# kkahatapitiya/Coarse-Fine-Networks

Hardware: AMD Instinct MI355X
Metric: clips/sec (fwd+bwd+SGD) x3d_fine X3D-M T=256x224x224 (higher is better)
Workload: dtype f32; 1 GPU; x3d_fine X3D-M train step (fwd+loss+bwd+SGD), 8x3x256x224x224 clips per GPU, random-init weights; clips_per_gpu=8, frames=256, parallelism=dp1, launch=eager

## Files before the change

### coarse-fine-networks_amd/cfn_hip/ops.py

```python
import torch
from torch.autograd import Function
from torch.autograd.function import once_differentiable

import ctypes
import threading

from . import call, call_try, check, query, ACT_NONE, ACT_RELU, ACT_SWISH, ACT_SIGMOID


_scratch_epoch = [0]


class _ZeroArena(object):
    CHUNK = 1 << 20

    def __init__(self):
        self.buf, self.off, self.epoch = {}, {}, _scratch_epoch[0]

    def take(self, numel, dev):
        if self.epoch != _scratch_epoch[0]:
            self.buf, self.off, self.epoch = {}, {}, _scratch_epoch[0]
        numel_al = (numel + 1) & ~1
        key = (dev.type, dev.index)
        if key not in self.buf or self.off[key] + numel_al > self.buf[key].numel():
            self.buf[key] = torch.zeros(max(self.CHUNK, numel_al), dtype=torch.float64, device=dev)
            self.off[key] = 0
        o = self.off[key]
        self.off[key] = o + numel_al
        return self.buf[key][o:o + numel]


class _GradCast(object):

    def __init__(self):
        self._reset()
        self.last_total = 0

    def _reset(self):
        self.cur, self.live, self.scheduled, self.seen, self.task = {}, [], False, set(), None

    def begin(self):
        tid = torch._C._current_graph_task_id()
        if tid != self.task:
            if self.live:
                self.flush()
            self._reset()
            self.task = tid

    def first_use(self, w):
        if id(w) in self.seen:
            return False
        self.seen.add(id(w))
        return True

    def take(self, numel, shape, dev):
        al = (numel + 3) & ~3
        key = (dev.type, dev.index)
        ch = self.cur.get(key)
        if ch is None or ch['off'] + al > ch['f64'].numel():
            size = max(int(self.last_total * 1.05) + 1024, al, 1 << 16)
            ch = {'f64': torch.zeros(size, dtype=torch.float64, device=dev),
                  'f32': torch.empty(size, dtype=torch.float32, device=dev), 'off': 0, 'done': 0}
            self.cur[key] = ch
            self.live.append(ch)
        o = ch['off']
        ch['off'] = o + al
        if not self.scheduled:
            torch.autograd.Variable._execution_engine.queue_callback(self._end_of_backward)
            self.scheduled = True
        return ch['f64'][o:o + numel], ch['f32'][o:o + numel].view(shape)

    def flush(self):
        for ch in self.live:
            if ch['off'] > ch['done']:
                ch['f32'][ch['done']:ch['off']].copy_(ch['f64'][ch['done']:ch['off']])
                ch['done'] = ch['off']

    def _end_of_backward(self):
        self.flush()
        self.last_total = max(sum(ch['off'] for ch in self.live), 1)
        self._reset()


class _PerThread(threading.local):

    def __init__(self):
        self.arena = _ZeroArena()
        self.gradcast = _GradCast()


_tls = _PerThread()
LAZY_GRAD_CAST = True


def _f64(n, c, dev):
    return _tls.arena.take(n * c, dev).view(n, c)


def _f64pair(n, c, dev):
    t = _tls.arena.take(2 * n * c, dev).view(2, n, c)
    return t, t[0], t[1]


def reset_scratch():
    _scratch_epoch[0] += 1


def flush_grad_casts():
    _tls.gradcast.flush()


def allow_lazy_grad_cast(params, ok=True):
    for p in params:
        p._cfn_lazy_grad_ok = bool(ok)


def _lazy_ok(w):
    if not LAZY_GRAD_CAST or w is None or not w.is_leaf or w.grad is not None or torch.is_grad_enabled():
        return False
    if not getattr(w, '_cfn_lazy_grad_ok', False):
        return False
    if w._backward_hooks:
        return False
    hooks = getattr(w, '_post_accumulate_grad_hooks', None)
    if hooks:
        from .dist import _BucketHook
        if not all(isinstance(h, _BucketHook) for h in hooks.values()):
            return False
    return True


def _lazy_ok_probe(w):
    with torch.no_grad():
        return _lazy_ok(w)


def _grad_owner(w):
    if w is not None and not w.is_leaf and w._is_view():
        base = w._base
        if base is not None and base.is_leaf and base.numel() == w.numel() and w.is_contiguous() and base.is_contiguous():
            return base
    return w


def _gw_buffers(w, rows, cols, dev):
    gc = _tls.gradcast
    owner = _grad_owner(w)
    if _lazy_ok(owner):
        gc.begin()
        if gc.first_use(owner):
            g64, g32 = gc.take(rows * cols, tuple(w.shape), dev)
            return g64.view(rows, cols), (lambda: g32)
        gc.flush()
    g64 = _f64(rows, cols, dev)
    return g64, (lambda: g64.float().view(tuple(w.shape)))


def _opt(t):
    return None if t is None else t.contiguous()


def _coef(t, rows=None, cols=None):
    if t is None:
        return None
    if rows is not None and t.numel() != rows * cols:
        raise RuntimeError('per-sample coefficients of %d x %d channels expected, got a tensor of shape %s' % (rows, cols, tuple(t.shape)))
    return t.to(torch.float64).contiguous()


class ShortcutToken(object):

    def __init__(self):
        self.acc, self.acc_stride, self.main_done = None, 1, False


class TailLink(object):

    def __init__(self):
        self.y_scale = self.res_scale = None
        self.done = False


def _bf(t):
    return t is not None and t.dtype in (torch.bfloat16, torch.float16)


def subsample_hw(x, s):
    N, C, T, H, W = x.shape
    out = torch.empty(N, C, T, (H - 1) // s + 1, (W - 1) // s + 1, dtype=x.dtype, device=x.device)
    call('cfn_subsample_hw' + _sfx(x), x, out, N * C * T, H, W, s)
    return out


class _PwConv(Function):

    @staticmethod
    def forward(ctx, x, A, B, w, act, stride, want_stats, token, role, tail=None, tail_role=None):
        x = check(x).contiguous()
        N, Cin, T, H, W = x.shape
        Cout = w.shape[0]
        Ho, Wo = (H - 1) // stride + 1, (W - 1) // stride + 1
        y = torch.empty(N, Cout, T, Ho, Wo, dtype=x.dtype, device=x.device)
        s = q = None
        if want_stats:
            s, q = _f64(N, Cout, x.device), _f64(N, Cout, x.device)
        w2 = w.reshape(Cout, Cin).contiguous()
        A, B = _coef(A, N, Cin), _coef(B, N, Cin)
        xs = None
        if _bf(x):
            xs = subsample_hw(x, stride) if stride > 1 else x
            call('cfn_pwconv_fwd' + _sfx(x), xs, A, B, act, w2, y, s, q, N, Cin, Cout, T * Ho * Wo)
        else:
            call('cfn_pwconv_fwd', x, A, B, act, w2, y, s, q, N, Cin, Cout, T, H, W, stride)
        ctx.save_for_backward(x, A, B, w2, y, xs if stride > 1 else None)
        ctx.meta = (act, stride, tuple(w.shape))
        ctx.wparam = w
        ctx.token, ctx.role = token, role
        ctx.tail, ctx.tail_role = tail, tail_role
        if not want_stats:
            return y, None, None
        return y, s, q

    @staticmethod
    @once_differentiable
    def backward(ctx, gy, gs, gq):
        x, A, B, w2, y, xs = ctx.saved_tensors
        act, stride, wshape = ctx.meta
        token, role = ctx.token, ctx.role
        N, Cin, T, H, W = x.shape
        Cout = w2.shape[0]
        gy = torch.zeros_like(y) if gy is None else gy.contiguous()
        gs, gq = _opt(gs), _opt(gq)
        gsc = None
        if ctx.tail is not None and ctx.tail.done:
            gsc = ctx.tail.y_scale if ctx.tail_role == 'y' else ctx.tail.res_scale
        if _bf(x):
            return _PwConv._backward_bf16(ctx, gy, gs, gq, gsc)
        gx = gA = gB = gw = None
        g64 = fin = None
        fused = False
        if ctx.needs_input_grad[0] or (A is not None and ctx.needs_input_grad[1]):
            if token is not None and role == 'short' and stride > 1 and not token.main_done:
                Ho, Wo = y.shape[3], y.shape[4]
                da = torch.empty(N, Cin, T, Ho, Wo, dtype=torch.float32, device=x.device)
                call('cfn_pwconv_bwd_data_acc', gy, y, gs, gq, w2, None, None, None, ACT_NONE, da, None, None, N, Cin, Cout, T,
                     Ho, Wo, 1, None, 1, gsc)
                token.acc, token.acc_stride = da, stride
            else:
                gx = torch.zeros_like(x) if stride != 1 else torch.empty_like(x)
                ab = a64 = b64 = None
                if A is not None:
                    ab, a64, b64 = _f64pair(N, Cin, x.device)
                acc, acc_stride = None, 1
                if token is not None and role == 'main':
                    if token.acc is not None:
                        acc, acc_stride, token.acc = token.acc, token.acc_stride, None
                    else:
                        token.main_done = True
                if stride == 1 and ctx.needs_input_grad[3]:
                    g64, fin = _gw_buffers(ctx.wparam, Cout, Cin, x.device)
                    fused = call_try('cfn_pwconv_bwd_fused', gy, y, gs, gq, w2, x, A, B, act, gx, a64, b64, g64, N, Cin, Cout,
                                     T, H, W, acc, acc_stride, gsc)
                if not fused:
                    call('cfn_pwconv_bwd_data_acc', gy, y, gs, gq, w2, x, A, B, act, gx, a64, b64, N, Cin, Cout, T, H, W, stride,
                         acc, acc_stride, gsc)
                if A is not None:
                    gA, gB = ab[0], ab[1]
        if ctx.needs_input_grad[3]:
            if g64 is None:
                g64, fin = _gw_buffers(ctx.wparam, Cout, Cin, x.device)
            if not fused:
                call('cfn_pwconv_bwd_weight', gy, y, gs, gq, x, A, B, act, g64, N, Cin, Cout, T, H, W, stride, gsc)
            gw = fin()
        return gx, gA, gB, gw, None, None, None, None, None, None, None

    @staticmethod
    def _backward_bf16(ctx, gy, gs, gq, gsc):
        x, A, B, w2, y, xs = ctx.saved_tensors
        act, stride, wshape = ctx.meta
        token, role = ctx.token, ctx.role
        N, Cin, T, H, W = x.shape
        Cout = w2.shape[0]
        Ho, Wo = y.shape[3], y.shape[4]
        xin = xs if stride > 1 else x
        gx = gA = gB = gw = None
        if ctx.needs_input_grad[0] or (A is not None and ctx.needs_input_grad[1]):
            if token is not None and role == 'short' and stride > 1 and not token.main_done:
                da = torch.empty(N, Cin, T, Ho, Wo, dtype=x.dtype, device=x.device)
                call('cfn_pwconv_bwd_data' + _sfx(gy), gy, y, gs, gq, w2, None, None, None, ACT_NONE, da, None, None, N, Cin, Cout, T,
                     Ho, Wo, None, 1, gsc)
                token.acc, token.acc_stride = da, stride
            else:
                ab = a64 = b64 = None
                if A is not None:
                    ab, a64, b64 = _f64pair(N, Cin, x.device)
                acc, acc_stride = None, 1
                if token is not None and role == 'main':
                    if token.acc is not None:
                        acc, acc_stride, token.acc = token.acc, token.acc_stride, None
                    else:
                        token.main_done = True
                gxc = torch.empty_like(xin)
                call('cfn_pwconv_bwd_data' + _sfx(gy), gy, y, gs, gq, w2, xin, A, B, act, gxc, a64, b64, N, Cin, Cout, T, Ho, Wo,
                     acc, acc_stride, gsc)
                if stride > 1:
                    gx = torch.zeros_like(x)
                    gx[:, :, :, ::stride, ::stride] = gxc
                else:
                    gx = gxc
                if A is not None:
                    gA, gB = ab[0], ab[1]
        if ctx.needs_input_grad[3]:
            g64, fin = _gw_buffers(ctx.wparam, Cout, Cin, x.device)
            call('cfn_pwconv_bwd_weight' + _sfx(gy), gy, y, gs, gq, xin, A, B, act, g64, N, Cin, Cout, T * Ho * Wo, gsc)
            gw = fin()
        return gx, gA, gB, gw, None, None, None, None, None, None, None


def pwconv(x, w, A=None, B=None, act=ACT_NONE, stride=1, stats=True, token=None, role=None, tail=None, tail_role=None):
    N, Cin, T, H, W = x.shape
    Ho, Wo = (H - 1) // stride + 1, (W - 1) // stride + 1
    es = x.element_size()
    lim = (1 << 31) if es == 4 else (1 << 30)
    span = max(Cin * H * W, w.shape[0] * H * W, w.shape[0] * Ho * Wo, Cin * Ho * Wo) * es
    needs_grad = torch.is_grad_enabled() and any(t is not None and t.requires_grad for t in (x, w, A, B))
    if span * T < lim or needs_grad or T == 1:
        return _PwConv.apply(x, A, B, w, act, stride, stats, token, role, tail, tail_role)
    step = max((lim - 1) // span, 1)
    odd_plane = es == 2 and (Ho * Wo) % 2 == 1
    if odd_plane:
        if 2 * span >= lim:
            raise RuntimeError('pwconv: two frames of %d x %d x %d bf16 elements exceed the 1 GiB buffer range the frame-range '
                               'chunking has to respect (odd plane: frames travel in pairs)' % (max(Cin, w.shape[0]), H, W))
        step = max(step & ~1, 2)
    y = torch.empty(N, w.shape[0], T, Ho, Wo, dtype=x.dtype, device=x.device)
    s = q = None
    t0 = 0
    while t0 < T:
        t1 = min(t0 + step, T)
        if odd_plane and (t1 - t0) % 2 and t1 - t0 > 1:
            t1 -= 1
        pad = odd_plane and (t1 - t0) % 2 == 1
        xc = x[:, :, t0:t1].contiguous()
        if pad:
            xc = torch.cat([xc, torch.zeros_like(xc)], 2)
        yc, sc, qc = _PwConv.apply(xc, A, B, w, act, stride, False if pad else stats, None, None)
        if pad:
            yc = yc[:, :, :1]
            if stats:
                sc, qc = yc.double().sum((2, 3, 4)), (yc.double() ** 2).sum((2, 3, 4))
        y[:, :, t0:t1] = yc
        if stats:
            s, q = (sc, qc) if s is None else (s + sc, q + qc)
        t0 = t1
    return y, s, q


def _sfx(t):
    return '_bf16' if t.dtype == torch.bfloat16 else ('_f16' if t.dtype == torch.float16 else '')


class _DwConv3d(Function):

    @staticmethod
    def forward(ctx, x, A, B, w, act, stride, want_stats):
        x = check(x).contiguous()
        N, C, T, H, W = x.shape
        Ho, Wo = (H + 2 - 3) // stride + 1, (W + 2 - 3) // stride + 1
        y = torch.empty(N, C, T, Ho, Wo, dtype=x.dtype, device=x.device)
        s = q = None
        if want_stats:
            s, q = _f64(N, C, x.device), _f64(N, C, x.device)
        w2 = w.reshape(C, 27).contiguous()
        A, B = _coef(A, N, C), _coef(B, N, C)
        call('cfn_dwconv3d_fwd' + _sfx(x), x, A, B, act, w2, y, s, q, N, C, T, H, W, stride)
        ctx.save_for_backward(x, A, B, w2, y)
        ctx.meta = (act, stride, tuple(w.shape))
        ctx.wparam = w
        if not want_stats:
            return y, None, None
        return y, s, q

    @staticmethod
    @once_differentiable
    def backward(ctx, gy, gs, gq):
        x, A, B, w2, y = ctx.saved_tensors
        act, stride, wshape = ctx.meta
        N, C, T, H, W = x.shape
        gy = torch.zeros_like(y) if gy is None else gy.contiguous()
        gs, gq = _opt(gs), _opt(gq)
        gx = gA = gB = gw = None
        want_x = ctx.needs_input_grad[0] or (A is not None and ctx.needs_input_grad[1])
        want_w = ctx.needs_input_grad[3]
        ab = a64 = b64 = g64 = fin = None
        if want_x:
            gx = torch.empty_like(x)
            if A is not None:
                ab, a64, b64 = _f64pair(N, C, x.device)
        if want_w:
            g64, fin = _gw_buffers(ctx.wparam, C, 27, x.device)
        sfx = _sfx(x)
        fused = want_x and want_w and stride == 1 and call_try('cfn_dwconv3d_bwd_fused' + sfx, gy, y, gs, gq, w2, x, A, B, act,
                                                             gx, a64, b64, g64, N, C, T, H, W)
        if not fused and want_x and want_w and stride == 2:
            fused = call_try('cfn_dwconv3d_bwd_fused_s2' + sfx, gy, y, gs, gq, w2, x, A, B, act, gx, a64, b64, g64, N, C, T, H, W)
        if not fused:
            if want_x:
                call('cfn_dwconv3d_bwd_data' + sfx, gy, y, gs, gq, w2, x, A, B, act, gx, a64, b64, N, C, T, H, W, stride)
            if want_w:
                call('cfn_dwconv3d_bwd_weight' + sfx, gy, y, gs, gq, x, A, B, act, g64, N, C, T, H, W, stride)
        if want_x and A is not None:
            gA, gB = ab[0], ab[1]
        if want_w:
            gw = fin()
        return gx, gA, gB, gw, None, None, None


def dwconv3d(x, w, A=None, B=None, act=ACT_NONE, stride=1, stats=True):
    return _DwConv3d.apply(x, A, B, w, act, stride, stats)


class _DwConvT5(Function):

    @staticmethod
    def forward(ctx, x, w, want_stats, out_dtype=None):
        x = check(x, torch.float32).contiguous()
        N, C, T, H, W = x.shape
        y = torch.empty_like(x, dtype=out_dtype or x.dtype)
        s = q = None
        if want_stats:
            s, q = _f64(N, C, x.device), _f64(N, C, x.device)
        w2 = w.reshape(C, 5).contiguous()
        call('cfn_dwconv_t5_fwd' + _sfx(y), x, w2, y, s, q, N, C, T, H * W)
        ctx.save_for_backward(x, w2, y)
        ctx.wshape = tuple(w.shape)
        ctx.wparam = w
        if not want_stats:
            return y, None, None
        return y, s, q

    @staticmethod
    @once_differentiable
    def backward(ctx, gy, gs, gq):
        x, w2, y = ctx.saved_tensors
        N, C, T, H, W = x.shape
        gy = torch.zeros_like(y) if gy is None else gy.contiguous()
        gs, gq = _opt(gs), _opt(gq)
        gx = gw = None
        want_x, want_w = ctx.needs_input_grad[0], ctx.needs_input_grad[1]
        if want_x:
            gx = torch.empty_like(x)
        if want_w:
            g64, fin = _gw_buffers(ctx.wparam, C, 5, x.device)
        fused = want_x and want_w and call_try('cfn_dwconv_t5_bwd_fused' + _sfx(y), gy, y, gs, gq, w2, x, gx, g64, N, C, T, H * W)
        if not fused:
            if want_x:
                call('cfn_dwconv_t5_bwd_data' + _sfx(y), gy, y, gs, gq, w2, gx, N, C, T, H * W)
            if want_w:
                call('cfn_dwconv_t5_bwd_weight' + _sfx(y), gy, y, gs, gq, x, g64, N, C, T, H * W)
        if want_w:
            gw = fin()
        return gx, gw, None, None


def dwconv_t5(x, w, stats=True, out_dtype=None):
    return _DwConvT5.apply(x, w, stats, out_dtype)


class _StemConv(Function):

    @staticmethod
    def forward(ctx, x, w):
        x = check(x).contiguous()
        N, Ci, T, H, W = x.shape
        Co = w.shape[0]
        Ho, Wo = (H + 2 - 3) // 2 + 1, (W + 2 - 3) // 2 + 1
        y = torch.empty(N, Co, T, Ho, Wo, dtype=torch.float32, device=x.device)
        w2 = w.reshape(Co, Ci * 9).contiguous()
        call('cfn_stem_conv_fwd', x, w2, y, N, Ci, Co, T, H, W)
        ctx.save_for_backward(x)
        ctx.wshape = tuple(w.shape)
        ctx.wparam = w
        return y

    @staticmethod
    @once_differentiable
    def backward(ctx, gy):
        (x,) = ctx.saved_tensors
        N, Ci, T, H, W = x.shape
        Co = ctx.wshape[0]
        gw = None
        if ctx.needs_input_grad[1]:
            g64, fin = _gw_buffers(ctx.wparam, Co, Ci * 9, x.device)
            call('cfn_stem_conv_bwd_weight', gy.contiguous(), x, g64, N, Ci, Co, T, H, W)
            gw = fin()
        return None, gw


def stem_conv(x, w):
    return _StemConv.apply(x, w)


class _BnFold(Function):

    @staticmethod
    def forward(ctx, s, q, gamma, beta, w1, b1, w2, b2, bufs, cfg):
        training, N, C, S, count, eps, momentum, pool_count = cfg
        run_mean, run_var, nbt = bufs
        dev = run_mean.device
        Wd = w1.shape[0] if w1 is not None else 0
        Se = S if training else 1
        A = torch.empty(N, C, dtype=torch.float64, device=dev)
        B = torch.empty_like(A)
        mean = torch.empty(Se, C, dtype=torch.float64, device=dev)
        rstd = torch.empty_like(mean)
        A0 = B0 = gate = hbuf = pooled = None
        w1c = w2c = None
        if Wd:
            A0, B0, gate, pooled = (torch.empty(N, C, dtype=torch.float32, device=dev) for _ in range(4))
            hbuf = torch.empty(N, Wd, dtype=torch.float32, device=dev)
            w1c, w2c = w1.reshape(Wd, C).contiguous(), w2.reshape(C, Wd).contiguous()
        s, q = _opt(s), _opt(q)
        call('cfn_bn_fold_fwd', s, q, gamma, beta, run_mean, run_var, nbt if training else None, int(training), N, C, S,
             float(count), float(eps), float(momentum), w1c, b1, w2c, b2, Wd, float(pool_count), A, B, mean, rstd,
             A0, B0, gate, hbuf, pooled)
        ctx.save_for_backward(s, gamma, mean, rstd, A0, B0, gate, hbuf, pooled, w1c, w2c)
        ctx.cfg = (training, N, C, S, Wd, count, pool_count, None if w1 is None else tuple(w1.shape),
                   None if w2 is None else tuple(w2.shape))
        return A, B

    @staticmethod
    @once_differentiable
    def backward(ctx, gA, gB):
        s, gamma, mean, rstd, A0, B0, gate, hbuf, pooled, w1c, w2c = ctx.saved_tensors
        training, N, C, S, Wd, count, pool_count, w1s, w2s = ctx.cfg
        dev = mean.device
        gA = torch.zeros(N, C, dtype=torch.float64, device=dev) if gA is None else gA.contiguous()
        gB = torch.zeros(N, C, dtype=torch.float64, device=dev) if gB is None else gB.contiguous()
        gs = gq = None
        if training:
            gs = torch.empty(N, C, dtype=torch.float64, device=dev)
            gq = torch.empty_like(gs)
        elif Wd:
            gs = torch.empty(N, C, dtype=torch.float64, device=dev)
        gg = gbt = None
        if gamma is not None:
            gg, gbt = torch.empty(C, device=dev), torch.empty(C, device=dev)
        gw1 = gb1 = gw2 = gb2 = tA = tB = None
        if Wd:
            gw1, gb1 = torch.empty(Wd, C, device=dev), torch.empty(Wd, device=dev)
            gw2, gb2 = torch.empty(C, Wd, device=dev), torch.empty(C, device=dev)
            tA, tB = (torch.empty(N, C, dtype=torch.float64, device=dev) for _ in range(2))
        call('cfn_bn_fold_bwd', gA, gB, s, gamma, mean, rstd, A0, B0, gate, hbuf, pooled, w1c, w2c, int(training), N, C, S,
             Wd, float(count), float(pool_count), gs, gq, gg, gbt, gw1, gb1, gw2, gb2, tA, tB)
        if Wd:
            gw1, gw2 = gw1.view(w1s), gw2.view(w2s)
        return gs, gq, gg, gbt, gw1, gb1, gw2, gb2, None, None


def bn_fold(s, q, gamma, beta, bufs, training, N, C, S, count, eps, momentum, se=None, pool_count=1.0):
    w1, b1, w2, b2 = se if se is not None else (None, None, None, None)
    return _BnFold.apply(s, q, gamma, beta, w1, b1, w2, b2, bufs, (training, N, C, S, count, eps, momentum, pool_count))


class _BnAddRelu(Function):

    @staticmethod
    def forward(ctx, y, A, B, res, Ar, Br, split, link):
        y, res = check(y).contiguous(), check(res).contiguous()
        N, C = y.shape[:2]
        vol = y[0, 0].numel()
        if tuple(res.shape) != tuple(y.shape):
            raise RuntimeError('bn_add_relu: residual %s does not match y %s' % (tuple(res.shape), tuple(y.shape)))
        out = torch.empty_like(y)
        A, B, Ar, Br = _coef(A, N, C), _coef(B, N, C), _coef(Ar, N, C), _coef(Br, N, C)
        mask = None
        sfx = _sfx(y)
        if link is not None:
            words = query('cfn_bn_add_relu_mask_words' + sfx, N * C, vol)
            if words > 0:
                mask = torch.empty(words, dtype=torch.int32, device=y.device)
        call('cfn_bn_add_relu_fwd' + sfx, y, A, B, res, Ar, Br, out, mask, N * C, vol)
        ctx.link, ctx.has_mask = link, mask is not None
        ctx.save_for_backward(y, A, res, Ar, mask if mask is not None else out)
        if not split:
            return out
        alias = torch.empty(0, dtype=out.dtype, device=out.device).set_(out.untyped_storage(), out.storage_offset(),
                                                                         out.shape, out.stride())
        return out, alias

    @staticmethod
    @once_differentiable
    def backward(ctx, gout, gout2=None):
        y, A, res, Ar, out = ctx.saved_tensors
        N, C = y.shape[:2]
        vol = y[0, 0].numel()
        if gout is None:
            gout, gout2 = gout2, None
        if gout is None:
            gout = torch.zeros_like(y)
        gout2 = None if gout2 is None else gout2.contiguous()
        t3 = _tls.arena.take(3 * N * C, y.device).view(3, N, C)
        gA, gB = t3[0], t3[1]
        gAr = t3[2] if Ar is not None else None
        gBr = gB if Ar is not None else None
        link = ctx.link
        if link is not None:
            g = torch.empty_like(y)
            mask = out if ctx.has_mask else None
            call('cfn_bn_add_relu_bwd_g' + _sfx(y), gout.contiguous(), gout2, None if ctx.has_mask else out, mask, y,
                 res if Ar is not None else None, g, gA, gB, gAr, N * C, vol)
            link.y_scale, link.res_scale, link.done = A.detach(), (None if Ar is None else Ar.detach()), True
            g2 = torch.empty(0, dtype=g.dtype, device=g.device).set_(g.untyped_storage(), g.storage_offset(), g.shape, g.stride())
            return g, gA, gB, g2, gAr, gBr, None, None
        if _bf(y):
            g = torch.empty_like(y)
            call('cfn_bn_add_relu_bwd_g' + _sfx(y), gout.contiguous(), gout2, out, None, y, res if Ar is not None else None, g, gA, gB,
                 gAr, N * C, vol)
            shp = (N, C) + (1,) * (y.dim() - 2)
            gres = g if Ar is None else (g.float() * Ar.float().view(shp)).to(y.dtype)
            return (g.float() * A.float().view(shp)).to(y.dtype), gA, gB, gres, gAr, gBr, None, None
        gy, gres = torch.empty_like(y), torch.empty_like(res)
        call('cfn_bn_add_relu_bwd', gout.contiguous(), gout2, out, y, A, res, Ar, gy, gres, gA, gB, gAr, N * C, vol)
        return gy, gA, gB, gres, gAr, gBr, None, None


def bn_add_relu(y, A, B, res, Ar=None, Br=None, split=False, link=None):
    return _BnAddRelu.apply(y, A, B, res, Ar, Br, split, link)


class _AffineAct(Function):
    @staticmethod
    def forward(ctx, x, A, B, act):
        x = check(x).contiguous()
        N, C = x.shape[:2]
        out = torch.empty_like(x)
        A, B = _coef(A, N, C), _coef(B, N, C)
        call('cfn_affine_act_fwd', x, A, B, act, out, N * C, x[0, 0].numel())
        ctx.save_for_backward(x, A, B)
        ctx.act = act
        return out

    @staticmethod
    @once_differentiable
    def backward(ctx, gout):
        x, A, B = ctx.saved_tensors
        N, C = x.shape[:2]
        gx = torch.empty_like(x)
        a64, b64 = _f64(N, C, x.device), _f64(N, C, x.device)
        call('cfn_affine_act_bwd', gout.contiguous(), x, A, B, ctx.act, gx, a64, b64, N * C, x[0, 0].numel())
        return gx, a64, b64, None


def affine_act(x, A, B, act=ACT_NONE):
    return _AffineAct.apply(x, A, B, act)


class _ChannelStats(Function):

    @staticmethod
    def forward(ctx, x):
        x = check(x).contiguous()
        N, C = x.shape[:2]
        s, q = _f64(N, C, x.device), _f64(N, C, x.device)
        call('cfn_channel_stats', x, s, q, N * C, x[0, 0].numel())
        ctx.save_for_backward(x)
        return s, q

    @staticmethod
    @once_differentiable
    def backward(ctx, gs, gq):
        (x,) = ctx.saved_tensors
        N, C = x.shape[:2]
        gx = torch.zeros_like(x)
        shp = (N, C) + (1,) * (x.dim() - 2)
        if gs is not None:
            gx = gx + gs.float().view(shp)
        if gq is not None:
            gx = gx + 2.0 * gq.float().view(shp) * x
        return gx


def channel_stats(x):
    return _ChannelStats.apply(x)


class _PoolHW(Function):

    @staticmethod
    def forward(ctx, x, A, B, act, OH, OW):
        x = check(x).contiguous()
        N, C, T, H, W = x.shape
        out = torch.empty(N, C, T, OH, OW, dtype=torch.float32, device=x.device)
        A, B = _coef(A, N, C), _coef(B, N, C)
        call('cfn_pool_hw_fwd' + _sfx(x), x, A, B, act, out, N * C, T, H, W, OH, OW)
        ctx.save_for_backward(x, A, B)
        ctx.meta = (act, OH, OW)
        return out

    @staticmethod
    @once_differentiable
    def backward(ctx, gout):
        x, A, B = ctx.saved_tensors
        act, OH, OW = ctx.meta
        N, C, T, H, W = x.shape
        gx = torch.empty_like(x)
        a64 = b64 = None
        if A is not None:
            a64, b64 = _f64(N, C, x.device), _f64(N, C, x.device)
        call('cfn_pool_hw_bwd' + _sfx(x), gout.contiguous(), x, A, B, act, gx, a64, b64, N * C, T, H, W, OH, OW)
        if A is None:
            return gx, None, None, None, None, None
        return gx, a64, b64, None, None, None


def pool_hw(x, OH, OW, A=None, B=None, act=ACT_NONE):
    return _PoolHW.apply(x, A, B, act, OH, OW)


class _Film(Function):

    @staticmethod
    def forward(ctx, x, m, c, f):
        x, m, c = check(x).contiguous(), check(m).contiguous(), check(c).contiguous()
        N, C, T, H, W = x.shape
        want = (N, C, T, H // f if f > 0 else -1, W // f if f > 0 else -1)
        if f <= 0 or H % f or W % f or tuple(m.shape) != want or tuple(c.shape) != want:
            raise RuntimeError('film: coefficients %s / %s do not tile x %s with %d x %d blocks (expected %s)'
                               % (tuple(m.shape), tuple(c.shape), tuple(x.shape), f, f, want))
        out = torch.empty_like(x)
        call('cfn_film_fwd', x, m, c, out, N * C, T, H, W, f)
        ctx.save_for_backward(x, m)
        ctx.f = f
        return out

    @staticmethod
    @once_differentiable
    def backward(ctx, g):
        x, m = ctx.saved_tensors
        N, C, T, H, W = x.shape
        gx, gm, gc = torch.empty_like(x), torch.empty_like(m), torch.empty_like(m)
        call('cfn_film_bwd', g.contiguous(), x, m, gx, gm, gc, N * C, T, H, W, ctx.f)
        return gx, gm, gc, None


def film(x, m, c, f):
    return _Film.apply(x, m, c, f)


class _TimeSample(Function):

    @staticmethod
    def forward(ctx, x, cdf):
        x, cdf = check(x).contiguous(), check(cdf).contiguous()
        B, C, Tin = x.shape[:3]
        K = cdf.shape[1]
        P = x[0, 0, 0].numel()
        out = torch.empty((B, C, K) + tuple(x.shape[3:]), dtype=torch.float32, device=x.device)
        call('cfn_time_sample_fwd', x, cdf, out, B, C, Tin, K, P)
        ctx.save_for_backward(x, cdf)
        return out

    @staticmethod
    @once_differentiable
    def backward(ctx, g):
        x, cdf = ctx.saved_tensors
        B, C, Tin = x.shape[:3]
        K = cdf.shape[1]
        P = x[0, 0, 0].numel()
        gx = torch.empty_like(x) if ctx.needs_input_grad[0] else None
        g64 = torch.zeros(B, K, dtype=torch.float64, device=x.device) if ctx.needs_input_grad[1] else None
        call('cfn_time_sample_bwd', g.contiguous(), x, cdf, gx, g64, B, C, Tin, K, P)
        return gx, (g64.float() if g64 is not None else None)


def time_sample(x, cdf):
    return _TimeSample.apply(x, cdf)


class _TimePool(Function):

    @staticmethod
    def forward(ctx, x, mode, R):
        x = check(x, torch.float32).contiguous()
        B, C, T = x.shape[:3]
        P = x[0, 0, 0].numel()
        out = torch.empty((B, C, T // R) + tuple(x.shape[3:]), dtype=torch.float32, device=x.device)
        call('cfn_time_pool_fwd', x, out, mode, B * C, T, R, P)
        ctx.save_for_backward(x)
        ctx.meta = (mode, R)
        return out

    @staticmethod
    @once_differentiable
    def backward(ctx, g):
        (x,) = ctx.saved_tensors
        mode, R = ctx.meta
        B, C, T = x.shape[:3]
        gx = torch.empty_like(x)
        call('cfn_time_pool_bwd', g.contiguous(), x, gx, mode, B * C, T, R, x[0, 0, 0].numel())
        return gx, None, None


def time_pool(x, mode, R=4):
    return _TimePool.apply(x, {'avg': 0, 'max': 1}[mode], R)


def grid_time_index(cdf, Tin):
    cdf = check(cdf).contiguous()
    i0 = torch.empty(cdf.shape, dtype=torch.int32, device=cdf.device)
    w1 = torch.empty(cdf.shape, dtype=torch.float32, device=cdf.device)
    call('cfn_grid_time_index', cdf, cdf.numel(), Tin, i0, w1)
    return i0, w1


class _Interp1d(Function):
    @staticmethod
    def forward(ctx, x, y, xnew):
        x, y, xnew = check(x).contiguous(), check(y).contiguous(), check(xnew).contiguous()
        B = max(x.shape[0], y.shape[0], xnew.shape[0])
        N, Pq = x.shape[1], xnew.shape[1]
        rows = (int(x.shape[0] > 1), int(y.shape[0] > 1), int(xnew.shape[0] > 1))
        ynew = torch.empty(B, Pq, dtype=torch.float32, device=x.device)
        ind = torch.empty(B, Pq, dtype=torch.int64, device=x.device)
        call('cfn_interp1d_fwd', x, y, xnew, ynew, ind, B, N, Pq, *rows)
        ctx.save_for_backward(x, y, xnew, ind)
        ctx.rows = rows
        ctx.mark_non_differentiable(ind)
        return ynew, ind

    @staticmethod
    @once_differentiable
    def backward(ctx, g, _gind):
        x, y, xnew, ind = ctx.saved_tensors
        B, Pq = ind.shape
        N = x.shape[1]
        gx = torch.zeros_like(x) if ctx.needs_input_grad[0] else None
        gy = torch.zeros_like(y) if ctx.needs_input_grad[1] else None
        gq = torch.zeros_like(xnew) if ctx.needs_input_grad[2] else None
        call('cfn_interp1d_bwd', g.contiguous(), x, y, xnew, ind, gx, gy, gq, B, N, Pq, *ctx.rows)
        return gx, gy, gq


def interp1d(x, y, xnew):
    return _Interp1d.apply(x, y, xnew)


class _TimeResize(Function):

    @staticmethod
    def forward(ctx, x, L, align_corners):
        x = check(x).contiguous()
        BC = x.shape[0] * x.shape[1]
        Kin = x.shape[2]
        P = x[0, 0, 0].numel()
        out = torch.empty(tuple(x.shape[:2]) + (L,) + tuple(x.shape[3:]), dtype=torch.float32, device=x.device)
        call('cfn_time_resize_fwd', x, out, BC, Kin, L, P, int(bool(align_corners)))
        ctx.meta = (tuple(x.shape), L, int(bool(align_corners)))
        return out

    @staticmethod
    @once_differentiable
    def backward(ctx, g):
        shape, L, ac = ctx.meta
        gx = torch.empty(shape, dtype=torch.float32, device=g.device)
        P = 1
        for d in shape[3:]:
            P *= d
        call('cfn_time_resize_bwd', g.contiguous(), gx, shape[0] * shape[1], shape[2], L, P, ac)
        return gx, None, None


def time_resize(x, L, align_corners=True):
    return _TimeResize.apply(x, L, align_corners)


def _geom(kernel, stride, padding):
    return (ctypes.c_int * 9)(*(tuple(kernel) + tuple(stride) + tuple(padding)))


class _ConvDense(Function):

    @staticmethod
    def forward(ctx, x, A, B, w, act, kernel, stride, padding, want_stats):
        x = check(x).contiguous()
        N, Ci, T, H, W = x.shape
        Co = w.shape[0]
        g = _geom(kernel, stride, padding)
        To = (T + 2 * padding[0] - kernel[0]) // stride[0] + 1
        Ho = (H + 2 * padding[1] - kernel[1]) // stride[1] + 1
        Wo = (W + 2 * padding[2] - kernel[2]) // stride[2] + 1
        y = torch.empty(N, Co, To, Ho, Wo, dtype=torch.float32, device=x.device)
        s = q = None
        if want_stats:
            s, q = _f64(N, Co, x.device), _f64(N, Co, x.device)
        w2 = w.reshape(Co, -1).contiguous()
        A, B = _coef(A, N, Ci), _coef(B, N, Ci)
        call('cfn_conv3d_dense_fwd', x, A, B, act, w2, y, s, q, N, Ci, Co, T, H, W, g)
        ctx.save_for_backward(x, A, B, w2, y)
        ctx.meta = (act, tuple(kernel), tuple(stride), tuple(padding), tuple(w.shape))
        ctx.wparam = w
        if not want_stats:
            return y, None, None
        return y, s, q

    @staticmethod
    @once_differentiable
    def backward(ctx, gy, gs, gq):
        x, A, B, w2, y = ctx.saved_tensors
        act, kernel, stride, padding, wshape = ctx.meta
        N, Ci, T, H, W = x.shape
        Co = w2.shape[0]
        g = _geom(kernel, stride, padding)
        gy = torch.zeros_like(y) if gy is None else gy.contiguous()
        gs, gq = _opt(gs), _opt(gq)
        gx = gA = gB = gw = None
        if ctx.needs_input_grad[0] or (A is not None and ctx.needs_input_grad[1]):
            gx = torch.empty_like(x)
            ab = a64 = b64 = None
            if A is not None:
                ab, a64, b64 = _f64pair(N, Ci, x.device)
            call('cfn_conv3d_dense_bwd_data', gy, y, gs, gq, w2, x, A, B, act, gx, a64, b64, N, Ci, Co, T, H, W, g)
            if A is not None:
                gA, gB = ab[0], ab[1]
        if ctx.needs_input_grad[3]:
            g64, fin = _gw_buffers(ctx.wparam, Co, w2.shape[1], x.device)
            call('cfn_conv3d_dense_bwd_weight', gy, y, gs, gq, x, A, B, act, g64, N, Ci, Co, T, H, W, g)
            gw = fin()
        return gx, gA, gB, gw, None, None, None, None, None


def conv3d_dense(x, w, kernel, stride, padding, A=None, B=None, act=ACT_NONE, stats=True):
    return _ConvDense.apply(x, A, B, w, act, kernel, stride, padding, stats)


class _FusionGather(Function):

    @staticmethod
    def forward(ctx, x, at_raw, at_bias, GX, mask, crops):
        x, at_raw, GX, mask = check(x).contiguous(), check(at_raw).contiguous(), check(GX).contiguous(), check(mask).contiguous()
        B, C, Tf, P = x.shape
        K = GX.shape[2]
        if GX.shape[0] != B * crops or GX.shape[1] != Tf or tuple(mask.shape) != (B, Tf) or tuple(at_raw.shape) != (B, Tf, P):
            raise RuntimeError('fusion_gather: inconsistent shapes x %s at %s GX %s mask %s crops %d'
                               % (tuple(x.shape), tuple(at_raw.shape), tuple(GX.shape), tuple(mask.shape), crops))
        z = torch.empty(B * crops, C, K, P, dtype=torch.float32, device=x.device)
        den = torch.empty(B * crops, K, P, dtype=torch.float32, device=x.device)
        call('cfn_fusion_gather_fwd', x, at_raw, at_bias, GX, mask, z, den, B, crops, C, Tf, K, P)
        ctx.save_for_backward(x, at_raw, at_bias, GX, mask, z, den)
        ctx.crops = crops
        return z

    @staticmethod
    @once_differentiable
    def backward(ctx, gz):
        x, at_raw, at_bias, GX, mask, z, den = ctx.saved_tensors
        B, C, Tf, P = x.shape
        K, crops = GX.shape[2], ctx.crops
        need = ctx.needs_input_grad
        gx = torch.empty_like(x) if need[0] else None
        want_at = need[1] or (at_bias is not None and need[2])
        gat = torch.empty_like(at_raw) if want_at else None
        gGX = torch.empty_like(GX) if need[3] else None
        dw = torch.empty(B * crops, Tf, K, P, dtype=torch.float32, device=x.device)
        call('cfn_fusion_gather_bwd', gz.contiguous(), z, den, x, at_raw, at_bias, GX, mask, gx, gat, gGX, dw, B, crops, C, Tf, K, P)
        gb = gat.sum().view(at_bias.shape) if (at_bias is not None and need[2]) else None
        return gx, (gat if need[1] else None), gb, gGX, None, None


def fusion_gather(x, at_raw, at_bias, GX, mask, crops=1):
    return _FusionGather.apply(x, at_raw, at_bias, GX, mask, crops)


class _GaussAlign(Function):

    @staticmethod
    def forward(ctx, meta, mask, gx, tx, ratio, crops, K):
        meta, mask = meta.contiguous(), check(mask).contiguous()
        if meta.dtype != torch.int64:
            meta = meta.to(torch.int64)
        B, Tf = mask.shape
        if gx is not None:
            gx = check(gx).contiguous()
        GX = torch.empty(B * crops, Tf, K, dtype=torch.float32, device=mask.device)
        call('cfn_gauss_align_fwd', meta, mask, gx, float(tx), float(ratio), GX, B, crops, Tf, K)
        ctx.save_for_backward(meta, mask, gx)
        ctx.cfg = (float(tx), float(ratio), crops, K)
        return GX

    @staticmethod
    @once_differentiable
    def backward(ctx, gGX):
        meta, mask, gx = ctx.saved_tensors
        tx, ratio, crops, K = ctx.cfg
        ggx = None
        if gx is not None and ctx.needs_input_grad[2]:
            B, Tf = mask.shape
            ggx = torch.empty_like(gx)
            call('cfn_gauss_align_bwd', gGX.contiguous(), meta, mask, gx, tx, ratio, ggx, B, crops, Tf, K)
        return None, None, ggx, None, None, None, None


def gauss_align(meta, mask, gx, tx, ratio, crops, K):
    return _GaussAlign.apply(meta, mask, gx, 1.0 if tx is None else tx, ratio, crops, K)


class _GridCdf(Function):

    @staticmethod
    def forward(ctx, g, bias):
        g = check(g).contiguous()
        B, Kin = g.shape
        cdf = torch.empty(B, Kin + 1, dtype=torch.float32, device=g.device)
        call('cfn_grid_cdf_fwd', g, bias, cdf, B, Kin)
        ctx.save_for_backward(g, bias)
        return cdf

    @staticmethod
    @once_differentiable
    def backward(ctx, gcdf):
        g, bias = ctx.saved_tensors
        B, Kin = g.shape
        gg = torch.empty_like(g)
        call('cfn_grid_cdf_bwd', gcdf.contiguous(), g, bias, gg, B, Kin)
        gb = gg.sum().view(bias.shape) if (bias is not None and ctx.needs_input_grad[1]) else None
        return gg, gb


def grid_cdf(g, bias=None):
    return _GridCdf.apply(g, bias)
```

### coarse-fine-networks_amd/csrc/pw_common.h

```cpp
#pragma once
#include "cfn_common.h"

typedef float __attribute__((ext_vector_type(16))) f16v;
typedef float __attribute__((ext_vector_type(4))) f4v;

enum { PW_FWD = 0, PW_DGRAD = 1 };
#define PW_KC 32
#define PW_RED_PITCH 33

struct PwArgs {
    const float* src;
    const float* src2;
    const double* pa;
    const double* pb;
    const double* gs;
    const double* gq;
    const double* gsc;
    const float* w;
    float* dst;
    const float* ex;
    const double* ea;
    const double* eb;
    const float* acc; int acc_s, acc_Ho, acc_Wo;
    double* s1;
    double* s2;
    int N, M, K, Q, Pin, Hi, Wi, Ho, Wo, stride, act;
    int Cin;
    int mtiles, nstrips, tpb, kres, Kpad;
    int stem, Cimg, kT, kH, kW, sT, sH, sW, pT, pH, pW, Ti, To;
};

#define PW_UNIT 8
#define PW_KRES_MAX 512

__device__ __forceinline__ float pw_bload(__amdgpu_buffer_rsrc_t r, int voff, int soff) {
    return __builtin_bit_cast(float, __builtin_amdgcn_raw_buffer_load_b32(r, voff, soff, 0));
}


int pwd_try_launch(PwArgs& a, int mode, bool stats, hipStream_t st);

int pws_try_launch(PwArgs& a, int mode, bool stats, hipStream_t st);
int pwk_try_launch(PwArgs& a, int mode, bool stats, hipStream_t st);
int pwt_try_launch(PwArgs& a, int mode, bool stats, hipStream_t st);
int pws_terms_now();
int pws_wgrad_try_launch(const float* gy, const float* y, const double* gs, const double* gq, const double* gsc, const float* x,
                         const double* pa, const double* pb, int act, double* gw, int N, int M, int K, int Q, hipStream_t st);

int pwss_wgrad_try_bf16(const uint16_t* gy, const uint16_t* y, const double* gs, const double* gq, const double* gsc, const uint16_t* x,
                        const double* pa, const double* pb, int act, double* gw, int N, int M, int K, int Q, hipStream_t st);

int pwd_wgrad_try_launch(const float* gy, const float* y, const double* gs, const double* gq, const double* gsc, const float* x,
                         const double* pa, const double* pb, int act, double* gw, int N, int M, int K, int Q, hipStream_t st);
int pwd_wgrad_try_strided(const float* gy, const float* y, const double* gs, const double* gq, const double* gsc, const float* x,
                          const double* pa, const double* pb, int act, double* gw, int N, int M, int K, int T, int Hi, int Wi,
                          int stride, hipStream_t st);
int pwd_wgrad_try_dense(const float* gy, const float* y, const double* gs, const double* gq, const float* x, const double* pa,
                        const double* pb, int act, double* gw, int N, int M, int Cimg, int T, int Hi, int Wi, const int* g,
                        hipStream_t st);

int stem_fwd_try_launch(const float* x, const float* w, float* y, int N, int Cimg, int Cout, int T, int Hi, int Wi, hipStream_t st);
int stem_wgrad_try_launch(const float* gy, const float* x, double* gw, int N, int Cimg, int Cout, int T, int Hi, int Wi, hipStream_t st, bool probe);

int sal_fwd_try_launch(const float* x, const double* A, const double* B, int act, const float* w, float* y, double* sum,
                       double* sumsq, int N, int Cin, int Cout, int T, int Hi, int Wi, const int* g, hipStream_t st);
int pwfs_try_launch(const float* gy, const float* y, const double* gsum, const double* gsumsq, const float* w, const float* x, const double* A,
                    const double* B, int act, float* gx, double* gA, double* gB, double* gw, int N, int Cin, int Cout, int T, int Hi, int Wi,
                    const float* acc, int acc_stride, const double* gscale, hipStream_t st);
int salb_fwd_try_launch(const float* x, const double* A, const double* B, int act, const float* w, float* y, double* sum,
                        double* sumsq, int N, int Cin, int Cout, int T, int Hi, int Wi, const int* g, hipStream_t st);
int sal_wgrad_try_launch(const float* gy, const float* y, const double* gs, const double* gq, const float* x, const double* A,
                         const double* B, int act, double* gw, int N, int Cin, int Cout, int T, int Hi, int Wi, const int* g,
                         hipStream_t st);
```

### coarse-fine-networks_amd/csrc/pwfused.hip

```cpp
#include "cfn_common.h"
#include <stdlib.h>

#include "pw_common.h"

typedef float __attribute__((ext_vector_type(4))) pf4;

#define PF_PT 64
#define PF_PITCH 65

struct PfArgs {
    const float* gy; const float* y; const double* gs; const double* gq; const double* gsc;
    const float* w;
    const float* x; const double* pa; const double* pb;
    float* gx; double* gA; double* gB; double* gw;
    const float* acc; int acc_s, acc_Ho, acc_Wo, Hi, Wi, T;
    int N, M, K, Q, nstrips, stages;
};

template <int MTW, int NTW, int ACT>
__global__ __launch_bounds__(256, ACT < 0 ? 3 : 2) void pw_bwd_fused_kernel(const PfArgs a) {
    extern __shared__ __attribute__((aligned(16))) float smem[];
    constexpr bool EPI = ACT >= 0;
    constexpr int ACTV = EPI ? ACT : CFN_ACT_NONE;
    constexpr int BM = 32 * MTW, BN = 32 * NTW;
    constexpr int NG = BM / 16, NX = BN / 16;
    constexpr int NT16 = BN / 16, KS = BM / 4;
    const int tid = threadIdx.x, wave = tid >> 6, lane = tid & 63, half = lane >> 5, col = lane & 31;
    const int m16 = lane & 15, kq = lane >> 4;
    unsigned L = cfn_xcd_remap(blockIdx.x, gridDim.x);
    const int strip = L % a.nstrips;
    const int n = L / a.nstrips;
    const int M = a.M, K = a.K, Q = a.Q;

    constexpr int IMG = (BM + BN) * PF_PITCH;
    float* img0 = smem;
    float* sCg = smem + 2 * IMG;
    float* sCz = sCg + 2 * BM;
    float* sCx = sCz + BM;
    float* sSt = sCx + 2 * BN;
    for (int m = tid; m < BM; m += 256) {
        const bool ok = m < M;
        sCg[2 * m] = (ok && a.gs) ? (float)a.gs[(long)n * M + m] : 0.0f;
        sCg[2 * m + 1] = (ok && a.gq && a.y) ? 2.0f * (float)a.gq[(long)n * M + m] : 0.0f;
        sCz[m] = (ok && a.gsc) ? (float)a.gsc[(long)n * M + m] : 1.0f;
    }
    for (int k = tid; k < BN; k += 256) {
        const bool ok = EPI && k < K;
        sCx[2 * k] = ok ? (float)a.pa[(long)n * K + k] : 1.0f;
        sCx[2 * k + 1] = ok ? (float)a.pb[(long)n * K + k] : 0.0f;
    }
    float wq[NT16][KS];
#pragma unroll
    for (int t = 0; t < NT16; ++t)
#pragma unroll
        for (int s = 0; s < KS; ++s) {
            const int ci = t * 16 + m16, co = 4 * s + kq;
            wq[t][s] = (ci < K && co < M) ? a.w[(long)co * K + ci] : 0.0f;
        }
    float ca[NTW], cb[NTW];
#pragma unroll
    for (int j = 0; j < NTW; ++j) {
        const int k = j * 32 + col;
        const bool ok = EPI && k < K;
        ca[j] = ok ? (float)a.pa[(long)n * K + k] : 1.0f;
        cb[j] = ok ? (float)a.pb[(long)n * K + k] : 0.0f;
    }
    f16v acc[MTW][NTW];
#pragma unroll
    for (int i = 0; i < MTW; ++i)
#pragma unroll
        for (int j = 0; j < NTW; ++j)
#pragma unroll
            for (int r = 0; r < 16; ++r) acc[i][j][r] = 0.0f;
    float sa[NT16][4], sb[NT16][4];
#pragma unroll
    for (int t = 0; t < NT16; ++t)
#pragma unroll
        for (int r = 0; r < 4; ++r) { sa[t][r] = 0.0f; sb[t][r] = 0.0f; }
    __syncthreads();

    const int lrow = tid >> 4, c4 = (tid & 15) * 4;
    constexpr int OOB = 0x7ffffff0;
    __amdgpu_buffer_rsrc_t rg = cfn_rsrc(const_cast<float*>(a.gy + (long)n * M * Q), (unsigned)((long)M * Q * 4));
    __amdgpu_buffer_rsrc_t ry = cfn_rsrc(const_cast<float*>((a.y ? a.y : a.gy) + (long)n * M * Q), a.y ? (unsigned)((long)M * Q * 4) : 0u);
    __amdgpu_buffer_rsrc_t rx = cfn_rsrc(const_cast<float*>(a.x + (long)n * K * Q), (unsigned)((long)K * Q * 4));
    __amdgpu_buffer_rsrc_t rd = cfn_rsrc(a.gx + (long)n * K * Q, (unsigned)((long)K * Q * 4));
    pf4 pg[NG], py[NG], px[NX];
    int vog[NG], vox[NX];
#pragma unroll
    for (int it = 0; it < NG; ++it) vog[it] = (it * 16 + lrow) < M ? ((it * 16 + lrow) * Q + c4) * 4 : OOB;
#pragma unroll
    for (int it = 0; it < NX; ++it) vox[it] = (it * 16 + lrow) < K ? ((it * 16 + lrow) * Q + c4) * 4 : OOB;
    auto prefetch = [&](int q0) {
        const bool inq = q0 + c4 < Q;
#pragma unroll
        for (int it = 0; it < NG; ++it) {
            const int vo = inq ? vog[it] : OOB;
            pg[it] = __builtin_bit_cast(pf4, __builtin_amdgcn_raw_buffer_load_b128(rg, vo, q0 * 4, 0));
            py[it] = __builtin_bit_cast(pf4, __builtin_amdgcn_raw_buffer_load_b128(ry, vo, q0 * 4, 0));
        }
#pragma unroll
        for (int it = 0; it < NX; ++it)
            px[it] = __builtin_bit_cast(pf4, __builtin_amdgcn_raw_buffer_load_b128(rx, inq ? vox[it] : OOB, q0 * 4, 0));
    };
    auto stage = [&](int q0, float* sG, float* sX) {
        const bool inq = q0 + c4 < Q;
#pragma unroll
        for (int it = 0; it < NG; ++it) {
            const int row = it * 16 + lrow;
            const float cs = cfn_settle(sCg[2 * row]), cq = cfn_settle(sCg[2 * row + 1]), cz = cfn_settle(sCz[row]);
            const bool ok = inq && (row < M);
            float* d = sG + row * PF_PITCH + c4;
            d[0] = ok ? fmaf(py[it].x, cq, fmaf(pg[it].x, cz, cs)) : 0.0f;
            d[1] = ok ? fmaf(py[it].y, cq, fmaf(pg[it].y, cz, cs)) : 0.0f;
            d[2] = ok ? fmaf(py[it].z, cq, fmaf(pg[it].z, cz, cs)) : 0.0f;
            d[3] = ok ? fmaf(py[it].w, cq, fmaf(pg[it].w, cz, cs)) : 0.0f;
        }
#pragma unroll
        for (int it = 0; it < NX; ++it) {
            const int row = it * 16 + lrow;
            float* d = sX + row * PF_PITCH + c4;
            d[0] = px[it].x; d[1] = px[it].y; d[2] = px[it].z; d[3] = px[it].w;
        }
    };

    const int qbeg = strip * a.stages * PF_PT;
    const int nst = min(a.stages, (Q - qbeg + PF_PT - 1) / PF_PT);
    if (nst > 0) {
        prefetch(qbeg);
        stage(qbeg, img0, img0 + BM * PF_PITCH);
        if (nst > 1) prefetch(qbeg + PF_PT);
    }
    __syncthreads();
    const int pbase = wave * (PF_PT / 4);
    const int hw = a.Hi * a.Wi;
    const int acc_pitch4 = a.T * a.acc_Ho * a.acc_Wo * 4;
    __amdgpu_buffer_rsrc_t racc = cfn_rsrc(const_cast<float*>(a.acc ? a.acc + (long)n * K * (acc_pitch4 / 4) : a.gy), a.acc ? (unsigned)((long)K * acc_pitch4) : 0u);
    for (int st = 0; st < nst; ++st) {
        const int q0 = qbeg + st * PF_PT;
        float* cur = img0 + (st & 1) * IMG;
        float* nxt = img0 + ((st + 1) & 1) * IMG;
        if (st + 1 < nst) {
            stage(q0 + PF_PT, nxt, nxt + BM * PF_PITCH);
            if (st + 2 < nst) prefetch(q0 + 2 * PF_PT);
        }
        const float* sG = cur;
        const float* sX = cur + BM * PF_PITCH;
#pragma unroll
        for (int s = 0; s < PF_PT / 8; ++s) {
            const int p = pbase + 2 * s + half;
            float av[MTW], bv[NTW];
#pragma unroll
            for (int i = 0; i < MTW; ++i) av[i] = sG[(i * 32 + col) * PF_PITCH + p];
#pragma unroll
            for (int j = 0; j < NTW; ++j) {
                const float xr = sX[(j * 32 + col) * PF_PITCH + p];
                bv[j] = EPI ? cfn_act<ACTV>(fmaf(xr, ca[j], cb[j])) : xr;
            }
#pragma unroll
            for (int i = 0; i < MTW; ++i)
#pragma unroll
                for (int j = 0; j < NTW; ++j) acc[i][j] = __builtin_amdgcn_mfma_f32_32x32x2f32(av[i], bv[j], acc[i][j], 0, 0, 0);
        }
        pf4 da[NT16];
#pragma unroll
        for (int t = 0; t < NT16; ++t) da[t] = (pf4){0.f, 0.f, 0.f, 0.f};
#pragma unroll
        for (int s = 0; s < KS; ++s) {
            const float b = sG[(4 * s + kq) * PF_PITCH + pbase + m16];
#pragma unroll
            for (int t = 0; t < NT16; ++t) da[t] = __builtin_amdgcn_mfma_f32_16x16x4f32(wq[t][s], b, da[t], 0, 0, 0);
        }
        const int q = q0 + pbase + m16;
        const bool qv = q < Q;
        int aoff = OOB;
        if (a.acc && qv) {
            const int tq = q / hw, rq = q - tq * hw;
            const int hq = rq / a.Wi, wq_ = rq - hq * a.Wi;
            if (hq % a.acc_s == 0 && wq_ % a.acc_s == 0) aoff = (((tq * a.acc_Ho + hq / a.acc_s) * a.acc_Wo + wq_ / a.acc_s)) * 4;
        }
        float av4[NT16][4];
#pragma unroll
        for (int t = 0; t < NT16; ++t)
#pragma unroll
            for (int r = 0; r < 4; ++r) av4[t][r] = 0.0f;
        if (a.acc) {
            const unsigned arow = (unsigned)aoff + (unsigned)(4 * kq) * (unsigned)acc_pitch4;
#pragma unroll
            for (int t = 0; t < NT16; ++t)
#pragma unroll
                for (int r = 0; r < 4; ++r)
                    av4[t][r] = __builtin_bit_cast(float, __builtin_amdgcn_raw_buffer_load_b32(
                        racc, (int)(aoff == OOB ? (unsigned)OOB : arow + (unsigned)r * (unsigned)acc_pitch4), t * 16 * acc_pitch4, 0));
        }
#pragma unroll
        for (int t = 0; t < NT16; ++t) {
#pragma unroll
            for (int r = 0; r < 4; ++r) {
                const int ci = t * 16 + 4 * kq + r;
                const bool ok = qv && ci < K;
                float v = da[t][r] + av4[t][r];
                if (EPI) {
                    const float xr = sX[ci * PF_PITCH + pbase + m16];
                    const float pa = sCx[2 * ci], pb = sCx[2 * ci + 1];
                    const float dz = ok ? v * cfn_act_grad<ACTV>(fmaf(xr, pa, pb)) : 0.0f;
                    sa[t][r] = fmaf(dz, xr, sa[t][r]);
                    sb[t][r] += dz;
                    v = dz * pa;
                }
                __builtin_amdgcn_raw_buffer_store_b32(__builtin_bit_cast(unsigned, v), rd, ok ? (ci * Q + pbase + m16) * 4 : OOB, q0 * 4, 0);
            }
        }
        __syncthreads();
    }

    if (EPI) {
#pragma unroll
        for (int t = 0; t < NT16; ++t)
#pragma unroll
            for (int r = 0; r < 4; ++r) {
                float u = sa[t][r], v = sb[t][r];
#pragma unroll
                for (int o = 1; o < 16; o <<= 1) { u += __shfl_xor(u, o, 64); v += __shfl_xor(v, o, 64); }
                if (m16 == 0) {
                    const int ci = t * 16 + 4 * kq + r;
                    sSt[(wave * BN + ci) * 2] = u;
                    sSt[(wave * BN + ci) * 2 + 1] = v;
                }
            }
    }
    constexpr int CWP = BN + 1;
    float* cw = smem + wave * (BM * CWP);
#pragma unroll
    for (int i = 0; i < MTW; ++i)
#pragma unroll
        for (int j = 0; j < NTW; ++j)
#pragma unroll
            for (int r = 0; r < 16; ++r) {
                const int ml = i * 32 + (r & 3) + 8 * (r >> 2) + 4 * half;
                cw[ml * CWP + j * 32 + col] = acc[i][j][r];
            }
    __syncthreads();
    for (int e = tid; e < BM * BN; e += 256) {
        const int ml = e / BN, kl = e - ml * BN;
        const int o = ml * CWP + kl;
        const float v = (smem[o] + smem[BM * CWP + o]) + (smem[2 * BM * CWP + o] + smem[3 * BM * CWP + o]);
        if (ml < M && kl < K) cfn_add64(&a.gw[(long)ml * K + kl], (double)v);
    }
    if (EPI && tid < K) {
        const float u = (sSt[2 * tid] + sSt[(BN + tid) * 2]) + (sSt[(2 * BN + tid) * 2] + sSt[(3 * BN + tid) * 2]);
        const float v = (sSt[2 * tid + 1] + sSt[(BN + tid) * 2 + 1]) + (sSt[(2 * BN + tid) * 2 + 1] + sSt[(3 * BN + tid) * 2 + 1]);
        cfn_add64(&a.gA[(long)n * K + tid], (double)u);
        cfn_add64(&a.gB[(long)n * K + tid], (double)v);
    }
}

template <int MTW, int NTW>
static int pf_launch(const PfArgs& a, int act, bool epi, unsigned blocks, hipStream_t st) {
    constexpr int BM = 32 * MTW, BN = 32 * NTW;
    size_t lds = ((size_t)2 * (BM + BN) * PF_PITCH + 3 * BM + 10 * BN) * sizeof(float);
    const size_t lds_cw = (size_t)4 * BM * (BN + 1) * sizeof(float);
    if (lds_cw > lds) lds = lds_cw;
#define CFN_PF_GO(ACTV)                                                                                         \
    do {                                                                                                        \
        auto k = pw_bwd_fused_kernel<MTW, NTW, ACTV>;                                                           \
        if (lds > 48 * 1024) (void)hipFuncSetAttribute((const void*)k, hipFuncAttributeMaxDynamicSharedMemorySize, (int)lds); \
        hipLaunchKernelGGL(k, dim3(blocks), dim3(256), lds, st, a);                                             \
    } while (0)
    if (!epi) CFN_PF_GO(-1);
    else if (act == CFN_ACT_RELU) CFN_PF_GO(CFN_ACT_RELU);
    else if (act == CFN_ACT_SWISH) CFN_PF_GO(CFN_ACT_SWISH);
    else CFN_PF_GO(CFN_ACT_NONE);
#undef CFN_PF_GO
    return cfn_check_launch("pwconv_bwd_fused");
}

extern "C" int cfn_pwconv_bwd_fused(const float* gy, const float* y, const double* gsum, const double* gsumsq, const float* w,
                                    const float* x, const double* A, const double* B, int act, float* gx, double* gA, double* gB,
                                    double* gw, int N, int Cin, int Cout, int T, int Hi, int Wi, const float* acc, int acc_stride,
                                    const double* gscale, void* stream) {
    CFN_REQUIRE(gy && w && x && gx && gw, "cfn_pwconv_bwd_fused: null tensor");
    CFN_REQUIRE((A == nullptr) == (B == nullptr), "cfn_pwconv_bwd_fused: A/B mismatch");
    CFN_REQUIRE(A == nullptr || (gA && gB), "cfn_pwconv_bwd_fused: prologue needs gA, gB");
    CFN_REQUIRE(gsumsq == nullptr || y != nullptr, "cfn_pwconv_bwd_fused: gsumsq needs y");
    CFN_REQUIRE(acc == nullptr || acc_stride >= 1, "cfn_pwconv_bwd_fused: bad acc_stride");
    {
        const int rs = pwfs_try_launch(gy, y, gsum, gsumsq, w, x, A, B, act, gx, gA, gB, gw, N, Cin, Cout, T, Hi, Wi, acc, acc_stride, gscale, (hipStream_t)stream);
        if (rs != -1) return rs;
    }
    const long Ql = (long)T * Hi * Wi;
    if (Cin > 64 || Cout > 64 || (Cin > 32 && Cout > 32) || Ql % 4 != 0 || Ql >= (1L << 30)) return -1;
    if ((long)Cout * Ql * 4 >= 0x7ffffff0L || (long)Cin * Ql * 4 >= 0x7ffffff0L) return -1;
    if (A && act != CFN_ACT_NONE && act != CFN_ACT_RELU && act != CFN_ACT_SWISH) return -1;
    if ((((uintptr_t)gy | (uintptr_t)x | (uintptr_t)(y ? y : gy)) & 15) != 0) return -1;
    { const char* e = getenv("CFN_PWF_OFF"); if (e && atoi(e)) return -1; }
    PfArgs a = {};
    a.gy = gy; a.y = gsumsq ? y : nullptr; a.gs = gsum; a.gq = gsumsq; a.gsc = gscale; a.w = w; a.x = x; a.pa = A; a.pb = B;
    a.gx = gx; a.gA = gA; a.gB = gB; a.gw = gw;
    a.acc = acc; a.acc_s = acc ? acc_stride : 1; a.Hi = Hi; a.Wi = Wi; a.T = T;
    a.acc_Ho = (Hi - 1) / a.acc_s + 1; a.acc_Wo = (Wi - 1) / a.acc_s + 1;
    a.N = N; a.M = Cout; a.K = Cin; a.Q = (int)Ql;
    const long nst = cfn_cdiv(Ql, PF_PT);
    const bool epi = A != nullptr;
    static const int wgs_env = getenv("CFN_PWF_WGS") ? atoi(getenv("CFN_PWF_WGS")) : 0;
    long want = (wgs_env > 0 ? wgs_env : (epi ? 1024 : 1536)) / N;
    if (want < 1) want = 1;
    long stages = cfn_cdiv(nst, want);
    if (stages < 4) stages = 4;
    a.stages = (int)stages;
    a.nstrips = (int)cfn_cdiv(nst, stages);
    const unsigned blocks = (unsigned)((long)N * a.nstrips);
    hipStream_t st = (hipStream_t)stream;
    CfnProfScope prof(CFN_K_PWCONV_BWD, st, 4.0 * N * ((double)Cout * Ql * (a.y ? 2 : 1) + (double)Cin * Ql * 2));
    if (Cout > 32) return pf_launch<2, 1>(a, act, epi, blocks, st);
    if (Cin > 32) return pf_launch<1, 2>(a, act, epi, blocks, st);
    return pf_launch<1, 1>(a, act, epi, blocks, st);
}
```

### coarse-fine-networks_amd/csrc/pwfuseds.hip

```cpp
#include "cfn_common.h"
#include <stdlib.h>
#include <map>
#include <mutex>

#include "pw_common.h"

typedef float __attribute__((ext_vector_type(4))) pf4;
typedef __bf16 pfs_bf8 __attribute__((ext_vector_type(8)));
typedef __bf16 pfs_bf2 __attribute__((ext_vector_type(2)));
typedef float pfs_f2 __attribute__((ext_vector_type(2)));
typedef unsigned pfs_u4 __attribute__((ext_vector_type(4)));

#define PFS_PT 64
#define PFS_PITCH 65

__device__ __forceinline__ float pfs_lo(unsigned u) { return __builtin_bit_cast(float, u << 16); }
__device__ __forceinline__ float pfs_hi(unsigned u) { return __builtin_bit_cast(float, u & 0xffff0000u); }
__device__ __forceinline__ unsigned pfs_pack(float lo, float hi) {
    const pfs_bf2 b = __builtin_convertvector((pfs_f2){lo, hi}, pfs_bf2);
    return __builtin_bit_cast(unsigned, b);
}
__device__ __forceinline__ void pfs_split3(float v0, float v1, unsigned (&p)[3]) {
    p[0] = pfs_pack(v0, v1);
    v0 -= pfs_lo(p[0]); v1 -= pfs_hi(p[0]);
    p[1] = pfs_pack(v0, v1);
    v0 -= pfs_lo(p[1]); v1 -= pfs_hi(p[1]);
    p[2] = pfs_pack(v0, v1);
}
#define PFS_TERMS(F) F(2, 0) F(0, 2) F(1, 1) F(1, 0) F(0, 1) F(0, 0)

struct PfsArgs {
    const float* gy; const float* y; const double* gs; const double* gq; const double* gsc;
    const float* w;
    const float* x; const double* pa; const double* pb;
    float* gx; double* gA; double* gB; double* gw;
    const float* acc; int acc_s, acc_Ho, acc_Wo, Hi, Wi, T;
    int N, M, K, Q, nstrips, stages;
    int dbg;
};

template <int MTW, int NTW, int ACT>
__global__ __launch_bounds__(512, 1) void pw_bwd_fused_split_kernel(const PfsArgs a) {
    extern __shared__ __attribute__((aligned(16))) float smem[];
    constexpr bool EPI = ACT >= 0;
    constexpr int ACTV = EPI ? ACT : CFN_ACT_NONE;
    constexpr int BM = 32 * MTW, BN = 32 * NTW;
    constexpr int NG = BM / 16, NX = BN / 16;
    constexpr int NT16 = BN / 16, KS = BM / 32;
    constexpr bool ROWSPLIT = MTW >= NTW;
    constexpr int MI = ROWSPLIT ? MTW / 2 : MTW, NJ = ROWSPLIT ? NTW : NTW / 2;
    constexpr int BMP = BM + 8;
    const int tid = threadIdx.x, wave = cfn_uni((int)(tid >> 6)), lane = tid & 63, half = lane >> 5, col = lane & 31;
    const int m16 = lane & 15, kq = lane >> 4;
    unsigned L = cfn_xcd_remap(blockIdx.x, gridDim.x);
    const int strip = L % a.nstrips;
    const int n = L / a.nstrips;
    const int M = a.M, K = a.K, Q = a.Q;

    constexpr int IMG = (BM + BN) * PFS_PITCH;
    float* img0 = smem;
    float* sCx = smem + 2 * IMG + 3 * BM;
    float* sSt = sCx + 2 * BN;
    unsigned* sW = reinterpret_cast<unsigned*>(sSt + 8 * BN);
    for (int k = tid; k < BN; k += 512) {
        const bool ok = EPI && k < K;
        sCx[2 * k] = ok ? (float)a.pa[(long)n * K + k] : 1.0f;
        sCx[2 * k + 1] = ok ? (float)a.pb[(long)n * K + k] : 0.0f;
    }
    for (int e = tid; e < BN * (BM / 2); e += 512) {
        const int ci = e / (BM / 2), mp = e - ci * (BM / 2), co = 2 * mp;
        const float w0 = (ci < K && co < M) ? a.w[(long)co * K + ci] : 0.0f;
        const float w1 = (ci < K && co + 1 < M) ? a.w[(long)(co + 1) * K + ci] : 0.0f;
        unsigned p[3];
        pfs_split3(w0, w1, p);
#pragma unroll
        for (int s = 0; s < 3; ++s) sW[(s * BN + ci) * (BMP / 2) + mp] = p[s];
    }
    __syncthreads();

    const int lrow = 4 * ((tid & 255) >> 6) + ((lane >> 3) & 3), c4 = ((lane & 7) + 8 * (lane >> 5)) * 4;
    constexpr int OOB = 0x7ffffff0;
    __amdgpu_buffer_rsrc_t rg = cfn_rsrc(const_cast<float*>(a.gy + (long)n * M * Q), (unsigned)((long)M * Q * 4));
    __amdgpu_buffer_rsrc_t ry = cfn_rsrc(const_cast<float*>((a.y ? a.y : a.gy) + (long)n * M * Q), a.y ? (unsigned)((long)M * Q * 4) : 0u);
    __amdgpu_buffer_rsrc_t rx = cfn_rsrc(const_cast<float*>(a.x + (long)n * K * Q), (unsigned)((long)K * Q * 4));
    __amdgpu_buffer_rsrc_t rd = cfn_rsrc(a.gx + (long)n * K * Q, (unsigned)((long)K * Q * 4));
    pf4 pg[NG], py[NG], px[NX];
    int vog[NG], vox[NX];
    float rcs[NG], rcq[NG], rcz[NG];
#pragma unroll
    for (int it = 0; it < NG; ++it) {
        const int row = it * 16 + lrow;
        const bool ok = row < M;
        rcs[it] = (ok && a.gs) ? (float)a.gs[(long)n * M + row] : 0.0f;
        rcq[it] = (ok && a.gq && a.y) ? 2.0f * (float)a.gq[(long)n * M + row] : 0.0f;
        rcz[it] = (ok && a.gsc) ? (float)a.gsc[(long)n * M + row] : 1.0f;
    }
#pragma unroll
    for (int it = 0; it < NG; ++it) vog[it] = (it * 16 + lrow) < M ? ((it * 16 + lrow) * Q + c4) * 4 : OOB;
#pragma unroll
    for (int it = 0; it < NX; ++it) vox[it] = (it * 16 + lrow) < K ? ((it * 16 + lrow) * Q + c4) * 4 : OOB;
    auto prefetch = [&](int q0) {
        const bool inq = q0 + c4 < Q;
#pragma unroll
        for (int it = 0; it < NG; ++it) {
            const int vo = inq ? vog[it] : OOB;
            pg[it] = __builtin_bit_cast(pf4, __builtin_amdgcn_raw_buffer_load_b128(rg, vo, q0 * 4, 0));
            py[it] = __builtin_bit_cast(pf4, __builtin_amdgcn_raw_buffer_load_b128(ry, vo, q0 * 4, 0));
        }
#pragma unroll
        for (int it = 0; it < NX; ++it)
            px[it] = __builtin_bit_cast(pf4, __builtin_amdgcn_raw_buffer_load_b128(rx, inq ? vox[it] : OOB, q0 * 4, 0));
    };
    auto stage = [&](int q0, float* sG, float* sX) {
        const bool inq = q0 + c4 < Q;
#pragma unroll
        for (int it = 0; it < NG; ++it) {
            const int row = it * 16 + lrow;
            const float cs = rcs[it], cq = rcq[it], cz = rcz[it];
            const bool ok = inq && (row < M);
            float* d = sG + row * PFS_PITCH + c4;
            d[0] = ok ? fmaf(py[it].x, cq, fmaf(pg[it].x, cz, cs)) : 0.0f;
            d[1] = ok ? fmaf(py[it].y, cq, fmaf(pg[it].y, cz, cs)) : 0.0f;
            d[2] = ok ? fmaf(py[it].z, cq, fmaf(pg[it].z, cz, cs)) : 0.0f;
            d[3] = ok ? fmaf(py[it].w, cq, fmaf(pg[it].w, cz, cs)) : 0.0f;
        }
#pragma unroll
        for (int it = 0; it < NX; ++it) {
            const int row = it * 16 + lrow;
            float* d = sX + row * PFS_PITCH + c4;
            d[0] = px[it].x; d[1] = px[it].y; d[2] = px[it].z; d[3] = px[it].w;
        }
    };

    const int qbeg = strip * a.stages * PFS_PT;
    const int nst = min(a.stages, (Q - qbeg + PFS_PT - 1) / PFS_PT);
    if (nst > 0 && wave < 4) {
        prefetch(qbeg);
        stage(qbeg, img0, img0 + BM * PFS_PITCH);
        if (nst > 1) prefetch(qbeg + PFS_PT);
    }
    __syncthreads();
    const int pbase = (wave & 3) * (PFS_PT / 4);
    constexpr int CWP = 33, CWT = 32 * CWP;

    if (wave < 4) {
        const int th = wave & 1, ph = wave >> 1;
        const int i0 = ROWSPLIT ? th * MI : 0, j0 = ROWSPLIT ? 0 : th * NJ;
        float ca[NJ], cb[NJ];
#pragma unroll
        for (int j = 0; j < NJ; ++j) {
            const int k = (j0 + j) * 32 + col;
            const bool ok = EPI && k < K;
            ca[j] = ok ? (float)a.pa[(long)n * K + k] : 1.0f;
            cb[j] = ok ? (float)a.pb[(long)n * K + k] : 0.0f;
        }
        f16v acc[MI][NJ];
#pragma unroll
        for (int i = 0; i < MI; ++i)
#pragma unroll
            for (int j = 0; j < NJ; ++j)
#pragma unroll
                for (int r = 0; r < 16; ++r) acc[i][j][r] = 0.0f;
        for (int st = 0; st < nst; ++st) {
            const int q0 = qbeg + st * PFS_PT;
            float* cur = img0 + (st & 1) * IMG;
            float* nxt = img0 + ((st + 1) & 1) * IMG;
            if (st + 1 < nst) {
                stage(q0 + PFS_PT, nxt, nxt + BM * PFS_PITCH);
                if (st + 2 < nst) prefetch(q0 + 2 * PFS_PT);
            }
            const float* sG = cur;
            const float* sX = cur + BM * PFS_PITCH;
            if (!(a.dbg & 1))
#pragma unroll
            for (int kb = 0; kb < 2; ++kb) {
                const int p0 = 32 * ph + 16 * kb + 8 * half;
                pfs_u4 Bf[NJ][3];
#pragma unroll
                for (int j = 0; j < NJ; ++j) {
                    const float* r = sX + ((j0 + j) * 32 + col) * PFS_PITCH + p0;
#pragma unroll
                    for (int h = 0; h < 4; ++h) {
                        float x0 = r[2 * h], x1 = r[2 * h + 1];
                        if (EPI) { x0 = cfn_act<ACTV>(fmaf(x0, ca[j], cb[j])); x1 = cfn_act<ACTV>(fmaf(x1, ca[j], cb[j])); }
                        unsigned p[3];
                        pfs_split3(x0, x1, p);
#pragma unroll
                        for (int s = 0; s < 3; ++s) Bf[j][s][h] = p[s];
                    }
                }
#pragma unroll
                for (int i = 0; i < MI; ++i) {
                    const float* r = sG + ((i0 + i) * 32 + col) * PFS_PITCH + p0;
                    pfs_u4 Af[3];
#pragma unroll
                    for (int h = 0; h < 4; ++h) {
                        unsigned p[3];
                        pfs_split3(r[2 * h], r[2 * h + 1], p);
#pragma unroll
                        for (int s = 0; s < 3; ++s) Af[s][h] = p[s];
                    }
#define PFS_WG(SA, SB) acc[i][j] = __builtin_amdgcn_mfma_f32_32x32x16_bf16(__builtin_bit_cast(pfs_bf8, Af[SA]), __builtin_bit_cast(pfs_bf8, Bf[j][SB]), acc[i][j], 0, 0, 0);
#pragma unroll
                    for (int j = 0; j < NJ; ++j) { PFS_TERMS(PFS_WG) }
#undef PFS_WG
                }
            }
            __syncthreads();
        }
        __syncthreads();
        __syncthreads();
        float* cw = smem + wave * (MI * NJ * CWT);
#pragma unroll
        for (int i = 0; i < MI; ++i)
#pragma unroll
            for (int j = 0; j < NJ; ++j)
#pragma unroll
                for (int r = 0; r < 16; ++r) cw[(i * NJ + j) * CWT + ((r & 3) + 8 * (r >> 2) + 4 * half) * CWP + col] = acc[i][j][r];
    } else {
        float sa[NT16][4], sb[NT16][4];
#pragma unroll
        for (int t = 0; t < NT16; ++t)
#pragma unroll
            for (int r = 0; r < 4; ++r) { sa[t][r] = 0.0f; sb[t][r] = 0.0f; }
        const int hw = a.Hi * a.Wi;
        const int acc_pitch4 = a.T * a.acc_Ho * a.acc_Wo * 4;
        __amdgpu_buffer_rsrc_t racc = cfn_rsrc(const_cast<float*>(a.acc ? a.acc + (long)n * K * (acc_pitch4 / 4) : a.gy), a.acc ? (unsigned)((long)K * acc_pitch4) : 0u);
        for (int st = 0; st < nst; ++st) {
            const int q0 = qbeg + st * PFS_PT;
            float* cur = img0 + (st & 1) * IMG;
            const float* sG = cur;
            const float* sX = cur + BM * PFS_PITCH;
            pf4 da[NT16];
#pragma unroll
            for (int t = 0; t < NT16; ++t) da[t] = (pf4){0.f, 0.f, 0.f, 0.f};
            if (!(a.dbg & 2))
#pragma unroll
            for (int s = 0; s < KS; ++s) {
                const float* r = sG + (32 * s + 8 * kq) * PFS_PITCH + pbase + m16;
                pfs_u4 Gf[3];
#pragma unroll
                for (int h = 0; h < 4; ++h) {
                    unsigned p[3];
                    pfs_split3(r[(2 * h) * PFS_PITCH], r[(2 * h + 1) * PFS_PITCH], p);
#pragma unroll
                    for (int u = 0; u < 3; ++u) Gf[u][h] = p[u];
                }
#pragma unroll
                for (int t = 0; t < NT16; ++t) {
                    const unsigned* wr = sW + ((t * 16 + m16) * BMP + 32 * s + 8 * kq) / 2;
                    pfs_u4 Wf[3];
#pragma unroll
                    for (int u = 0; u < 3; ++u) Wf[u] = *reinterpret_cast<const pfs_u4*>(wr + u * BN * (BMP / 2));
#define PFS_DG(SA, SB) da[t] = __builtin_amdgcn_mfma_f32_16x16x32_bf16(__builtin_bit_cast(pfs_bf8, Wf[SA]), __builtin_bit_cast(pfs_bf8, Gf[SB]), da[t], 0, 0, 0);
                    PFS_TERMS(PFS_DG)
#undef PFS_DG
                    if (NT16 > 4 && (t & 1)) __builtin_amdgcn_sched_barrier(0);
                }
            }
            const int q = q0 + pbase + m16;
            const bool qv = q < Q;
            const int gvo = (qv && !(a.dbg & 8)) ? (4 * kq * Q + pbase + m16) * 4 : OOB;
            int aoff = OOB;
            if (a.acc && qv) {
                const int tq = q / hw, rq = q - tq * hw;
                const int hq = rq / a.Wi, wq_ = rq - hq * a.Wi;
                if (hq % a.acc_s == 0 && wq_ % a.acc_s == 0) aoff = (((tq * a.acc_Ho + hq / a.acc_s) * a.acc_Wo + wq_ / a.acc_s)) * 4;
            }
            const unsigned arow = (unsigned)aoff + (unsigned)(4 * kq) * (unsigned)acc_pitch4;
            constexpr bool AV_UPFRONT = NT16 <= 4;
            float av4[AV_UPFRONT ? NT16 : 1][4];
            if (AV_UPFRONT) {
#pragma unroll
                for (int t = 0; t < NT16; ++t)
#pragma unroll
                    for (int r = 0; r < 4; ++r) av4[AV_UPFRONT ? t : 0][r] = 0.0f;
                if (a.acc) {
#pragma unroll
                    for (int t = 0; t < NT16; ++t)
#pragma unroll
                        for (int r = 0; r < 4; ++r)
                            av4[AV_UPFRONT ? t : 0][r] = __builtin_bit_cast(float, __builtin_amdgcn_raw_buffer_load_b32(
                                racc, (int)(aoff == OOB ? (unsigned)OOB : arow + (unsigned)r * (unsigned)acc_pitch4), t * 16 * acc_pitch4, 0));
                }
            }
#pragma unroll
            for (int t = 0; t < NT16; ++t) {
#pragma unroll
                for (int r = 0; r < 4; ++r) {
                    const int ci = t * 16 + 4 * kq + r;
                    float v = da[t][r];
                    if (AV_UPFRONT) v += av4[AV_UPFRONT ? t : 0][r];
                    else if (a.acc)
                        v += __builtin_bit_cast(float, __builtin_amdgcn_raw_buffer_load_b32(
                            racc, (int)(aoff == OOB ? (unsigned)OOB : arow + (unsigned)r * (unsigned)acc_pitch4), t * 16 * acc_pitch4, 0));
                    if (EPI && !(a.dbg & 4)) {
                        const float xr = sX[ci * PFS_PITCH + pbase + m16];
                        const float2 pab = cfn_settle(*reinterpret_cast<const float2*>(sCx + 2 * ci));
                        const float pa = pab.x, pb = pab.y;
                        const float dz = v * cfn_act_grad<ACTV>(fmaf(xr, pa, pb));
                        sa[t][r] = fmaf(dz, xr, sa[t][r]);
                        sb[t][r] += dz;
                        v = dz * pa;
                    }
                    __builtin_amdgcn_raw_buffer_store_b32(__builtin_bit_cast(unsigned, v), rd, gvo, (q0 + (t * 16 + r) * Q) * 4, 0);
                }
                if (NT16 > 4) __builtin_amdgcn_sched_barrier(0);
            }
            __syncthreads();
        }
        if (EPI) {
#pragma unroll
            for (int t = 0; t < NT16; ++t)
#pragma unroll
                for (int r = 0; r < 4; ++r) {
                    float u = sa[t][r], v = sb[t][r];
#pragma unroll
                    for (int o = 1; o < 16; o <<= 1) { u += __shfl_xor(u, o, 64); v += __shfl_xor(v, o, 64); }
                    if (m16 == 0) {
                        const int ci = t * 16 + 4 * kq + r;
                        sSt[((wave & 3) * BN + ci) * 2] = u;
                        sSt[((wave & 3) * BN + ci) * 2 + 1] = v;
                    }
                }
        }
        __syncthreads();
        const int t2 = tid - 256;
        if (EPI && t2 < K) {
            const float u = (sSt[2 * t2] + sSt[(BN + t2) * 2]) + (sSt[(2 * BN + t2) * 2] + sSt[(3 * BN + t2) * 2]);
            const float v = (sSt[2 * t2 + 1] + sSt[(BN + t2) * 2 + 1]) + (sSt[(2 * BN + t2) * 2 + 1] + sSt[(3 * BN + t2) * 2 + 1]);
            cfn_add64(&a.gA[(long)n * K + t2], (double)u);
            cfn_add64(&a.gB[(long)n * K + t2], (double)v);
        }
        __syncthreads();
    }
    __syncthreads();
    constexpr int WT = MI * NJ;
    for (int e = tid; e < 2 * WT * 1024; e += 512) {
        const int th = e / (WT * 1024), tile = (e >> 10) % WT, ml = (e >> 5) & 31, kl = e & 31, o = tile * CWT + ml * CWP + kl;
        const float v = smem[th * (WT * CWT) + o] + smem[(2 + th) * (WT * CWT) + o];
        const int i = tile / NJ, j = tile - i * NJ;
        const int gm = ((ROWSPLIT ? th * MI : 0) + i) * 32 + ml, gk = ((ROWSPLIT ? 0 : th * NJ) + j) * 32 + kl;
        if (gm < M && gk < K) cfn_add64(&a.gw[(long)gm * K + gk], (double)v);
    }
}

template <int MTW, int NTW>
static int pfs_launch(const PfsArgs& a, int act, bool epi, unsigned blocks, hipStream_t st) {
    constexpr int BM = 32 * MTW, BN = 32 * NTW, BMP = BM + 8;
    size_t lds = ((size_t)2 * (BM + BN) * PFS_PITCH + 3 * BM + 10 * BN) * sizeof(float) + (size_t)3 * BN * BMP * 2;
    const size_t lds_cw = (size_t)4 * (MTW * NTW / 2) * 32 * 33 * sizeof(float);
    if (lds_cw > lds) lds = lds_cw;
#define CFN_PFS_GO(ACTV)                                                                                        \
    do {                                                                                                        \
        auto k = pw_bwd_fused_split_kernel<MTW, NTW, ACTV>;                                                     \
        (void)hipFuncSetAttribute((const void*)k, hipFuncAttributeMaxDynamicSharedMemorySize, (int)lds);        \
        hipLaunchKernelGGL(k, dim3(blocks), dim3(512), lds, st, a);                                             \
    } while (0)
    if (!epi) CFN_PFS_GO(-1);
    else if (act == CFN_ACT_RELU) CFN_PFS_GO(CFN_ACT_RELU);
    else if (act == CFN_ACT_SWISH) CFN_PFS_GO(CFN_ACT_SWISH);
    else CFN_PFS_GO(CFN_ACT_NONE);
#undef CFN_PFS_GO
    return cfn_check_launch("pwconv_bwd_fused (split bf16)");
}

#define PF3_PT 32
#define PF3_PITCH 33
#define PF3_TP 36

struct Pf3Args {
    const float* gy; const float* y; const double* gs; const double* gq; const double* gsc;
    const float* x; const unsigned* wsplit;
    float* gx; double* gw;
    const float* acc; int acc_s, acc_Ho, acc_Wo, Hi, Wi, T;
    int N, M, K, Q, nstrips, stages;
    int dbg;
};

template <int MT, int NT>
__global__ __launch_bounds__(256) void pf3_presplit_kernel(const float* w, int M, int K, unsigned* ws) {
    constexpr int BM = 32 * MT, BN = 32 * NT, BMP = BM + 8;
    const int e = blockIdx.x * 256 + threadIdx.x;
    if (e >= BN * (BMP / 2)) return;
    const int ci = e / (BMP / 2), mp = e - ci * (BMP / 2), co = 2 * mp;
    const float w0 = (ci < K && co < M) ? w[(long)co * K + ci] : 0.0f;
    const float w1 = (ci < K && co + 1 < M) ? w[(long)(co + 1) * K + ci] : 0.0f;
    unsigned p[3];
    pfs_split3(w0, w1, p);
#pragma unroll
    for (int s = 0; s < 3; ++s) ws[(s * BN + ci) * (BMP / 2) + mp] = p[s];
}

template <int MT, int NT>
__global__ __launch_bounds__(512, 1) void pw_bwd_fused_split3_kernel(const Pf3Args a) {
    extern __shared__ __attribute__((aligned(16))) float smem[];
    constexpr int BM = 32 * MT, BN = 32 * NT, BMP = BM + 8;
    constexpr int NG = BM / 32, NX = BN / 32;
    constexpr int NT16 = BN / 16, KS = BM / 32;
    constexpr int NR = (MT + 3) / 4;
    constexpr int NDW = NT16 / 2;
    static_assert(NT16 % 2 == 0 && NDW <= 3, "at most three data-gradient waves beside the staging wave");
    const int tid = threadIdx.x, wave = cfn_uni((int)(tid >> 6)), lane = tid & 63, half = lane >> 5, col = lane & 31;
    const int m16 = lane & 15, kq = lane >> 4;
    unsigned L = cfn_xcd_remap(blockIdx.x, gridDim.x);
    const int strip = L % a.nstrips;
    const int n = L / a.nstrips;
    const int M = a.M, K = a.K, Q = a.Q;
    constexpr int IMG = (BM + BN) * PF3_PITCH;
    float* img0 = smem;
    constexpr int OOB = 0x7ffffff0;
    const int qbeg = strip * a.stages * PF3_PT;
    const int nst = min(a.stages, (Q - qbeg + PF3_PT - 1) / PF3_PT);
    const int lrow = (tid & 255) >> 3, c4 = (tid & 7) * 4;

    if (wave < 4) {
        __amdgpu_buffer_rsrc_t rg = cfn_rsrc(const_cast<float*>(a.gy + (long)n * M * Q), (unsigned)((long)M * Q * 4));
        __amdgpu_buffer_rsrc_t ry = cfn_rsrc(const_cast<float*>((a.y ? a.y : a.gy) + (long)n * M * Q), a.y ? (unsigned)((long)M * Q * 4) : 0u);
        pf4 pg[NG], py[NG];
        int vog[NG];
        float rcs[NG], rcq[NG], rcz[NG];
#pragma unroll
        for (int it = 0; it < NG; ++it) {
            const int row = it * 32 + lrow;
            const bool ok = row < M;
            rcs[it] = (ok && a.gs) ? (float)a.gs[(long)n * M + row] : 0.0f;
            rcq[it] = (ok && a.gq && a.y) ? 2.0f * (float)a.gq[(long)n * M + row] : 0.0f;
            rcz[it] = (ok && a.gsc) ? (float)a.gsc[(long)n * M + row] : 1.0f;
            vog[it] = ok ? (row * Q + c4) * 4 : OOB;
        }
        auto prefetch = [&](int q0) {
            const bool inq = q0 + c4 < Q;
#pragma unroll
            for (int it = 0; it < NG; ++it) {
                const int vo = inq ? vog[it] : OOB;
                pg[it] = __builtin_bit_cast(pf4, __builtin_amdgcn_raw_buffer_load_b128(rg, vo, q0 * 4, 0));
                py[it] = __builtin_bit_cast(pf4, __builtin_amdgcn_raw_buffer_load_b128(ry, vo, q0 * 4, 0));
            }
        };
        auto stage = [&](int q0, float* sG) {
            const bool inq = q0 + c4 < Q;
#pragma unroll
            for (int it = 0; it < NG; ++it) {
                const int row = it * 32 + lrow;
                const float cs = rcs[it], cq = rcq[it], cz = rcz[it];
                const bool ok = inq && (row < M);
                float* d = sG + row * PF3_PITCH + c4;
                d[0] = ok ? fmaf(py[it].x, cq, fmaf(pg[it].x, cz, cs)) : 0.0f;
                d[1] = ok ? fmaf(py[it].y, cq, fmaf(pg[it].y, cz, cs)) : 0.0f;
                d[2] = ok ? fmaf(py[it].z, cq, fmaf(pg[it].z, cz, cs)) : 0.0f;
                d[3] = ok ? fmaf(py[it].w, cq, fmaf(pg[it].w, cz, cs)) : 0.0f;
            }
        };
        if (nst > 0) {
            prefetch(qbeg);
            stage(qbeg, img0);
            if (nst > 1) prefetch(qbeg + PF3_PT);
        }
        __syncthreads();
        f16v acc[NR][NT];
#pragma unroll
        for (int t = 0; t < NR; ++t)
#pragma unroll
            for (int j = 0; j < NT; ++j)
#pragma unroll
                for (int r = 0; r < 16; ++r) acc[t][j][r] = 0.0f;
        for (int st = 0; st < nst; ++st) {
            const int q0 = qbeg + st * PF3_PT;
            float* cur = img0 + (st & 1) * IMG;
            float* nxt = img0 + ((st + 1) & 1) * IMG;
            if (st + 1 < nst) {
                stage(q0 + PF3_PT, nxt);
                if (st + 2 < nst) prefetch(q0 + 2 * PF3_PT);
            }
            const float* sG = cur;
            const float* sX = cur + BM * PF3_PITCH;
            if (!(a.dbg & 1))
#pragma unroll
            for (int kb = 0; kb < 2; ++kb) {
                const int p0 = 16 * kb + 8 * half;
                pfs_u4 Af[NR][3];
#pragma unroll
                for (int t = 0; t < NR; ++t) {
                    const int i = wave + 4 * t;
                    if (i < MT) {
                        const float* r = sG + (i * 32 + col) * PF3_PITCH + p0;
#pragma unroll
                        for (int h = 0; h < 4; ++h) {
                            unsigned p[3];
                            pfs_split3(r[2 * h], r[2 * h + 1], p);
#pragma unroll
                            for (int s = 0; s < 3; ++s) Af[t][s][h] = p[s];
                        }
                    }
                }
#pragma unroll
                for (int j = 0; j < NT; ++j) {
                    pfs_u4 Bf[3];
                    const float* r = sX + (j * 32 + col) * PF3_PITCH + p0;
#pragma unroll
                    for (int h = 0; h < 4; ++h) {
                        unsigned p[3];
                        pfs_split3(r[2 * h], r[2 * h + 1], p);
#pragma unroll
                        for (int s = 0; s < 3; ++s) Bf[s][h] = p[s];
                    }
#define PF3_WG(SA, SB)                                                                                                                         \
                    _Pragma("unroll") for (int t = 0; t < NR; ++t)                                                                              \
                        if (wave + 4 * t < MT)                                                                                                  \
                            acc[t][j] = __builtin_amdgcn_mfma_f32_32x32x16_bf16(__builtin_bit_cast(pfs_bf8, Af[t][SA]), __builtin_bit_cast(pfs_bf8, Bf[SB]), acc[t][j], 0, 0, 0);
                    PFS_TERMS(PF3_WG)
#undef PF3_WG
                }
            }
            __syncthreads();
        }
#pragma unroll
        for (int t = 0; t < NR; ++t) {
            const int i = wave + 4 * t;
            if (i < MT) {
#pragma unroll
                for (int j = 0; j < NT; ++j)
#pragma unroll
                    for (int r = 0; r < 16; ++r) {
                        const int gm = i * 32 + (r & 3) + 8 * (r >> 2) + 4 * half, gk = j * 32 + col;
                        const float v = acc[t][j][r];
                        if (gm < M && gk < K) cfn_add64(&a.gw[(long)gm * K + gk], (double)v);
                    }
            }
        }
    } else if (wave < 4 + NDW) {
        const int d = wave - 4;
        __amdgpu_buffer_rsrc_t rd = cfn_rsrc(a.gx + (long)n * K * Q, (unsigned)((long)K * Q * 4));
        __amdgpu_buffer_rsrc_t rw = cfn_rsrc(const_cast<unsigned*>(a.wsplit), (unsigned)((size_t)3 * BN * (BMP / 2) * 4));
        const int wlane = ((m16 * BMP + 8 * kq) / 2) * 4;
        pfs_u4 Wr[2][KS][3];
#pragma unroll
        for (int t = 0; t < 2; ++t)
#pragma unroll
            for (int s = 0; s < KS; ++s)
#pragma unroll
                for (int u = 0; u < 3; ++u)
                    Wr[t][s][u] = __builtin_bit_cast(pfs_u4, __builtin_amdgcn_raw_buffer_load_b128(rw, wlane, (((u * BN + (2 * d + t) * 16) * BMP + 32 * s) / 2) * 4, 0));
        const int hw = a.Hi * a.Wi;
        const int acc_pitch4 = a.T * a.acc_Ho * a.acc_Wo * 4;
        __amdgpu_buffer_rsrc_t racc = cfn_rsrc(const_cast<float*>(a.acc ? a.acc + (long)n * K * (acc_pitch4 / 4) : a.gy), a.acc ? (unsigned)((long)K * acc_pitch4) : 0u);
        __syncthreads();
        for (int st = 0; st < nst; ++st) {
            const int q0 = qbeg + st * PF3_PT;
            const float* sG = img0 + (st & 1) * IMG;
            float av[2][2][4];
#pragma unroll
            for (int pb = 0; pb < 2; ++pb)
#pragma unroll
                for (int t = 0; t < 2; ++t)
#pragma unroll
                    for (int r = 0; r < 4; ++r) av[pb][t][r] = 0.0f;
            if (a.acc) {
#pragma unroll
                for (int pb = 0; pb < 2; ++pb) {
                    const int q = q0 + 16 * pb + m16;
                    int aoff = OOB;
                    if (q < Q) {
                        const int tq = q / hw, rq = q - tq * hw;
                        const int hq = rq / a.Wi, wq_ = rq - hq * a.Wi;
                        if (hq % a.acc_s == 0 && wq_ % a.acc_s == 0) aoff = (((tq * a.acc_Ho + hq / a.acc_s) * a.acc_Wo + wq_ / a.acc_s)) * 4;
                    }
                    const unsigned arow = (unsigned)aoff + (unsigned)(4 * kq) * (unsigned)acc_pitch4;
#pragma unroll
                    for (int t = 0; t < 2; ++t)
#pragma unroll
                        for (int r = 0; r < 4; ++r)
                            av[pb][t][r] = __builtin_bit_cast(float, __builtin_amdgcn_raw_buffer_load_b32(
                                racc, (int)(aoff == OOB ? (unsigned)OOB : arow + (unsigned)r * (unsigned)acc_pitch4), (2 * d + t) * 16 * acc_pitch4, 0));
                }
            }
            pf4 da[2][2];
#pragma unroll
            for (int pb = 0; pb < 2; ++pb)
#pragma unroll
                for (int t = 0; t < 2; ++t) da[pb][t] = (pf4){0.f, 0.f, 0.f, 0.f};
            if (!(a.dbg & 2))
#pragma unroll
            for (int s = 0; s < KS; ++s) {
#pragma unroll
                for (int pb = 0; pb < 2; ++pb) {
                    const float* r = sG + (32 * s + 8 * kq) * PF3_PITCH + 16 * pb + m16;
                    pfs_u4 Gf[3];
#pragma unroll
                    for (int h = 0; h < 4; ++h) {
                        unsigned p[3];
                        pfs_split3(r[(2 * h) * PF3_PITCH], r[(2 * h + 1) * PF3_PITCH], p);
#pragma unroll
                        for (int u = 0; u < 3; ++u) Gf[u][h] = p[u];
                    }
#define PF3_DG(SA, SB)                                                                                                                         \
                    _Pragma("unroll") for (int t = 0; t < 2; ++t)                                                                               \
                        da[pb][t] = __builtin_amdgcn_mfma_f32_16x16x32_bf16(__builtin_bit_cast(pfs_bf8, Wr[t][s][SA]), __builtin_bit_cast(pfs_bf8, Gf[SB]), da[pb][t], 0, 0, 0);
                    PFS_TERMS(PF3_DG)
#undef PF3_DG
                }
            }
            float* tile = smem + 2 * IMG + d * (32 * PF3_TP);
#pragma unroll
            for (int pb = 0; pb < 2; ++pb)
#pragma unroll
                for (int t = 0; t < 2; ++t)
#pragma unroll
                    for (int r = 0; r < 4; ++r) {
                        const float v = da[pb][t][r] + av[pb][t][r];
                        tile[(t * 16 + 4 * kq + r) * PF3_TP + 16 * pb + m16] = v;
                    }
            __builtin_amdgcn_fence(__ATOMIC_RELEASE, "wavefront");
            __builtin_amdgcn_wave_barrier();
            __builtin_amdgcn_fence(__ATOMIC_ACQUIRE, "wavefront");
            {
                const int seg = lane & 7, r0 = lane >> 3;
                const bool inq = q0 + 4 * seg < Q && !(a.dbg & 8);
#pragma unroll
                for (int ps = 0; ps < 4; ++ps) {
                    const int row = ps * 8 + r0;
                    const pf4 v = *reinterpret_cast<const pf4*>(tile + row * PF3_TP + 4 * seg);
                    __builtin_amdgcn_raw_buffer_store_b128(__builtin_bit_cast(pfs_u4, v), rd, inq ? (r0 * Q + 4 * seg) * 4 : OOB, (q0 + (32 * d + ps * 8) * Q) * 4, 0);
                }
            }
            __syncthreads();
        }
    } else if (wave < 7) {
        __syncthreads();
        for (int st = 0; st < nst; ++st) __syncthreads();
    } else {
        __amdgpu_buffer_rsrc_t rx = cfn_rsrc(const_cast<float*>(a.x + (long)n * K * Q), (unsigned)((long)K * Q * 4));
        constexpr int NP = BN / 8;
        const int xrow = lane >> 3;
        pf4 px[NP];
        int vox[NP];
#pragma unroll
        for (int it = 0; it < NP; ++it) vox[it] = (it * 8 + xrow) < K ? ((it * 8 + xrow) * Q + c4) * 4 : OOB;
        auto prefetch = [&](int q0) {
            const bool inq = q0 + c4 < Q;
#pragma unroll
            for (int it = 0; it < NP; ++it)
                px[it] = __builtin_bit_cast(pf4, __builtin_amdgcn_raw_buffer_load_b128(rx, inq ? vox[it] : OOB, q0 * 4, 0));
        };
        auto stage = [&](float* sX) {
#pragma unroll
            for (int it = 0; it < NP; ++it) {
                float* dd = sX + (it * 8 + xrow) * PF3_PITCH + c4;
                dd[0] = px[it].x; dd[1] = px[it].y; dd[2] = px[it].z; dd[3] = px[it].w;
            }
        };
        if (nst > 0) {
            prefetch(qbeg);
            stage(img0 + BM * PF3_PITCH);
            if (nst > 1) prefetch(qbeg + PF3_PT);
        }
        __syncthreads();
        for (int st = 0; st < nst; ++st) {
            const int q0 = qbeg + st * PF3_PT;
            float* nxt = img0 + ((st + 1) & 1) * IMG;
            if (st + 1 < nst) {
                stage(nxt + BM * PF3_PITCH);
                if (st + 2 < nst) prefetch(q0 + 2 * PF3_PT);
            }
            __syncthreads();
        }
    }
}

struct Pf3eArgs {
    const float* gy; const float* y; const double* gs; const double* gq; const double* gsc;
    const float* x; const double* pa; const double* pb; const unsigned* wsplit;
    float* gx; double* gA; double* gB; double* gw;
    int N, M, K, Q, nstrips, stages;
};

template <int MT, int NT, int ACT>
__global__ __launch_bounds__(512, 1) void pw_bwd_fused_split3e_kernel(const Pf3eArgs a) {
    extern __shared__ __attribute__((aligned(16))) float smem[];
    constexpr int BM = 32 * MT, BN = 32 * NT, BMP = BM + 8;
    constexpr int NG = BM / 32, NX = BN / 32;
    constexpr int NT16 = BN / 16, KS = BM / 32;
    constexpr int NC = (NT + 3) / 4;
    constexpr int ND = 4;
    static_assert(NT16 <= 4 * ND, "four data-gradient waves x four channel tiles");
    const int tid = threadIdx.x, wave = cfn_uni((int)(tid >> 6)), lane = tid & 63, half = lane >> 5, col = lane & 31;
    const int m16 = lane & 15, kq = lane >> 4;
    unsigned L = cfn_xcd_remap(blockIdx.x, gridDim.x);
    const int strip = L % a.nstrips;
    const int n = L / a.nstrips;
    const int M = a.M, K = a.K, Q = a.Q;
    constexpr int IMG = (BM + BN) * PF3_PITCH;
    float* img0 = smem;
    float* sCx = smem + 2 * IMG;
    constexpr int OOB = 0x7ffffff0;
    const int qbeg = strip * a.stages * PF3_PT;
    const int nst = min(a.stages, (Q - qbeg + PF3_PT - 1) / PF3_PT);
    for (int k = tid; k < BN; k += 512) {
        const bool ok = k < K;
        sCx[2 * k] = ok ? (float)a.pa[(long)n * K + k] : 1.0f;
        sCx[2 * k + 1] = ok ? (float)a.pb[(long)n * K + k] : 0.0f;
    }

    if (wave < 4) {
        const int lrow = tid >> 3, c4 = (tid & 7) * 4;
        __amdgpu_buffer_rsrc_t rg = cfn_rsrc(const_cast<float*>(a.gy + (long)n * M * Q), (unsigned)((long)M * Q * 4));
        __amdgpu_buffer_rsrc_t ry = cfn_rsrc(const_cast<float*>((a.y ? a.y : a.gy) + (long)n * M * Q), a.y ? (unsigned)((long)M * Q * 4) : 0u);
        __amdgpu_buffer_rsrc_t rx = cfn_rsrc(const_cast<float*>(a.x + (long)n * K * Q), (unsigned)((long)K * Q * 4));
        pf4 pg[NG], py[NG], px[NX];
        int vog[NG], vox[NX];
        float rcs[NG], rcq[NG], rcz[NG];
#pragma unroll
        for (int it = 0; it < NG; ++it) {
            const int row = it * 32 + lrow;
            const bool ok = row < M;
            rcs[it] = (ok && a.gs) ? (float)a.gs[(long)n * M + row] : 0.0f;
            rcq[it] = (ok && a.gq && a.y) ? 2.0f * (float)a.gq[(long)n * M + row] : 0.0f;
            rcz[it] = (ok && a.gsc) ? (float)a.gsc[(long)n * M + row] : 1.0f;
            vog[it] = ok ? (row * Q + c4) * 4 : OOB;
        }
#pragma unroll
        for (int it = 0; it < NX; ++it) vox[it] = (it * 32 + lrow) < K ? ((it * 32 + lrow) * Q + c4) * 4 : OOB;
        auto prefetch = [&](int q0) {
            const bool inq = q0 + c4 < Q;
#pragma unroll
            for (int it = 0; it < NG; ++it) {
                const int vo = inq ? vog[it] : OOB;
                pg[it] = __builtin_bit_cast(pf4, __builtin_amdgcn_raw_buffer_load_b128(rg, vo, q0 * 4, 0));
                py[it] = __builtin_bit_cast(pf4, __builtin_amdgcn_raw_buffer_load_b128(ry, vo, q0 * 4, 0));
            }
#pragma unroll
            for (int it = 0; it < NX; ++it)
                px[it] = __builtin_bit_cast(pf4, __builtin_amdgcn_raw_buffer_load_b128(rx, inq ? vox[it] : OOB, q0 * 4, 0));
        };
        auto stage = [&](int q0, float* sG, float* sX) {
            const bool inq = q0 + c4 < Q;
#pragma unroll
            for (int it = 0; it < NG; ++it) {
                const int row = it * 32 + lrow;
                const float cs = rcs[it], cq = rcq[it], cz = rcz[it];
                const bool ok = inq && (row < M);
                float* d = sG + row * PF3_PITCH + c4;
                d[0] = ok ? fmaf(py[it].x, cq, fmaf(pg[it].x, cz, cs)) : 0.0f;
                d[1] = ok ? fmaf(py[it].y, cq, fmaf(pg[it].y, cz, cs)) : 0.0f;
                d[2] = ok ? fmaf(py[it].z, cq, fmaf(pg[it].z, cz, cs)) : 0.0f;
                d[3] = ok ? fmaf(py[it].w, cq, fmaf(pg[it].w, cz, cs)) : 0.0f;
            }
#pragma unroll
            for (int it = 0; it < NX; ++it) {
                float* d = sX + (it * 32 + lrow) * PF3_PITCH + c4;
                d[0] = px[it].x; d[1] = px[it].y; d[2] = px[it].z; d[3] = px[it].w;
            }
        };
        if (nst > 0) {
            prefetch(qbeg);
            stage(qbeg, img0, img0 + BM * PF3_PITCH);
            if (nst > 1) prefetch(qbeg + PF3_PT);
        }
        float ca[NC], cb[NC];
#pragma unroll
        for (int c = 0; c < NC; ++c) {
            const int k = (wave + 4 * c) * 32 + col;
            const bool ok = k < K;
            ca[c] = ok ? (float)a.pa[(long)n * K + k] : 1.0f;
            cb[c] = ok ? (float)a.pb[(long)n * K + k] : 0.0f;
        }
        __syncthreads();
        f16v acc[NC][MT];
#pragma unroll
        for (int c = 0; c < NC; ++c)
#pragma unroll
            for (int i = 0; i < MT; ++i)
#pragma unroll
                for (int r = 0; r < 16; ++r) acc[c][i][r] = 0.0f;
        for (int st = 0; st < nst; ++st) {
            const int q0 = qbeg + st * PF3_PT;
            float* cur = img0 + (st & 1) * IMG;
            float* nxt = img0 + ((st + 1) & 1) * IMG;
            if (st + 1 < nst) {
                stage(q0 + PF3_PT, nxt, nxt + BM * PF3_PITCH);
                if (st + 2 < nst) prefetch(q0 + 2 * PF3_PT);
            }
            const float* sG = cur;
            const float* sX = cur + BM * PF3_PITCH;
#pragma unroll
            for (int kb = 0; kb < 2; ++kb) {
                const int p0 = 16 * kb + 8 * half;
                pfs_u4 Bf[NC][3];
#pragma unroll
                for (int c = 0; c < NC; ++c) {
                    const int j = wave + 4 * c;
                    if (j < NT) {
                        const float* r = sX + (j * 32 + col) * PF3_PITCH + p0;
#pragma unroll
                        for (int h = 0; h < 4; ++h) {
                            const float x0 = cfn_act<ACT>(fmaf(r[2 * h], ca[c], cb[c])), x1 = cfn_act<ACT>(fmaf(r[2 * h + 1], ca[c], cb[c]));
                            unsigned p[3];
                            pfs_split3(x0, x1, p);
#pragma unroll
                            for (int s = 0; s < 3; ++s) Bf[c][s][h] = p[s];
                        }
                    }
                }
#pragma unroll
                for (int i = 0; i < MT; ++i) {
                    pfs_u4 Af[3];
                    const float* r = sG + (i * 32 + col) * PF3_PITCH + p0;
#pragma unroll
                    for (int h = 0; h < 4; ++h) {
                        unsigned p[3];
                        pfs_split3(r[2 * h], r[2 * h + 1], p);
#pragma unroll
                        for (int s = 0; s < 3; ++s) Af[s][h] = p[s];
                    }
#define PF3E_WG(SA, SB)                                                                                                                        \
                    _Pragma("unroll") for (int c = 0; c < NC; ++c)                                                                              \
                        if (wave + 4 * c < NT)                                                                                                  \
                            acc[c][i] = __builtin_amdgcn_mfma_f32_32x32x16_bf16(__builtin_bit_cast(pfs_bf8, Af[SA]), __builtin_bit_cast(pfs_bf8, Bf[c][SB]), acc[c][i], 0, 0, 0);
                    PFS_TERMS(PF3E_WG)
#undef PF3E_WG
                }
            }
            __syncthreads();
        }
#pragma unroll
        for (int c = 0; c < NC; ++c) {
            const int j = wave + 4 * c;
            if (j < NT) {
#pragma unroll
                for (int i = 0; i < MT; ++i)
#pragma unroll
                    for (int r = 0; r < 16; ++r) {
                        const int gm = i * 32 + (r & 3) + 8 * (r >> 2) + 4 * half, gk = j * 32 + col;
                        const float v = acc[c][i][r];
                        if (gm < M && gk < K) cfn_add64(&a.gw[(long)gm * K + gk], (double)v);
                    }
            }
        }
    } else {
        const int d = wave - 4;
        const int tb = ND * d, tn = ND;
        __amdgpu_buffer_rsrc_t rd = cfn_rsrc(a.gx + (long)n * K * Q, (unsigned)((long)K * Q * 4));
        __amdgpu_buffer_rsrc_t rw = cfn_rsrc(const_cast<unsigned*>(a.wsplit), (unsigned)((size_t)3 * BN * (BMP / 2) * 4));
        const int wlane = ((m16 * BMP + 8 * kq) / 2) * 4;
        pfs_u4 Wr[ND][KS][3];
#pragma unroll
        for (int t = 0; t < ND; ++t)
#pragma unroll
            for (int s = 0; s < KS; ++s)
#pragma unroll
                for (int u = 0; u < 3; ++u)
                    Wr[t][s][u] = (t < tn && tb + t < NT16) ? __builtin_bit_cast(pfs_u4, __builtin_amdgcn_raw_buffer_load_b128(rw, wlane, cfn_uni((((u * BN + (tb + t) * 16) * BMP + 32 * s) / 2) * 4), 0))
                                                      : (pfs_u4){0u, 0u, 0u, 0u};
        float sa[ND][4], sb[ND][4];
#pragma unroll
        for (int t = 0; t < ND; ++t)
#pragma unroll
            for (int r = 0; r < 4; ++r) { sa[t][r] = 0.0f; sb[t][r] = 0.0f; }
        __syncthreads();
        for (int st = 0; st < nst; ++st) {
            const int q0 = qbeg + st * PF3_PT;
            const float* sG = img0 + (st & 1) * IMG;
            const float* sX = sG + BM * PF3_PITCH;
            pf4 da[2][ND];
#pragma unroll
            for (int pb = 0; pb < 2; ++pb)
#pragma unroll
                for (int t = 0; t < ND; ++t) da[pb][t] = (pf4){0.f, 0.f, 0.f, 0.f};
#pragma unroll
            for (int s = 0; s < KS; ++s) {
#pragma unroll
                for (int pb = 0; pb < 2; ++pb) {
                    const float* r = sG + (32 * s + 8 * kq) * PF3_PITCH + 16 * pb + m16;
                    pfs_u4 Gf[3];
#pragma unroll
                    for (int h = 0; h < 4; ++h) {
                        unsigned p[3];
                        pfs_split3(r[(2 * h) * PF3_PITCH], r[(2 * h + 1) * PF3_PITCH], p);
#pragma unroll
                        for (int u = 0; u < 3; ++u) Gf[u][h] = p[u];
                    }
#define PF3E_DG(SA, SB)                                                                                                                        \
                    _Pragma("unroll") for (int t = 0; t < ND; ++t)                                                                              \
                        da[pb][t] = __builtin_amdgcn_mfma_f32_16x16x32_bf16(__builtin_bit_cast(pfs_bf8, Wr[t][s][SA]), __builtin_bit_cast(pfs_bf8, Gf[SB]), da[pb][t], 0, 0, 0);
                    PFS_TERMS(PF3E_DG)
#undef PF3E_DG
                }
            }
#pragma unroll
            for (int pb = 0; pb < 2; ++pb) {
                const int q = q0 + 16 * pb + m16;
                const int gvo = q < Q ? (4 * kq * Q + 16 * pb + m16) * 4 : OOB;
#pragma unroll
                for (int t = 0; t < ND; ++t) {
#pragma unroll
                    for (int r = 0; r < 4; ++r) {
                        const int ci = (tb + t) * 16 + 4 * kq + r;
                        const float v = da[pb][t][r];
                        const float xr = sX[ci * PF3_PITCH + 16 * pb + m16];
                        const float2 pab = cfn_settle(*reinterpret_cast<const float2*>(sCx + 2 * ci));
                        const float dz = v * cfn_act_grad<ACT>(fmaf(xr, pab.x, pab.y));
                        sa[t][r] = fmaf(dz, xr, sa[t][r]);
                        sb[t][r] += dz;
                        const float o = dz * pab.x;
                        __builtin_amdgcn_raw_buffer_store_b32(__builtin_bit_cast(unsigned, o), rd, gvo, (q0 + ((tb + t) * 16 + r) * Q) * 4, 0);
                    }
                    __builtin_amdgcn_sched_barrier(0);
                }
            }
            __syncthreads();
        }
#pragma unroll
        for (int t = 0; t < ND; ++t)
#pragma unroll
            for (int r = 0; r < 4; ++r) {
                float u = sa[t][r], v = sb[t][r];
#pragma unroll
                for (int o = 1; o < 16; o <<= 1) { u += __shfl_xor(u, o, 64); v += __shfl_xor(v, o, 64); }
                const int ci = (tb + t) * 16 + 4 * kq + r;
                if (m16 == 0 && t < tn && ci < K) {
                    cfn_add64(&a.gA[(long)n * K + ci], (double)u);
                    cfn_add64(&a.gB[(long)n * K + ci], (double)v);
                }
            }
    }
}

static unsigned* pf3_workspace(size_t bytes, hipStream_t st) {
    static std::mutex mu;
    static std::map<std::pair<int, hipStream_t>, std::pair<unsigned*, size_t>> bufs;
    int dev = 0;
    if (hipGetDevice(&dev) != hipSuccess) { (void)hipGetLastError(); return nullptr; }
    std::lock_guard<std::mutex> lk(mu);
    auto& b = bufs[std::make_pair(dev, st)];
    if (b.second >= bytes) return b.first;
    hipStreamCaptureStatus cs = hipStreamCaptureStatusNone;
    if (hipStreamIsCapturing(st, &cs) != hipSuccess || cs != hipStreamCaptureStatusNone) return nullptr;
    unsigned* p = nullptr;
    if (hipMalloc(&p, bytes) != hipSuccess) { (void)hipGetLastError(); return nullptr; }
    b = {p, bytes};
    return p;
}

template <int NT>
static int pf3_launch(const float* gy, const float* y, const double* gsum, const double* gsumsq, const float* w, const float* x, float* gx, double* gw,
                      int N, int Cin, int Cout, int T, int Hi, int Wi, const float* acc, int acc_stride, const double* gscale, hipStream_t st) {
    constexpr int MT = 7, BM = 32 * MT, BN = 32 * NT, BMP = BM + 8;
    const long Ql = (long)T * Hi * Wi;
    const size_t wbytes = (size_t)3 * BN * (BMP / 2) * 4;
    unsigned* ws = pf3_workspace(wbytes, st);
    if (!ws) return -1;
    hipLaunchKernelGGL((pf3_presplit_kernel<MT, NT>), dim3((BN * (BMP / 2) + 255) / 256), dim3(256), 0, st, w, Cout, Cin, ws);
    Pf3Args a = {};
    a.gy = gy; a.y = gsumsq ? y : nullptr; a.gs = gsum; a.gq = gsumsq; a.gsc = gscale; a.x = x; a.wsplit = ws; a.gx = gx; a.gw = gw;
    a.acc = acc; a.acc_s = acc ? acc_stride : 1; a.Hi = Hi; a.Wi = Wi; a.T = T;
    a.acc_Ho = (Hi - 1) / a.acc_s + 1; a.acc_Wo = (Wi - 1) / a.acc_s + 1;
    a.N = N; a.M = Cout; a.K = Cin; a.Q = (int)Ql;
    { const char* e = getenv("CFN_PWFS_DBG"); a.dbg = e ? atoi(e) : 0; }
    const long nst = cfn_cdiv(Ql, PF3_PT);
    static const int wgs_env = getenv("CFN_PWF3_WGS") ? atoi(getenv("CFN_PWF3_WGS")) : 0;
    const long wgs = wgs_env > 0 ? wgs_env : ((long)N * nst > 256L * 100 ? 512 : 256);
    long want = wgs / N;
    if (want < 1) want = 1;
    long stages = cfn_cdiv(nst, want);
    if (stages < 4) stages = 4;
    a.stages = (int)stages;
    a.nstrips = (int)cfn_cdiv(nst, stages);
    const unsigned blocks = (unsigned)((long)N * a.nstrips);
    const size_t lds = ((size_t)2 * (BM + BN) * PF3_PITCH + 3 * 32 * PF3_TP) * sizeof(float);
    CfnProfScope prof(CFN_K_PWCONV_BWD, st, 4.0 * N * ((double)Cout * Ql * (a.y ? 2 : 1) + (double)Cin * Ql * 2));
    auto k = pw_bwd_fused_split3_kernel<MT, NT>;
    (void)hipFuncSetAttribute((const void*)k, hipFuncAttributeMaxDynamicSharedMemorySize, (int)lds);
    hipLaunchKernelGGL(k, dim3(blocks), dim3(512), lds, st, a);
    return cfn_check_launch("pwconv_bwd_fused (split bf16, layer 3)");
}

static int pf3e_try_launch(const float* gy, const float* y, const double* gsum, const double* gsumsq, const float* w, const float* x, const double* A, const double* B,
                           int act, float* gx, double* gA, double* gB, double* gw, int N, int Cin, int Cout, long Ql, const double* gscale, hipStream_t st) {
    constexpr int MT = 3, NT = 7, BM = 32 * MT, BN = 32 * NT, BMP = BM + 8;
    const size_t wbytes = (size_t)3 * BN * (BMP / 2) * 4;
    unsigned* ws = pf3_workspace(wbytes, st);
    if (!ws) return -1;
    hipLaunchKernelGGL((pf3_presplit_kernel<MT, NT>), dim3((BN * (BMP / 2) + 255) / 256), dim3(256), 0, st, w, Cout, Cin, ws);
    Pf3eArgs a = {};
    a.gy = gy; a.y = gsumsq ? y : nullptr; a.gs = gsum; a.gq = gsumsq; a.gsc = gscale; a.x = x; a.pa = A; a.pb = B; a.wsplit = ws;
    a.gx = gx; a.gA = gA; a.gB = gB; a.gw = gw;
    a.N = N; a.M = Cout; a.K = Cin; a.Q = (int)Ql;
    const long nst = cfn_cdiv(Ql, PF3_PT);
    static const int wgs = getenv("CFN_PWF3_WGS") ? atoi(getenv("CFN_PWF3_WGS")) : 256;
    long want = wgs / N;
    if (want < 1) want = 1;
    long stages = cfn_cdiv(nst, want);
    if (stages < 4) stages = 4;
    a.stages = (int)stages;
    a.nstrips = (int)cfn_cdiv(nst, stages);
    const unsigned blocks = (unsigned)((long)N * a.nstrips);
    const size_t lds = ((size_t)2 * (BM + BN) * PF3_PITCH + 2 * BN) * sizeof(float);
    CfnProfScope prof(CFN_K_PWCONV_BWD, st, 4.0 * N * ((double)Cout * Ql * (a.y ? 2 : 1) + (double)Cin * Ql * 2));
#define CFN_PF3E_GO(ACTV)                                                                                       \
    do {                                                                                                        \
        auto k = pw_bwd_fused_split3e_kernel<MT, NT, ACTV>;                                                     \
        (void)hipFuncSetAttribute((const void*)k, hipFuncAttributeMaxDynamicSharedMemorySize, (int)lds);        \
        hipLaunchKernelGGL(k, dim3(blocks), dim3(512), lds, st, a);                                             \
    } while (0)
    if (act == CFN_ACT_RELU) CFN_PF3E_GO(CFN_ACT_RELU);
    else if (act == CFN_ACT_SWISH) CFN_PF3E_GO(CFN_ACT_SWISH);
    else CFN_PF3E_GO(CFN_ACT_NONE);
#undef CFN_PF3E_GO
    return cfn_check_launch("pwconv_bwd_fused (split bf16, layer 3 conv3)");
}

int pwfs_try_launch(const float* gy, const float* y, const double* gsum, const double* gsumsq, const float* w, const float* x, const double* A,
                    const double* B, int act, float* gx, double* gA, double* gB, double* gw, int N, int Cin, int Cout, int T, int Hi, int Wi,
                    const float* acc, int acc_stride, const double* gscale, hipStream_t st) {
    const char* env_on = getenv("CFN_PWF_SPLIT");
    const int on = env_on ? atoi(env_on) : 1;
    if (!on || pws_terms_now() != 6) return -1;
    const bool wide_m = Cout > 64 && Cout <= 128 && Cin > 32 && Cin <= 64;
    const bool thin_k = Cout > 64 && Cout <= 128 && Cin >= 16 && Cin <= 32;
    const bool wide_k = Cin > 64 && Cin <= 128 && Cout > 32 && Cout <= 64;
    const bool l1_m = on >= 3 && Cout > 32 && Cout <= 64 && Cin >= 16 && Cin <= 32;
    const bool l1_k = on >= 3 && Cin > 32 && Cin <= 64 && Cout >= 16 && Cout <= 32;
    static const int l3_on = getenv("CFN_PWF_L3") ? atoi(getenv("CFN_PWF_L3")) : 1;
    if (on >= 1 && l3_on && A == nullptr && Cout > 192 && Cout <= 224 && Cin > 32 && Cin <= 96) {
        const long Ql3 = (long)T * Hi * Wi;
        if (Ql3 % 4 == 0 && Ql3 < (1L << 30) && (long)Cout * Ql3 * 4 < 0x7ffffff0L && ((((uintptr_t)gy | (uintptr_t)x | (uintptr_t)(y ? y : gy)) & 15) == 0) &&
            (acc == nullptr || acc_stride >= 1)) {
            if (Cin > 64) return pf3_launch<3>(gy, y, gsum, gsumsq, w, x, gx, gw, N, Cin, Cout, T, Hi, Wi, acc, acc_stride, gscale, st);
            return pf3_launch<2>(gy, y, gsum, gsumsq, w, x, gx, gw, N, Cin, Cout, T, Hi, Wi, acc, acc_stride, gscale, st);
        }
    }
    const char* env_l3e = getenv("CFN_PWF_L3E");
    const int l3e_on = env_l3e ? atoi(env_l3e) : 0;
    if (on >= 1 && l3e_on && A != nullptr && acc == nullptr && Cout > 64 && Cout <= 96 && Cin > 192 && Cin <= 224) {
        const long Ql3 = (long)T * Hi * Wi;
        if (Ql3 % 4 == 0 && Ql3 < (1L << 30) && (long)Cin * Ql3 * 4 < 0x7ffffff0L && ((((uintptr_t)gy | (uintptr_t)x | (uintptr_t)(y ? y : gy)) & 15) == 0) &&
            (act == CFN_ACT_NONE || act == CFN_ACT_RELU || act == CFN_ACT_SWISH))
            return pf3e_try_launch(gy, y, gsum, gsumsq, w, x, A, B, act, gx, gA, gB, gw, N, Cin, Cout, Ql3, gscale, st);
    }
    if (!wide_m && !wide_k && !thin_k && !l1_m && !l1_k) return -1;
    if (A != nullptr && on < 2) return -1;
    const long Ql = (long)T * Hi * Wi;
    if (Ql % 4 != 0 || Ql >= (1L << 30)) return -1;
    if ((long)Cout * Ql * 4 >= 0x7ffffff0L || (long)Cin * Ql * 4 >= 0x7ffffff0L) return -1;
    if (A && act != CFN_ACT_NONE && act != CFN_ACT_RELU && act != CFN_ACT_SWISH) return -1;
    if ((((uintptr_t)gy | (uintptr_t)x | (uintptr_t)(y ? y : gy)) & 15) != 0) return -1;
    PfsArgs a = {};
    a.gy = gy; a.y = gsumsq ? y : nullptr; a.gs = gsum; a.gq = gsumsq; a.gsc = gscale; a.w = w; a.x = x; a.pa = A; a.pb = B;
    a.gx = gx; a.gA = gA; a.gB = gB; a.gw = gw;
    a.acc = acc; a.acc_s = acc ? acc_stride : 1; a.Hi = Hi; a.Wi = Wi; a.T = T;
    a.acc_Ho = (Hi - 1) / a.acc_s + 1; a.acc_Wo = (Wi - 1) / a.acc_s + 1;
    a.N = N; a.M = Cout; a.K = Cin; a.Q = (int)Ql;
    { const char* e = getenv("CFN_PWFS_DBG"); a.dbg = e ? atoi(e) : 0; }
    const long nst = cfn_cdiv(Ql, PFS_PT);
    static const int wgs = getenv("CFN_PWFS_WGS") ? atoi(getenv("CFN_PWFS_WGS")) : 512;
    long want = wgs / N;
    if (want < 1) want = 1;
    long stages = cfn_cdiv(nst, want);
    if (stages < 4) stages = 4;
    a.stages = (int)stages;
    a.nstrips = (int)cfn_cdiv(nst, stages);
    const unsigned blocks = (unsigned)((long)N * a.nstrips);
    CfnProfScope prof(CFN_K_PWCONV_BWD, st, 4.0 * N * ((double)Cout * Ql * (a.y ? 2 : 1) + (double)Cin * Ql * 2));
    const bool epi = A != nullptr;
    if (wide_m) return pfs_launch<4, 2>(a, act, epi, blocks, st);
    if (thin_k) return pfs_launch<4, 1>(a, act, epi, blocks, st);
    if (l1_m) return pfs_launch<2, 1>(a, act, epi, blocks, st);
    if (l1_k) return pfs_launch<1, 2>(a, act, epi, blocks, st);
    return pfs_launch<2, 4>(a, act, epi, blocks, st);
}
```

### coarse-fine-networks_amd/x3d_fine.py

```python
import os

import torch
import torch.nn as nn
import torch.nn.functional as F

from cfn_hip import ops, ACT_NONE, ACT_RELU, ACT_SWISH

USE_TORCH_OPS = os.environ.get('CFN_USE_TORCH_OPS', '0') == '1'


class Deferred(object):
    __slots__ = ('raw', 'A', 'B', 'act')

    def __init__(self, raw, A, B, act):
        self.raw, self.A, self.B, self.act = raw, A, B, act

    @property
    def shape(self):
        return self.raw.shape

    def materialize(self):
        return ops.affine_act(self.raw, self.A, self.B, self.act)


def _unpack(x):
    if isinstance(x, Deferred):
        return x.raw, x.A, x.B, x.act
    return x, None, None, ACT_NONE


class SubBatchNorm3d(nn.Module):

    def __init__(self, num_splits, **args):
        super(SubBatchNorm3d, self).__init__()
        self.num_splits = num_splits
        self.num_features = args['num_features']
        self.eps = args.get('eps', 1e-5)
        self.momentum = args.get('momentum', 0.1)
        if args.get('affine', True):
            self.affine = True
            self.weight = nn.Parameter(torch.ones(self.num_features))
            self.bias = nn.Parameter(torch.zeros(self.num_features))
        else:
            self.affine = False
        self.bn = nn.BatchNorm3d(self.num_features, eps=self.eps, momentum=self.momentum, affine=False)
        self.split_bn = nn.BatchNorm3d(self.num_features * self.num_splits, eps=self.eps, momentum=self.momentum,
                                       affine=False)

    def aggregate_stats(self):
        if self.split_bn.track_running_stats:
            n = self.num_splits
            means = self.split_bn.running_mean.view(n, -1)
            mean = means.sum(0) / n
            var = self.split_bn.running_var.view(n, -1).sum(0) / n + ((means - mean) ** 2).sum(0) / n
            self.bn.running_mean.data = mean.detach()
            self.bn.running_var.data = var.detach()

    def fold(self, s, q, count, n, se=None):
        if self.training:
            bufs = (self.split_bn.running_mean, self.split_bn.running_var, self.split_bn.num_batches_tracked)
        else:
            bufs = (self.bn.running_mean, self.bn.running_var, self.bn.num_batches_tracked)
        gamma, beta = (self.weight, self.bias) if self.affine else (None, None)
        return ops.bn_fold(s, q, gamma, beta, bufs, self.training, n, self.num_features, self.num_splits, count, self.eps,
                           self.momentum, se=se, pool_count=count)

    def fold_op(self, s, q, count, n, se=None):
        tr = self.training
        bn = self.split_bn if tr else self.bn
        gamma, beta = (self.weight, self.bias) if self.affine else (None, None)
        w1, b1, w2, b2 = se if se is not None else (None, None, None, None)
        out = torch.ops.cfn.bn_fold(s, q, gamma, beta, bn.running_mean, bn.running_var, bn.num_batches_tracked, tr, n,
                                    self.num_features, self.num_splits, float(count), self.eps, self.momentum, w1, b1, w2, b2, float(count))
        if tr:
            with torch.no_grad():
                bn.running_mean.copy_(out[9])
                bn.running_var.copy_(out[10])
                bn.num_batches_tracked.copy_(out[11])
        return out[0], out[1]

    def forward(self, x):
        n = x.shape[0]
        s = q = None
        if self.training:
            s, q = ops.channel_stats(x)
        A, B = self.fold(s, q, x[0, 0].numel(), n)
        return ops.affine_act(x, A, B, ACT_NONE)


class Swish(nn.Module):

    def forward(self, x):
        n, c = x.shape[:2]
        one = torch.ones(n, c, device=x.device)
        return ops.affine_act(x, one, torch.zeros_like(one), ACT_SWISH)


def conv3x3x3(in_planes, out_planes, stride=1, t_downsample=False):
    return nn.Conv3d(in_planes, out_planes, kernel_size=3, stride=stride if t_downsample else (1, stride, stride), padding=1,
                     bias=False, groups=in_planes)


def conv1x1x1(in_planes, out_planes, stride=1, t_downsample=False):
    return nn.Conv3d(in_planes, out_planes, kernel_size=1, stride=stride if t_downsample else (1, stride, stride), bias=False)


def _every(x, s):
    return x if s == 1 else x[:, :, ::s].contiguous()


def _count(y):
    return y.shape[2] * y.shape[3] * y.shape[4]


class Bottleneck(nn.Module):

    def __init__(self, in_planes, planes, stride=1, downsample=None, index=0, base_bn_splits=8, t_downsample=False):
        super(Bottleneck, self).__init__()
        self.index = index
        self.base_bn_splits = base_bn_splits
        self.conv1 = conv1x1x1(in_planes, planes[0])
        self.bn1 = SubBatchNorm3d(num_splits=base_bn_splits, num_features=planes[0], affine=True)
        self.conv2 = conv3x3x3(planes[0], planes[0], stride, t_downsample=t_downsample)
        self.bn2 = SubBatchNorm3d(num_splits=base_bn_splits, num_features=planes[0], affine=True)
        self.conv3 = conv1x1x1(planes[0], planes[1], t_downsample=t_downsample)
        self.bn3 = SubBatchNorm3d(num_splits=base_bn_splits, num_features=planes[1], affine=True)
        self.swish = Swish()
        self.relu = nn.ReLU(inplace=True)
        if self.index % 2 == 0:
            width = self.round_width(planes[0])
            self.global_pool = nn.AdaptiveAvgPool3d((1, 1, 1))
            self.fc1 = nn.Conv3d(planes[0], width, kernel_size=1, stride=1)
            self.fc2 = nn.Conv3d(width, planes[0], kernel_size=1, stride=1)
            self.sigmoid = nn.Sigmoid()
        self.downsample = downsample
        self.stride = stride
        self.t_stride = stride if t_downsample else 1
        self.split_out = False

    def round_width(self, width, multiplier=0.0625, min_width=8, divisor=8):
        if not multiplier:
            return width
        width *= multiplier
        min_width = min_width or divisor
        width_out = max(min_width, int(width + divisor / 2) // divisor * divisor)
        if width_out < 0.9 * width:
            width_out += divisor
        return int(width_out)

    def _forward_torch_ops(self, x):
        import cfn_hip.torchlib
        T = torch.ops.cfn
        if isinstance(x, tuple):
            x = x[0]
        if isinstance(x, Deferred):
            x = x.materialize()
        if self.t_stride != 1 or (self.downsample is not None and not isinstance(self.downsample, nn.Sequential)):
            raise NotImplementedError('CFN_USE_TORCH_OPS: t_downsample / shortcut type A run on the default path only')
        n = x.shape[0]
        has_se = self.index % 2 == 0
        y1, s1, q1 = T.pwconv(x, self.conv1.weight, None, None, ACT_NONE, 1)
        A1, B1 = self.bn1.fold_op(s1, q1, _count(y1), n)
        y2, s2, q2 = T.dwconv3d(y1, self.conv2.weight, A1, B1, ACT_RELU, self.stride)
        se = (self.fc1.weight, self.fc1.bias, self.fc2.weight, self.fc2.bias) if has_se else None
        A2, B2 = self.bn2.fold_op(s2, q2, _count(y2), n, se=se)
        y3, s3, q3 = T.pwconv(y2, self.conv3.weight, A2, B2, ACT_SWISH, 1)
        A3, B3 = self.bn3.fold_op(s3, q3, _count(y3), n)
        if self.downsample is not None:
            yd, sd, qd = T.pwconv(x, self.downsample[0].weight, None, None, ACT_NONE, self.stride)
            Ad, Bd = self.downsample[1].fold_op(sd, qd, _count(yd), n)
            return T.bn_add_relu(y3, A3, B3, yd, Ad, Bd)
        return T.bn_add_relu(y3, A3, B3, x)

    def forward(self, x):
        if USE_TORCH_OPS:
            return self._forward_torch_ops(x)
        x, x_res = x if isinstance(x, tuple) else (x, x)
        xr, xa, xb, xact = _unpack(x)
        n = xr.shape[0]
        tr = self.training
        has_se = self.index % 2 == 0

        ts = self.t_stride
        tok = ops.ShortcutToken() if (isinstance(self.downsample, nn.Sequential) and self.stride > 1 and ts == 1) else None
        y1, s1, q1 = ops.pwconv(xr, self.conv1.weight, xa, xb, xact, 1, stats=tr, token=tok, role='main')
        A1, B1 = self.bn1.fold(s1, q1, _count(y1), n)
        if ts == 1:
            y2, s2, q2 = ops.dwconv3d(y1, self.conv2.weight, A1, B1, ACT_RELU, self.stride, stats=tr or has_se)
        else:
            y2f, _, _ = ops.dwconv3d(y1, self.conv2.weight, A1, B1, ACT_RELU, self.stride, stats=False)
            y2 = _every(y2f, ts)
            s2, q2 = ops.channel_stats(y2) if (tr or has_se) else (None, None)
        se = (self.fc1.weight, self.fc1.bias, self.fc2.weight, self.fc2.bias) if has_se else None
        A2, B2 = self.bn2.fold(s2, q2, _count(y2), n, se=se)
        link = ops.TailLink() if torch.is_grad_enabled() else None
        y3, s3, q3 = ops.pwconv(y2, self.conv3.weight, A2, B2, ACT_SWISH, 1, stats=tr, tail=link, tail_role='y')
        A3, B3 = self.bn3.fold(s3, q3, _count(y3), n)

        if self.downsample is not None:
            if not isinstance(self.downsample, nn.Sequential):
                _, planes_out, s_ = self.downsample
                xm = x_res.materialize() if isinstance(x_res, Deferred) else x_res
                res = xm.detach()[:, :, ::s_, ::s_, ::s_]
                if planes_out > res.shape[1]:
                    res = torch.cat([res, res.new_zeros((res.shape[0], planes_out - res.shape[1]) + tuple(res.shape[2:]))], dim=1)
                return ops.bn_add_relu(y3, A3, B3, res.contiguous(), split=self.split_out, link=link)
            yd, sd, qd = ops.pwconv(_every(xr, ts), self.downsample[0].weight, xa, xb, xact, self.stride, stats=tr, token=tok, role='short',
                                    tail=link, tail_role='res')
            Ad, Bd = self.downsample[1].fold(sd, qd, _count(yd), n)
            return ops.bn_add_relu(y3, A3, B3, yd, Ad, Bd, split=self.split_out, link=link)
        res = x_res.materialize() if isinstance(x_res, Deferred) else x_res
        return ops.bn_add_relu(y3, A3, B3, res, split=self.split_out, link=link)


class ResNet(nn.Module):

    def __init__(self, block, layers, block_inplanes, n_input_channels=3, conv1_t_size=7, conv1_t_stride=1,
                 shortcut_type='B', widen_factor=1.0, dropout=0.5, n_classes=400, base_bn_splits=8, task='class',
                 extract_feat=False, global_tower=False, t_downsample=False, aux_losses=None, _skip_module_init=False,
                 act_dtype=None):
        if not _skip_module_init:
            super(ResNet, self).__init__()
        block_inplanes = [(int(x * widen_factor), int(y * widen_factor)) for x, y in block_inplanes]
        self.index = 0
        self.base_bn_splits = base_bn_splits
        self.task = task
        self.extract_feat = extract_feat
        self.global_tower = global_tower
        self.t_downsample = t_downsample
        self.act_dtype = {None: torch.float32, 'f32': torch.float32, 'fp32': torch.float32, torch.float32: torch.float32,
                          'bf16': torch.bfloat16, torch.bfloat16: torch.bfloat16,
                          'fp16': torch.float16, 'f16': torch.float16, torch.float16: torch.float16}[act_dtype]
        self.in_planes = block_inplanes[0][1]

        self.conv1_s = nn.Conv3d(n_input_channels, self.in_planes, kernel_size=(1, 3, 3), stride=(1, 2, 2),
                                 padding=(0, 1, 1), bias=False)
        self.conv1_t = nn.Conv3d(self.in_planes, self.in_planes, kernel_size=(5, 1, 1), stride=(1, 1, 1),
                                 padding=(2, 0, 0), bias=False, groups=self.in_planes)
        self.bn1 = SubBatchNorm3d(num_splits=base_bn_splits, num_features=self.in_planes, affine=True)
        self.relu = nn.ReLU(inplace=True)
        self.layer1 = self._make_layer(block, block_inplanes[0], layers[0], shortcut_type, stride=2)
        self.layer2 = self._make_layer(block, block_inplanes[1], layers[1], shortcut_type, stride=2)
        self.layer3 = self._make_layer(block, block_inplanes[2], layers[2], shortcut_type, stride=2)
        self.layer4 = self._make_layer(block, block_inplanes[3], layers[3], shortcut_type, stride=2)
        self.conv5 = nn.Conv3d(block_inplanes[3][1], block_inplanes[3][0], kernel_size=(1, 1, 1), stride=(1, 1, 1),
                               padding=(0, 0, 0), bias=False)
        self.bn5 = SubBatchNorm3d(num_splits=base_bn_splits, num_features=block_inplanes[3][0], affine=True)
        if task == 'class':
            self.avgpool = nn.AdaptiveAvgPool3d((1, 1, 1))
        elif task == 'loc':
            self.avgpool = nn.AdaptiveAvgPool3d((None, 1, 1))
        self.fc1 = nn.Conv3d(block_inplanes[3][0], 2048, bias=False, kernel_size=1, stride=1)
        self.fc2 = nn.Linear(2048, n_classes)
        self.dropout = nn.Dropout(dropout)

        for m in self.modules():
            if isinstance(m, nn.Conv3d):
                nn.init.kaiming_normal_(m.weight, mode='fan_out', nonlinearity='relu')

    def _make_layer(self, block, planes, blocks, shortcut_type, stride=1):
        downsample = None
        if stride != 1 or self.in_planes != planes[1]:
            if shortcut_type == 'A':
                downsample = ('A', planes[1], stride)
            else:
                downsample = nn.Sequential(
                    conv1x1x1(self.in_planes, planes[1], stride, t_downsample=self.t_downsample),
                    SubBatchNorm3d(num_splits=self.base_bn_splits, num_features=planes[1], affine=True))
        layers = [block(in_planes=self.in_planes, planes=planes, stride=stride, downsample=downsample,
                        index=self.index, base_bn_splits=self.base_bn_splits, t_downsample=self.t_downsample)]
        self.in_planes = planes[1]
        self.index += 1
        for _ in range(1, blocks):
            layers.append(block(self.in_planes, planes, index=self.index, base_bn_splits=self.base_bn_splits,
                                t_downsample=self.t_downsample))
            self.index += 1
        self.index = 0
        for blk in layers[:-1]:
            blk.split_out = True
        return nn.Sequential(*layers)

    def replace_logits(self, n_classes):
        self.fc2 = nn.Linear(2048, n_classes).to(self.fc1.weight.device)

    def update_bn_splits_long_cycle(self, long_cycle_bn_scale):
        for m in self.modules():
            if isinstance(m, SubBatchNorm3d):
                m.num_splits = self.base_bn_splits * long_cycle_bn_scale
                m.split_bn = nn.BatchNorm3d(num_features=m.num_features * m.num_splits, affine=False).to(m.weight.device)
        return self.base_bn_splits * long_cycle_bn_scale

    def aggregate_sub_bn_stats(self):
        count = 0
        for m in self.modules():
            if isinstance(m, SubBatchNorm3d):
                m.aggregate_stats()
                count += 1
        return count

    def _stem(self, x):
        y = ops.stem_conv(x, self.conv1_s.weight)
        y, s, q = ops.dwconv_t5(y, self.conv1_t.weight, stats=self.training, out_dtype=self.act_dtype)
        A, B = self.bn1.fold(s, q, _count(y), y.shape[0])
        return Deferred(y, A, B, ACT_RELU)

    def _head(self, x):
        n = x.shape[0]
        y5, s5, q5 = ops.pwconv(x, self.conv5.weight, stats=self.training)
        A5, B5 = self.bn5.fold(s5, q5, _count(y5), n)
        if self.task == 'class':
            pooled = ops.pool_hw(y5, 1, 1, A5, B5, ACT_RELU).mean(dim=2, keepdim=True)
        else:
            pooled = ops.pool_hw(y5, 1, 1, A5, B5, ACT_RELU)
        if self.extract_feat:
            return pooled
        f1, _, _ = ops.pwconv(pooled, self.fc1.weight, stats=False)
        one = torch.ones(n, f1.shape[1], device=f1.device)
        z = ops.affine_act(f1, one, torch.zeros_like(one), ACT_RELU)
        z = self.dropout(z)
        out, _, _ = ops.pwconv(z, self.fc2.weight.view(self.fc2.weight.shape[0], -1, 1, 1, 1), stats=False)
        out = out.squeeze(4).squeeze(3) + self.fc2.bias.view(1, -1, 1)
        return out

    def forward(self, inp):
        x, masks = inp
        x = self._stem(x)
        feat_g = {}
        for i, layer in enumerate((self.layer1, self.layer2, self.layer3, self.layer4), start=1):
            x = layer(x)
            if self.global_tower:
                feat_g['layer%d' % i] = ops.pool_hw(x, 7, 7)
        if self.global_tower:
            n = x.shape[0]
            y5, s5, q5 = ops.pwconv(x, self.conv5.weight, stats=self.training)
            A5, B5 = self.bn5.fold(s5, q5, _count(y5), n)
            feat_g['conv5'] = ops.pool_hw(y5, 7, 7, A5, B5, ACT_RELU)
            return feat_g, masks
        return self._head(x)


def replace_logits(self, n_classes):
    self.fc2 = nn.Linear(2048, n_classes)


def get_inplanes(version):
    planes = {'S': [(54, 24), (108, 48), (216, 96), (432, 192)],
              'M': [(54, 24), (108, 48), (216, 96), (432, 192)],
              'XL': [(72, 32), (162, 72), (306, 136), (630, 280)]}
    return planes[version]


def get_blocks(version):
    blocks = {'S': [3, 5, 11, 7], 'M': [3, 5, 11, 7], 'XL': [5, 10, 25, 15]}
    return blocks[version]


def generate_model(x3d_version, **kwargs):
    return ResNet(Bottleneck, get_blocks(x3d_version), get_inplanes(x3d_version), **kwargs)
```

### include/cfn_hip.h

```cpp
#ifndef CFN_HIP_H
#define CFN_HIP_H
#ifdef __cplusplus
extern "C" {
#endif

const char* cfn_last_error(void);
const char* cfn_version(void);
int cfn_device_info(int* cus, int* lds_per_cu, char* name, int name_len);

int cfn_prof_enable(int family, int on);
int cfn_prof_collect(int family, double* total_ms, long* launches, double* total_bytes);

int cfn_dwconv3d_fwd(const float* x, const double* A, const double* B, int act, const float* w, float* y, double* sum,
                     double* sumsq, int N, int C, int T, int Hi, int Wi, int stride, void* stream);
int cfn_dwconv3d_bwd_data(const float* gy, const float* y, const double* gsum, const double* gsumsq, const float* w,
                          const float* x, const double* A, const double* B, int act, float* gx, double* gA, double* gB,
                          int N, int C, int T, int Hi, int Wi, int stride, void* stream);
int cfn_dwconv3d_bwd_weight(const float* gy, const float* y, const double* gsum, const double* gsumsq, const float* x,
                            const double* A, const double* B, int act, double* gw, int N, int C, int T, int Hi, int Wi,
                            int stride, void* stream);
int cfn_dwconv3d_bwd_fused(const float* gy, const float* y, const double* gsum, const double* gsumsq, const float* w,
                           const float* x, const double* A, const double* B, int act, float* gx, double* gA, double* gB,
                           double* gw, int N, int C, int T, int H, int W, void* stream);
int cfn_dwconv3d_bwd_fused_s2(const float* gy, const float* y, const double* gsum, const double* gsumsq, const float* w,
                              const float* x, const double* A, const double* B, int act, float* gx, double* gA, double* gB,
                              double* gw, int N, int C, int T, int H, int W, void* stream);

int cfn_dwconv_t5_fwd(const float* x, const float* w, float* y, double* sum, double* sumsq, int N, int C, int T,
                      long plane, void* stream);
int cfn_dwconv_t5_bwd_data(const float* gy, const float* y, const double* gsum, const double* gsumsq, const float* w,
                           float* gx, int N, int C, int T, long plane, void* stream);
int cfn_dwconv_t5_bwd_weight(const float* gy, const float* y, const double* gsum, const double* gsumsq, const float* x,
                             double* gw, int N, int C, int T, long plane, void* stream);
int cfn_dwconv_t5_bwd_fused(const float* gy, const float* y, const double* gsum, const double* gsumsq, const float* w,
                            const float* x, float* gx, double* gw, int N, int C, int T, long plane, void* stream);

int cfn_pwconv_fwd(const float* x, const double* A, const double* B, int act, const float* w, float* y, double* sum,
                   double* sumsq, int N, int Cin, int Cout, int T, int Hi, int Wi, int stride, void* stream);
int cfn_pwconv_bwd_data(const float* gy, const float* y, const double* gsum, const double* gsumsq, const float* w,
                        const float* x, const double* A, const double* B, int act, float* gx, double* gA, double* gB, int N,
                        int Cin, int Cout, int T, int Hi, int Wi, int stride, void* stream);
int cfn_pwconv_bwd_data_acc(const float* gy, const float* y, const double* gsum, const double* gsumsq, const float* w,
                        const float* x, const double* A, const double* B, int act, float* gx, double* gA, double* gB, int N,
                        int Cin, int Cout, int T, int Hi, int Wi, int stride, const float* acc, int acc_stride,
                        const double* gscale, void* stream);
int cfn_pwconv_bwd_weight(const float* gy, const float* y, const double* gsum, const double* gsumsq, const float* x,
                          const double* A, const double* B, int act, double* gw, int N, int Cin, int Cout, int T, int Hi,
                          int Wi, int stride, const double* gscale, void* stream);

int cfn_pw_split_terms(int terms);

int cfn_deterministic(int on);

int cfn_pwconv_bwd_fused(const float* gy, const float* y, const double* gsum, const double* gsumsq, const float* w,
                         const float* x, const double* A, const double* B, int act, float* gx, double* gA, double* gB,
                         double* gw, int N, int Cin, int Cout, int T, int Hi, int Wi, const float* acc, int acc_stride,
                         const double* gscale, void* stream);

int cfn_stem_conv_fwd(const float* x, const float* w, float* y, int N, int Cimg, int Cout, int T, int Hi, int Wi,
                      void* stream);
int cfn_stem_conv_bwd_weight(const float* gy, const float* x, double* gw, int N, int Cimg, int Cout, int T, int Hi, int Wi,
                             void* stream);

int cfn_bn_fold_fwd(const double* s, const double* q, const float* gamma, const float* beta, float* run_mean, float* run_var,
                    long* nbt, int training, int N, int C, int S, double count, double eps, double momentum, const float* w1,
                    const float* b1, const float* w2, const float* b2, int Wd, double pool_count, double* A, double* B,
                    double* mean, double* rstd, float* A0, float* B0, float* gate, float* hbuf, float* pooled, void* stream);
int cfn_bn_fold_bwd(const double* gA, const double* gB, const double* s, const float* gamma, const double* mean,
                    const double* rstd, const float* A0, const float* B0, const float* gate, const float* hbuf,
                    const float* pooled, const float* w1, const float* w2, int training, int N, int C, int S, int Wd,
                    double count, double pool_count, double* gs, double* gq, float* ggamma, float* gbeta, float* gw1,
                    float* gb1, float* gw2, float* gb2, double* tA, double* tB, void* stream);

int cfn_conv3d_dense_fwd(const float* x, const double* A, const double* B, int act, const float* w, float* y, double* sum,
                         double* sumsq, int N, int Cin, int Cout, int T, int Hi, int Wi, const int* geom, void* stream);
int cfn_conv3d_dense_bwd_data(const float* gy, const float* y, const double* gsum, const double* gsumsq, const float* w,
                              const float* x, const double* A, const double* B, int act, float* gx, double* gA, double* gB,
                              int N, int Cin, int Cout, int T, int Hi, int Wi, const int* geom, void* stream);
int cfn_conv3d_dense_bwd_weight(const float* gy, const float* y, const double* gsum, const double* gsumsq, const float* x,
                                const double* A, const double* B, int act, double* gw, int N, int Cin, int Cout, int T, int Hi,
                                int Wi, const int* geom, void* stream);

int cfn_gauss_align_fwd(const long* meta, const float* mask, const float* gx, double tx, double ratio, float* GX, int B, int crops,
                        int Tf, int K, void* stream);
int cfn_gauss_align_bwd(const float* gGX, const long* meta, const float* mask, const float* gx, double tx, double ratio,
                        float* ggx, int B, int crops, int Tf, int K, void* stream);

int cfn_fusion_gather_fwd(const float* x, const float* at_raw, const float* at_bias, const float* GX, const float* mask, float* z,
                          float* den, int B, int crops, int C, int Tf, int K, int P, void* stream);
int cfn_fusion_gather_bwd(const float* gz, const float* z, const float* den, const float* x, const float* at_raw,
                          const float* at_bias, const float* GX, const float* mask, float* gx, float* gat, float* gGX, float* dw,
                          int B, int crops, int C, int Tf, int K, int P, void* stream);

int cfn_bn_add_relu_fwd(const float* y, const double* A, const double* B, const float* res, const double* Ar, const double* Br,
                        float* out, int* mask, long NC, long vol, void* stream);
int cfn_bn_add_relu_bwd(const float* gout, const float* gout2, const float* out, const float* y, const double* A, const float* res,
                        const double* Ar, float* gy, float* gres, double* gA, double* gB, double* gAr, long NC, long vol,
                        void* stream);
long cfn_bn_add_relu_mask_words(long NC, long vol);
int cfn_bn_add_relu_bwd_g(const float* gout, const float* gout2, const float* out, const int* mask, const float* y,
                          const float* res, float* g, double* gA, double* gB, double* gAr, long NC, long vol, void* stream);

int cfn_affine_act_fwd(const float* x, const double* A, const double* B, int act, float* out, long NC, long vol, void* stream);
int cfn_affine_act_bwd(const float* gout, const float* x, const double* A, const double* B, int act, float* gx, double* gA,
                       double* gB, long NC, long vol, void* stream);
int cfn_channel_stats(const float* x, double* sum, double* sumsq, long NC, long vol, void* stream);

int cfn_pool_hw_fwd(const float* x, const double* A, const double* B, int act, float* out, long NC, int T, int H, int W, int OH,
                    int OW, void* stream);
int cfn_pool_hw_bwd(const float* gout, const float* x, const double* A, const double* B, int act, float* gx, double* gA,
                    double* gB, long NC, int T, int H, int W, int OH, int OW, void* stream);

int cfn_film_fwd(const float* x, const float* m, const float* c, float* out, long NC, int T, int H, int W, int f,
                 void* stream);
int cfn_film_bwd(const float* g, const float* x, const float* m, float* gx, float* gm, float* gc, long NC, int T, int H,
                 int W, int f, void* stream);

int cfn_grid_time_index(const float* cdf, int n, int Tin, int* i0, float* w1, void* stream);
int cfn_grid_cdf_fwd(const float* g, const float* bias, float* cdf, int B, int Kin, void* stream);
int cfn_grid_cdf_bwd(const float* gcdf, const float* g, const float* bias, float* gg, int B, int Kin, void* stream);
int cfn_time_sample_fwd(const float* x, const float* cdf, float* out, int B, int C, int Tin, int K, long P, void* stream);
int cfn_time_sample_bwd(const float* g, const float* x, const float* cdf, float* gx, double* gcdf, int B, int C, int Tin,
                        int K, long P, void* stream);

int cfn_time_pool_fwd(const float* x, float* out, int mode, long BC, int Tin, int R, long P, void* stream);
int cfn_time_pool_bwd(const float* g, const float* x, float* gx, int mode, long BC, int Tin, int R, long P, void* stream);

int cfn_interp1d_fwd(const float* x, const float* y, const float* xnew, float* ynew, long* ind, int B, int N, int Pq,
                     int xrow, int yrow, int qrow, void* stream);
int cfn_interp1d_bwd(const float* g, const float* x, const float* y, const float* xnew, const long* ind, float* gx, float* gy,
                     float* gq, int B, int N, int Pq, int xrow, int yrow, int qrow, void* stream);

int cfn_time_resize_fwd(const float* x, float* out, long BC, int Kin, int Lout, long P, int align_corners, void* stream);
int cfn_time_resize_bwd(const float* g, float* gx, long BC, int Kin, int Lout, long P, int align_corners, void* stream);

int cfn_pwconv_fwd_bf16(const unsigned short* x, const double* A, const double* B, int act, const float* w, unsigned short* y,
                        double* sum, double* sumsq, int N, int Cin, int Cout, long Q, void* stream);
int cfn_pwconv_bwd_data_bf16(const unsigned short* gy, const unsigned short* y, const double* gsum, const double* gsumsq,
                             const float* w, const unsigned short* x, const double* A, const double* B, int act,
                             unsigned short* gx, double* gA, double* gB, int N, int Cin, int Cout, int T, int H, int W,
                             const unsigned short* acc, int acc_stride, const double* gscale, void* stream);
int cfn_pwconv_bwd_weight_bf16(const unsigned short* gy, const unsigned short* y, const double* gsum, const double* gsumsq,
                               const unsigned short* x, const double* A, const double* B, int act, double* gw, int N, int Cin,
                               int Cout, long Q, const double* gscale, void* stream);
int cfn_subsample_hw_bf16(const unsigned short* x, unsigned short* out, long planes, int H, int W, int s, void* stream);

int cfn_dwconv3d_fwd_bf16(const unsigned short* x, const double* A, const double* B, int act, const float* w, unsigned short* y,
                          double* sum, double* sumsq, int N, int C, int T, int Hi, int Wi, int stride, void* stream);
int cfn_dwconv3d_bwd_data_bf16(const unsigned short* gy, const unsigned short* y, const double* gsum, const double* gsumsq,
                               const float* w, const unsigned short* x, const double* A, const double* B, int act,
                               unsigned short* gx, double* gA, double* gB, int N, int C, int T, int Hi, int Wi, int stride,
                               void* stream);
int cfn_dwconv3d_bwd_weight_bf16(const unsigned short* gy, const unsigned short* y, const double* gsum, const double* gsumsq,
                                 const unsigned short* x, const double* A, const double* B, int act, double* gw, int N, int C,
                                 int T, int Hi, int Wi, int stride, void* stream);
int cfn_dwconv3d_bwd_fused_bf16(const unsigned short* gy, const unsigned short* y, const double* gsum, const double* gsumsq,
                                const float* w, const unsigned short* x, const double* A, const double* B, int act,
                                unsigned short* gx, double* gA, double* gB, double* gw, int N, int C, int T, int H, int W,
                                void* stream);
int cfn_dwconv3d_bwd_fused_s2_bf16(const unsigned short* gy, const unsigned short* y, const double* gsum, const double* gsumsq,
                                   const float* w, const unsigned short* x, const double* A, const double* B, int act,
                                   unsigned short* gx, double* gA, double* gB, double* gw, int N, int C, int T, int H, int W,
                                   void* stream);

int cfn_dwconv_t5_fwd_bf16(const float* x, const float* w, unsigned short* y, double* sum, double* sumsq, int N, int C, int T,
                           long plane, void* stream);
int cfn_dwconv_t5_bwd_data_bf16(const unsigned short* gy, const unsigned short* y, const double* gsum, const double* gsumsq,
                                const float* w, float* gx, int N, int C, int T, long plane, void* stream);
int cfn_dwconv_t5_bwd_weight_bf16(const unsigned short* gy, const unsigned short* y, const double* gsum, const double* gsumsq,
                                  const float* x, double* gw, int N, int C, int T, long plane, void* stream);
int cfn_dwconv_t5_bwd_fused_bf16(const unsigned short* gy, const unsigned short* y, const double* gsum, const double* gsumsq,
                                 const float* w, const float* x, float* gx, double* gw, int N, int C, int T, long plane,
                                 void* stream);

long cfn_bn_add_relu_mask_words_bf16(long NC, long vol);
int cfn_bn_add_relu_fwd_bf16(const unsigned short* y, const double* A, const double* B, const unsigned short* res,
                             const double* Ar, const double* Br, unsigned short* out, int* mask, long NC, long vol, void* stream);
int cfn_bn_add_relu_bwd_g_bf16(const unsigned short* gout, const unsigned short* gout2, const unsigned short* out, const int* mask,
                               const unsigned short* y, const unsigned short* res, unsigned short* g, double* gA, double* gB,
                               double* gAr, long NC, long vol, void* stream);
int cfn_pool_hw_fwd_bf16(const unsigned short* x, const double* A, const double* B, int act, float* out, long NC, int T, int H,
                         int W, int OH, int OW, void* stream);
int cfn_pool_hw_bwd_bf16(const float* gout, const unsigned short* x, const double* A, const double* B, int act,
                         unsigned short* gx, double* gA, double* gB, long NC, int T, int H, int W, int OH, int OW, void* stream);

int cfn_pwconv_fwd_f16(const unsigned short* x, const double* A, const double* B, int act, const float* w, unsigned short* y,
                        double* sum, double* sumsq, int N, int Cin, int Cout, long Q, void* stream);
int cfn_pwconv_bwd_data_f16(const unsigned short* gy, const unsigned short* y, const double* gsum, const double* gsumsq,
                             const float* w, const unsigned short* x, const double* A, const double* B, int act,
                             unsigned short* gx, double* gA, double* gB, int N, int Cin, int Cout, int T, int H, int W,
                             const unsigned short* acc, int acc_stride, const double* gscale, void* stream);
int cfn_pwconv_bwd_weight_f16(const unsigned short* gy, const unsigned short* y, const double* gsum, const double* gsumsq,
                               const unsigned short* x, const double* A, const double* B, int act, double* gw, int N, int Cin,
                               int Cout, long Q, const double* gscale, void* stream);
int cfn_subsample_hw_f16(const unsigned short* x, unsigned short* out, long planes, int H, int W, int s, void* stream);

int cfn_dwconv3d_fwd_f16(const unsigned short* x, const double* A, const double* B, int act, const float* w, unsigned short* y,
                          double* sum, double* sumsq, int N, int C, int T, int Hi, int Wi, int stride, void* stream);
int cfn_dwconv3d_bwd_data_f16(const unsigned short* gy, const unsigned short* y, const double* gsum, const double* gsumsq,
                               const float* w, const unsigned short* x, const double* A, const double* B, int act,
                               unsigned short* gx, double* gA, double* gB, int N, int C, int T, int Hi, int Wi, int stride,
                               void* stream);
int cfn_dwconv3d_bwd_weight_f16(const unsigned short* gy, const unsigned short* y, const double* gsum, const double* gsumsq,
                                 const unsigned short* x, const double* A, const double* B, int act, double* gw, int N, int C,
                                 int T, int Hi, int Wi, int stride, void* stream);
int cfn_dwconv3d_bwd_fused_f16(const unsigned short* gy, const unsigned short* y, const double* gsum, const double* gsumsq,
                                const float* w, const unsigned short* x, const double* A, const double* B, int act,
                                unsigned short* gx, double* gA, double* gB, double* gw, int N, int C, int T, int H, int W,
                                void* stream);
int cfn_dwconv3d_bwd_fused_s2_f16(const unsigned short* gy, const unsigned short* y, const double* gsum, const double* gsumsq,
                                   const float* w, const unsigned short* x, const double* A, const double* B, int act,
                                   unsigned short* gx, double* gA, double* gB, double* gw, int N, int C, int T, int H, int W,
                                   void* stream);

int cfn_dwconv_t5_fwd_f16(const float* x, const float* w, unsigned short* y, double* sum, double* sumsq, int N, int C, int T,
                           long plane, void* stream);
int cfn_dwconv_t5_bwd_data_f16(const unsigned short* gy, const unsigned short* y, const double* gsum, const double* gsumsq,
                                const float* w, float* gx, int N, int C, int T, long plane, void* stream);
int cfn_dwconv_t5_bwd_weight_f16(const unsigned short* gy, const unsigned short* y, const double* gsum, const double* gsumsq,
                                  const float* x, double* gw, int N, int C, int T, long plane, void* stream);
int cfn_dwconv_t5_bwd_fused_f16(const unsigned short* gy, const unsigned short* y, const double* gsum, const double* gsumsq,
                                 const float* w, const float* x, float* gx, double* gw, int N, int C, int T, long plane,
                                 void* stream);

long cfn_bn_add_relu_mask_words_f16(long NC, long vol);
int cfn_bn_add_relu_fwd_f16(const unsigned short* y, const double* A, const double* B, const unsigned short* res,
                             const double* Ar, const double* Br, unsigned short* out, int* mask, long NC, long vol, void* stream);
int cfn_bn_add_relu_bwd_g_f16(const unsigned short* gout, const unsigned short* gout2, const unsigned short* out, const int* mask,
                               const unsigned short* y, const unsigned short* res, unsigned short* g, double* gA, double* gB,
                               double* gAr, long NC, long vol, void* stream);
int cfn_pool_hw_fwd_f16(const unsigned short* x, const double* A, const double* B, int act, float* out, long NC, int T, int H,
                         int W, int OH, int OW, void* stream);
int cfn_pool_hw_bwd_f16(const float* gout, const unsigned short* x, const double* A, const double* B, int act,
                         unsigned short* gx, double* gA, double* gB, long NC, int T, int H, int W, int OH, int OW, void* stream);

#ifdef __cplusplus
}
#endif
#endif
```

Baseline: 103.6 clips/s.

## Fuse previous block's bn-add-relu backward into next block's pointwise conv backward

Adds a FoldLink that carries the previous bottleneck's bn_add_relu tail state (pre-activation y, residual, relu mask) into the next block's conv1 pointwise backward. The fused pwconv backward kernel gets a tail epilogue that adds the skip gradient, applies the relu mask, writes the combined gradient and reduces the BN A/B/Ar grads. The separate bn_add_relu_bwd_g pass can then be skipped. This removes one full read/write pass over the activation gradient per block, at the cost of extra per-tile loads and register/LDS pressure (lower occupancy bound) in the fused kernel.

```diff
diff --git a/coarse-fine-networks_amd/cfn_hip/ops.py b/coarse-fine-networks_amd/cfn_hip/ops.py
--- a/coarse-fine-networks_amd/cfn_hip/ops.py
+++ b/coarse-fine-networks_amd/cfn_hip/ops.py
@@ -181,6 +181,14 @@
         self.done = False
 
 
+class FoldLink(object):
+
+    def __init__(self):
+        self.tail = None
+        self.g2 = None
+        self.out = None
+
+
 def _bf(t):
     return t is not None and t.dtype in (torch.bfloat16, torch.float16)
 
@@ -195,7 +203,7 @@
 class _PwConv(Function):
 
     @staticmethod
-    def forward(ctx, x, A, B, w, act, stride, want_stats, token, role, tail=None, tail_role=None):
+    def forward(ctx, x, A, B, w, act, stride, want_stats, token, role, tail=None, tail_role=None, fold=None):
         x = check(x).contiguous()
         N, Cin, T, H, W = x.shape
         Cout = w.shape[0]
@@ -217,6 +225,7 @@
         ctx.wparam = w
         ctx.token, ctx.role = token, role
         ctx.tail, ctx.tail_role = tail, tail_role
+        ctx.fold = fold
         if not want_stats:
             return y, None, None
         return y, s, q
@@ -259,8 +268,19 @@
                         token.main_done = True
                 if stride == 1 and ctx.needs_input_grad[3]:
                     g64, fin = _gw_buffers(ctx.wparam, Cout, Cin, x.device)
-                    fused = call_try('cfn_pwconv_bwd_fused', gy, y, gs, gq, w2, x, A, B, act, gx, a64, b64, g64, N, Cin, Cout,
-                                     T, H, W, acc, acc_stride, gsc)
+                    fold = ctx.fold
+                    if (fold is not None and fold.tail is not None and A is None and
+                            ((token is None and fold.g2 is not None) or (token is not None and acc is not None and fold.g2 is None))):
+                        ty, yd, mask = fold.tail
+                        t3 = _tls.arena.take(3 * N * Cin, x.device).view(3, N, Cin)
+                        tAr = t3[2] if yd is not None else None
+                        fused = call_try('cfn_pwconv_bwd_fused_tail', gy, y, gs, gq, w2, x, gx, g64, N, Cin, Cout, T, H, W, acc,
+                                         acc_stride, gsc, fold.g2, ty, yd, mask, t3[0], t3[1], tAr)
+                        if fused:
+                            fold.out = (gx, t3[0], t3[1], tAr)
+                    if not fused:
+                        fused = call_try('cfn_pwconv_bwd_fused', gy, y, gs, gq, w2, x, A, B, act, gx, a64, b64, g64, N, Cin, Cout,
+                                         T, H, W, acc, acc_stride, gsc)
                 if not fused:
                     call('cfn_pwconv_bwd_data_acc', gy, y, gs, gq, w2, x, A, B, act, gx, a64, b64, N, Cin, Cout, T, H, W, stride,
                          acc, acc_stride, gsc)
@@ -272,7 +292,7 @@
             if not fused:
                 call('cfn_pwconv_bwd_weight', gy, y, gs, gq, x, A, B, act, g64, N, Cin, Cout, T, H, W, stride, gsc)
             gw = fin()
-        return gx, gA, gB, gw, None, None, None, None, None, None, None
+        return gx, gA, gB, gw, None, None, None, None, None, None, None, None
 
     @staticmethod
     def _backward_bf16(ctx, gy, gs, gq, gsc):
@@ -314,10 +334,10 @@
             g64, fin = _gw_buffers(ctx.wparam, Cout, Cin, x.device)
             call('cfn_pwconv_bwd_weight' + _sfx(gy), gy, y, gs, gq, xin, A, B, act, g64, N, Cin, Cout, T * Ho * Wo, gsc)
             gw = fin()
-        return gx, gA, gB, gw, None, None, None, None, None, None, None
-
-
-def pwconv(x, w, A=None, B=None, act=ACT_NONE, stride=1, stats=True, token=None, role=None, tail=None, tail_role=None):
+        return gx, gA, gB, gw, None, None, None, None, None, None, None, None
+
+
+def pwconv(x, w, A=None, B=None, act=ACT_NONE, stride=1, stats=True, token=None, role=None, tail=None, tail_role=None, fold=None):
     N, Cin, T, H, W = x.shape
     Ho, Wo = (H - 1) // stride + 1, (W - 1) // stride + 1
     es = x.element_size()
@@ -325,7 +345,7 @@
     span = max(Cin * H * W, w.shape[0] * H * W, w.shape[0] * Ho * Wo, Cin * Ho * Wo) * es
     needs_grad = torch.is_grad_enabled() and any(t is not None and t.requires_grad for t in (x, w, A, B))
     if span * T < lim or needs_grad or T == 1:
-        return _PwConv.apply(x, A, B, w, act, stride, stats, token, role, tail, tail_role)
+        return _PwConv.apply(x, A, B, w, act, stride, stats, token, role, tail, tail_role, fold)
     step = max((lim - 1) // span, 1)
     odd_plane = es == 2 and (Ho * Wo) % 2 == 1
     if odd_plane:
@@ -566,7 +586,7 @@
 class _BnAddRelu(Function):
 
     @staticmethod
-    def forward(ctx, y, A, B, res, Ar, Br, split, link):
+    def forward(ctx, y, A, B, res, Ar, Br, split, link, fold=None, park=None):
         y, res = check(y).contiguous(), check(res).contiguous()
         N, C = y.shape[:2]
         vol = y[0, 0].numel()
@@ -582,6 +602,9 @@
                 mask = torch.empty(words, dtype=torch.int32, device=y.device)
         call('cfn_bn_add_relu_fwd' + sfx, y, A, B, res, Ar, Br, out, mask, N * C, vol)
         ctx.link, ctx.has_mask = link, mask is not None
+        ctx.fold, ctx.park = fold, park
+        if fold is not None and link is not None and mask is not None and not _bf(y):
+            fold.tail = (y.detach(), res.detach() if Ar is not None else None, mask)
         ctx.save_for_backward(y, A, res, Ar, mask if mask is not None else out)
         if not split:
             return out
@@ -606,27 +629,36 @@
         gBr = gB if Ar is not None else None
         link = ctx.link
         if link is not None:
-            g = torch.empty_like(y)
-            mask = out if ctx.has_mask else None
-            call('cfn_bn_add_relu_bwd_g' + _sfx(y), gout.contiguous(), gout2, None if ctx.has_mask else out, mask, y,
-                 res if Ar is not None else None, g, gA, gB, gAr, N * C, vol)
+            fold, park = getattr(ctx, 'fold', None), getattr(ctx, 'park', None)
+            if fold is not None and fold.out is not None:
+                g, gA, gB, gAr = fold.out
+            else:
+                g = torch.empty_like(y)
+                mask = out if ctx.has_mask else None
+                call('cfn_bn_add_relu_bwd_g' + _sfx(y), gout.contiguous(), gout2, None if ctx.has_mask else out, mask, y,
+                     res if Ar is not None else None, g, gA, gB, gAr, N * C, vol)
+            if fold is not None:
+                fold.tail = fold.g2 = fold.out = None
+            if park is not None:
+                park.g2 = g
+            gBr = gB if Ar is not None else None
             link.y_scale, link.res_scale, link.done = A.detach(), (None if Ar is None else Ar.detach()), True
             g2 = torch.empty(0, dtype=g.dtype, device=g.device).set_(g.untyped_storage(), g.storage_offset(), g.shape, g.stride())
-            return g, gA, gB, g2, gAr, gBr, None, None
+            return g, gA, gB, g2, gAr, gBr, None, None, None, None
         if _bf(y):
             g = torch.empty_like(y)
             call('cfn_bn_add_relu_bwd_g' + _sfx(y), gout.contiguous(), gout2, out, None, y, res if Ar is not None else None, g, gA, gB,
                  gAr, N * C, vol)
             shp = (N, C) + (1,) * (y.dim() - 2)
             gres = g if Ar is None else (g.float() * Ar.float().view(shp)).to(y.dtype)
-            return (g.float() * A.float().view(shp)).to(y.dtype), gA, gB, gres, gAr, gBr, None, None
+            return (g.float() * A.float().view(shp)).to(y.dtype), gA, gB, gres, gAr, gBr, None, None, None, None
         gy, gres = torch.empty_like(y), torch.empty_like(res)
         call('cfn_bn_add_relu_bwd', gout.contiguous(), gout2, out, y, A, res, Ar, gy, gres, gA, gB, gAr, N * C, vol)
-        return gy, gA, gB, gres, gAr, gBr, None, None
-
-
-def bn_add_relu(y, A, B, res, Ar=None, Br=None, split=False, link=None):
-    return _BnAddRelu.apply(y, A, B, res, Ar, Br, split, link)
+        return gy, gA, gB, gres, gAr, gBr, None, None, None, None
+
+
+def bn_add_relu(y, A, B, res, Ar=None, Br=None, split=False, link=None, fold=None, park=None):
+    return _BnAddRelu.apply(y, A, B, res, Ar, Br, split, link, fold, park)
 
 
 class _AffineAct(Function):
diff --git a/coarse-fine-networks_amd/csrc/pw_common.h b/coarse-fine-networks_amd/csrc/pw_common.h
--- a/coarse-fine-networks_amd/csrc/pw_common.h
+++ b/coarse-fine-networks_amd/csrc/pw_common.h
@@ -64,9 +64,19 @@
 
 int sal_fwd_try_launch(const float* x, const double* A, const double* B, int act, const float* w, float* y, double* sum,
                        double* sumsq, int N, int Cin, int Cout, int T, int Hi, int Wi, const int* g, hipStream_t st);
+struct PwTail {
+    const float* g2; const float* y; const float* yd; const unsigned* mask; double* gA; double* gB; double* gAr; int nch;
+};
+__device__ __forceinline__ int pw_tail_mask_off(int q) { return ((q >> 13) * 256 + ((q & 1023) >> 2)) * 4; }
+__device__ __forceinline__ int pw_tail_mask_bit(int q) { return 4 * ((q >> 10) & 7) + (q & 3); }
+extern "C" long cfn_bn_add_relu_mask_words(long NC, long vol);
+static inline double pw_tail_bytes(const PwTail* t, int N, int K, long Q) {
+    return t ? 4.0 * N * K * (double)Q * ((t->g2 ? 1 : 0) + 1 + (t->yd ? 1 : 0) + 1.0 / 32) : 0.0;
+}
+
 int pwfs_try_launch(const float* gy, const float* y, const double* gsum, const double* gsumsq, const float* w, const float* x, const double* A,
                     const double* B, int act, float* gx, double* gA, double* gB, double* gw, int N, int Cin, int Cout, int T, int Hi, int Wi,
-                    const float* acc, int acc_stride, const double* gscale, hipStream_t st);
+                    const float* acc, int acc_stride, const double* gscale, hipStream_t st, const PwTail* tail = nullptr);
 int salb_fwd_try_launch(const float* x, const double* A, const double* B, int act, const float* w, float* y, double* sum,
                         double* sumsq, int N, int Cin, int Cout, int T, int Hi, int Wi, const int* g, hipStream_t st);
 int sal_wgrad_try_launch(const float* gy, const float* y, const double* gs, const double* gq, const float* x, const double* A,
diff --git a/coarse-fine-networks_amd/csrc/pwfused.hip b/coarse-fine-networks_amd/csrc/pwfused.hip
--- a/coarse-fine-networks_amd/csrc/pwfused.hip
+++ b/coarse-fine-networks_amd/csrc/pwfused.hip
@@ -15,12 +15,14 @@
     float* gx; double* gA; double* gB; double* gw;
     const float* acc; int acc_s, acc_Ho, acc_Wo, Hi, Wi, T;
     int N, M, K, Q, nstrips, stages;
+    PwTail t;
 };
 
-template <int MTW, int NTW, int ACT>
-__global__ __launch_bounds__(256, ACT < 0 ? 3 : 2) void pw_bwd_fused_kernel(const PfArgs a) {
+template <int MTW, int NTW, int ACT, bool TL = false>
+__global__ __launch_bounds__(256, ACT < 0 && !TL ? 3 : 2) void pw_bwd_fused_kernel(const PfArgs a) {
     extern __shared__ __attribute__((aligned(16))) float smem[];
     constexpr bool EPI = ACT >= 0;
+    static_assert(!(TL && EPI), "the tail epilogue replaces the act' epilogue");
     constexpr int ACTV = EPI ? ACT : CFN_ACT_NONE;
     constexpr int BM = 32 * MTW, BN = 32 * NTW;
     constexpr int NG = BM / 16, NX = BN / 16;
@@ -38,6 +40,7 @@
     float* sCz = sCg + 2 * BM;
     float* sCx = sCz + BM;
     float* sSt = sCx + 2 * BN;
+    float* sSr = sSt + 8 * BN;
     for (int m = tid; m < BM; m += 256) {
         const bool ok = m < M;
         sCg[2 * m] = (ok && a.gs) ? (float)a.gs[(long)n * M + m] : 0.0f;
@@ -77,6 +80,11 @@
     for (int t = 0; t < NT16; ++t)
 #pragma unroll
         for (int r = 0; r < 4; ++r) { sa[t][r] = 0.0f; sb[t][r] = 0.0f; }
+    float sr[TL ? NT16 : 1][4];
+#pragma unroll
+    for (int t = 0; t < (TL ? NT16 : 1); ++t)
+#pragma unroll
+        for (int r = 0; r < 4; ++r) sr[t][r] = 0.0f;
     __syncthreads();
 
     const int lrow = tid >> 4, c4 = (tid & 15) * 4;
@@ -136,6 +144,11 @@
     const int hw = a.Hi * a.Wi;
     const int acc_pitch4 = a.T * a.acc_Ho * a.acc_Wo * 4;
     __amdgpu_buffer_rsrc_t racc = cfn_rsrc(const_cast<float*>(a.acc ? a.acc + (long)n * K * (acc_pitch4 / 4) : a.gy), a.acc ? (unsigned)((long)K * acc_pitch4) : 0u);
+    const unsigned kqb = (unsigned)((long)K * Q * 4), mcb = (unsigned)a.t.nch * 1024u;
+    __amdgpu_buffer_rsrc_t rt2 = cfn_rsrc(const_cast<float*>(TL && a.t.g2 ? a.t.g2 + (long)n * K * Q : a.gy), TL && a.t.g2 ? kqb : 0u);
+    __amdgpu_buffer_rsrc_t rty = cfn_rsrc(const_cast<float*>(TL ? a.t.y + (long)n * K * Q : a.gy), TL ? kqb : 0u);
+    __amdgpu_buffer_rsrc_t rtd = cfn_rsrc(const_cast<float*>(TL && a.t.yd ? a.t.yd + (long)n * K * Q : a.gy), TL && a.t.yd ? kqb : 0u);
+    __amdgpu_buffer_rsrc_t rtm = cfn_rsrc(const_cast<float*>(TL ? reinterpret_cast<const float*>(a.t.mask + (long)n * K * a.t.nch * 256) : a.gy), TL ? (unsigned)K * mcb : 0u);
     for (int st = 0; st < nst; ++st) {
         const int q0 = qbeg + st * PF_PT;
         float* cur = img0 + (st & 1) * IMG;
@@ -161,6 +174,23 @@
             for (int i = 0; i < MTW; ++i)
 #pragma unroll
                 for (int j = 0; j < NTW; ++j) acc[i][j] = __builtin_amdgcn_mfma_f32_32x32x2f32(av[i], bv[j], acc[i][j], 0, 0, 0);
+        }
+        float tg2[TL ? NT16 : 1][4], ty3[TL ? NT16 : 1][4], tyd[TL ? NT16 : 1][4];
+        unsigned tmw[TL ? NT16 : 1][4];
+        if (TL) {
+            const int qt = q0 + pbase + m16;
+            const int mo = qt < Q ? pw_tail_mask_off(qt) + 4 * kq * (int)mcb : OOB;
+#pragma unroll
+            for (int t = 0; t < NT16; ++t)
+#pragma unroll
+                for (int r = 0; r < 4; ++r) {
+                    const int ci = t * 16 + 4 * kq + r;
+                    const int vo = (qt < Q && ci < K) ? (ci * Q + pbase + m16) * 4 : OOB;
+                    tg2[TL ? t : 0][r] = __builtin_bit_cast(float, __builtin_amdgcn_raw_buffer_load_b32(rt2, vo, q0 * 4, 0));
+                    ty3[TL ? t : 0][r] = __builtin_bit_cast(float, __builtin_amdgcn_raw_buffer_load_b32(rty, vo, q0 * 4, 0));
+                    tyd[TL ? t : 0][r] = __builtin_bit_cast(float, __builtin_amdgcn_raw_buffer_load_b32(rtd, vo, q0 * 4, 0));
+                    tmw[TL ? t : 0][r] = __builtin_amdgcn_raw_buffer_load_b32(rtm, ci < K ? mo : OOB, (t * 16 + r) * (int)mcb, 0);
+                }
         }
         pf4 da[NT16];
 #pragma unroll
@@ -208,24 +238,36 @@
                     sb[t][r] += dz;
                     v = dz * pa;
                 }
+                if (TL) {
+                    const float gs = v + tg2[TL ? t : 0][r];
+                    const float g = ((tmw[TL ? t : 0][r] >> pw_tail_mask_bit(q)) & 1u) ? gs : 0.0f;
+                    sa[t][r] = fmaf(g, ty3[TL ? t : 0][r], sa[t][r]);
+                    sb[t][r] += g;
+                    sr[TL ? t : 0][r] = fmaf(g, tyd[TL ? t : 0][r], sr[TL ? t : 0][r]);
+                    v = g;
+                }
                 __builtin_amdgcn_raw_buffer_store_b32(__builtin_bit_cast(unsigned, v), rd, ok ? (ci * Q + pbase + m16) * 4 : OOB, q0 * 4, 0);
             }
         }
         __syncthreads();
     }
 
-    if (EPI) {
+    if (EPI || TL) {
 #pragma unroll
         for (int t = 0; t < NT16; ++t)
 #pragma unroll
             for (int r = 0; r < 4; ++r) {
-                float u = sa[t][r], v = sb[t][r];
-#pragma unroll
-                for (int o = 1; o < 16; o <<= 1) { u += __shfl_xor(u, o, 64); v += __shfl_xor(v, o, 64); }
+                float u = sa[t][r], v = sb[t][r], z = sr[TL ? t : 0][r];
+#pragma unroll
+                for (int o = 1; o < 16; o <<= 1) {
+                    u += __shfl_xor(u, o, 64); v += __shfl_xor(v, o, 64);
+                    if (TL) z += __shfl_xor(z, o, 64);
+                }
                 if (m16 == 0) {
                     const int ci = t * 16 + 4 * kq + r;
                     sSt[(wave * BN + ci) * 2] = u;
                     sSt[(wave * BN + ci) * 2 + 1] = v;
+                    if (TL) sSr[wave * BN + ci] = z;
                 }
             }
     }
@@ -247,18 +289,22 @@
         const float v = (smem[o] + smem[BM * CWP + o]) + (smem[2 * BM * CWP + o] + smem[3 * BM * CWP + o]);
         if (ml < M && kl < K) cfn_add64(&a.gw[(long)ml * K + kl], (double)v);
     }
-    if (EPI && tid < K) {
+    if ((EPI || TL) && tid < K) {
         const float u = (sSt[2 * tid] + sSt[(BN + tid) * 2]) + (sSt[(2 * BN + tid) * 2] + sSt[(3 * BN + tid) * 2]);
         const float v = (sSt[2 * tid + 1] + sSt[(BN + tid) * 2 + 1]) + (sSt[(2 * BN + tid) * 2 + 1] + sSt[(3 * BN + tid) * 2 + 1]);
-        cfn_add64(&a.gA[(long)n * K + tid], (double)u);
-        cfn_add64(&a.gB[(long)n * K + tid], (double)v);
+        cfn_add64(&(TL ? a.t.gA : a.gA)[(long)n * K + tid], (double)u);
+        cfn_add64(&(TL ? a.t.gB : a.gB)[(long)n * K + tid], (double)v);
+        if (TL && a.t.gAr) {
+            const float z = (sSr[tid] + sSr[BN + tid]) + (sSr[2 * BN + tid] + sSr[3 * BN + tid]);
+            cfn_add64(&a.t.gAr[(long)n * K + tid], (double)z);
+        }
     }
 }
 
 template <int MTW, int NTW>
-static int pf_launch(const PfArgs& a, int act, bool epi, unsigned blocks, hipStream_t st) {
+static int pf_launch(const PfArgs& a, int act, bool epi, unsigned blocks, hipStream_t st, bool tl = false) {
     constexpr int BM = 32 * MTW, BN = 32 * NTW;
-    size_t lds = ((size_t)2 * (BM + BN) * PF_PITCH + 3 * BM + 10 * BN) * sizeof(float);
+    size_t lds = ((size_t)2 * (BM + BN) * PF_PITCH + 3 * BM + (tl ? 14 : 10) * BN) * sizeof(float);
     const size_t lds_cw = (size_t)4 * BM * (BN + 1) * sizeof(float);
     if (lds_cw > lds) lds = lds_cw;
 #define CFN_PF_GO(ACTV)                                                                                         \
@@ -267,7 +313,13 @@
         if (lds > 48 * 1024) (void)hipFuncSetAttribute((const void*)k, hipFuncAttributeMaxDynamicSharedMemorySize, (int)lds); \
         hipLaunchKernelGGL(k, dim3(blocks), dim3(256), lds, st, a);                                             \
     } while (0)
-    if (!epi) CFN_PF_GO(-1);
+    if (tl) {
+        if constexpr (MTW == 2 && NTW == 1) {
+            auto k = pw_bwd_fused_kernel<MTW, NTW, -1, true>;
+            if (lds > 48 * 1024) (void)hipFuncSetAttribute((const void*)k, hipFuncAttributeMaxDynamicSharedMemorySize, (int)lds);
+            hipLaunchKernelGGL(k, dim3(blocks), dim3(256), lds, st, a);
+        } else return -1;
+    } else if (!epi) CFN_PF_GO(-1);
     else if (act == CFN_ACT_RELU) CFN_PF_GO(CFN_ACT_RELU);
     else if (act == CFN_ACT_SWISH) CFN_PF_GO(CFN_ACT_SWISH);
     else CFN_PF_GO(CFN_ACT_NONE);
@@ -275,19 +327,19 @@
     return cfn_check_launch("pwconv_bwd_fused");
 }
 
-extern "C" int cfn_pwconv_bwd_fused(const float* gy, const float* y, const double* gsum, const double* gsumsq, const float* w,
-                                    const float* x, const double* A, const double* B, int act, float* gx, double* gA, double* gB,
-                                    double* gw, int N, int Cin, int Cout, int T, int Hi, int Wi, const float* acc, int acc_stride,
-                                    const double* gscale, void* stream) {
+static int pf_run(const float* gy, const float* y, const double* gsum, const double* gsumsq, const float* w, const float* x, const double* A,
+                  const double* B, int act, float* gx, double* gA, double* gB, double* gw, int N, int Cin, int Cout, int T, int Hi, int Wi,
+                  const float* acc, int acc_stride, const double* gscale, void* stream, const PwTail* tail) {
     CFN_REQUIRE(gy && w && x && gx && gw, "cfn_pwconv_bwd_fused: null tensor");
     CFN_REQUIRE((A == nullptr) == (B == nullptr), "cfn_pwconv_bwd_fused: A/B mismatch");
     CFN_REQUIRE(A == nullptr || (gA && gB), "cfn_pwconv_bwd_fused: prologue needs gA, gB");
     CFN_REQUIRE(gsumsq == nullptr || y != nullptr, "cfn_pwconv_bwd_fused: gsumsq needs y");
     CFN_REQUIRE(acc == nullptr || acc_stride >= 1, "cfn_pwconv_bwd_fused: bad acc_stride");
     {
-        const int rs = pwfs_try_launch(gy, y, gsum, gsumsq, w, x, A, B, act, gx, gA, gB, gw, N, Cin, Cout, T, Hi, Wi, acc, acc_stride, gscale, (hipStream_t)stream);
+        const int rs = pwfs_try_launch(gy, y, gsum, gsumsq, w, x, A, B, act, gx, gA, gB, gw, N, Cin, Cout, T, Hi, Wi, acc, acc_stride, gscale, (hipStream_t)stream, tail);
         if (rs != -1) return rs;
     }
+    if (tail && (A != nullptr || Cout <= 32 || Cin > 32)) return -1;
     const long Ql = (long)T * Hi * Wi;
     if (Cin > 64 || Cout > 64 || (Cin > 32 && Cout > 32) || Ql % 4 != 0 || Ql >= (1L << 30)) return -1;
     if ((long)Cout * Ql * 4 >= 0x7ffffff0L || (long)Cin * Ql * 4 >= 0x7ffffff0L) return -1;
@@ -300,10 +352,11 @@
     a.acc = acc; a.acc_s = acc ? acc_stride : 1; a.Hi = Hi; a.Wi = Wi; a.T = T;
     a.acc_Ho = (Hi - 1) / a.acc_s + 1; a.acc_Wo = (Wi - 1) / a.acc_s + 1;
     a.N = N; a.M = Cout; a.K = Cin; a.Q = (int)Ql;
+    if (tail) a.t = *tail;
     const long nst = cfn_cdiv(Ql, PF_PT);
     const bool epi = A != nullptr;
     static const int wgs_env = getenv("CFN_PWF_WGS") ? atoi(getenv("CFN_PWF_WGS")) : 0;
-    long want = (wgs_env > 0 ? wgs_env : (epi ? 1024 : 1536)) / N;
+    long want = (wgs_env > 0 ? wgs_env : (epi || tail ? 1024 : 1536)) / N;
     if (want < 1) want = 1;
     long stages = cfn_cdiv(nst, want);
     if (stages < 4) stages = 4;
@@ -311,8 +364,31 @@
     a.nstrips = (int)cfn_cdiv(nst, stages);
     const unsigned blocks = (unsigned)((long)N * a.nstrips);
     hipStream_t st = (hipStream_t)stream;
-    CfnProfScope prof(CFN_K_PWCONV_BWD, st, 4.0 * N * ((double)Cout * Ql * (a.y ? 2 : 1) + (double)Cin * Ql * 2));
-    if (Cout > 32) return pf_launch<2, 1>(a, act, epi, blocks, st);
+    CfnProfScope prof(CFN_K_PWCONV_BWD, st, 4.0 * N * ((double)Cout * Ql * (a.y ? 2 : 1) + (double)Cin * Ql * 2) + pw_tail_bytes(tail, N, Cin, Ql));
+    if (Cout > 32) return pf_launch<2, 1>(a, act, epi, blocks, st, tail != nullptr);
     if (Cin > 32) return pf_launch<1, 2>(a, act, epi, blocks, st);
     return pf_launch<1, 1>(a, act, epi, blocks, st);
 }
+
+extern "C" int cfn_pwconv_bwd_fused(const float* gy, const float* y, const double* gsum, const double* gsumsq, const float* w,
+                                    const float* x, const double* A, const double* B, int act, float* gx, double* gA, double* gB,
+                                    double* gw, int N, int Cin, int Cout, int T, int Hi, int Wi, const float* acc, int acc_stride,
+                                    const double* gscale, void* stream) {
+    return pf_run(gy, y, gsum, gsumsq, w, x, A, B, act, gx, gA, gB, gw, N, Cin, Cout, T, Hi, Wi, acc, acc_stride, gscale, stream, nullptr);
+}
+
+extern "C" int cfn_pwconv_bwd_fused_tail(const float* gy, const float* y, const double* gsum, const double* gsumsq, const float* w,
+                                         const float* x, float* g, double* gw, int N, int Cin, int Cout, int T, int Hi, int Wi,
+                                         const float* acc, int acc_stride, const double* gscale, const float* g2, const float* ty,
+                                         const float* yd, const int* mask, double* tA, double* tB, double* tAr, void* stream) {
+    CFN_REQUIRE(ty && tA && tB, "cfn_pwconv_bwd_fused_tail: null tensor");
+    CFN_REQUIRE(tAr == nullptr || yd != nullptr, "cfn_pwconv_bwd_fused_tail: gAr needs yd");
+    { const char* e = getenv("CFN_TAIL_FOLD"); if (e && !atoi(e)) return -1; }
+    const long Ql = (long)T * Hi * Wi;
+    if (mask == nullptr || Ql % 4 != 0 || cfn_bn_add_relu_mask_words((long)N * Cin, Ql) <= 0) return -1;
+    PwTail t = {};
+    t.g2 = g2; t.y = ty; t.yd = tAr ? yd : nullptr; t.mask = (const unsigned*)mask; t.gA = tA; t.gB = tB; t.gAr = tAr;
+    t.nch = (int)cfn_cdiv(Ql, 8192L);
+    return pf_run(gy, y, gsum, gsumsq, w, x, nullptr, nullptr, CFN_ACT_NONE, g, nullptr, nullptr, gw, N, Cin, Cout, T, Hi, Wi, acc, acc_stride,
+                  gscale, stream, &t);
+}
diff --git a/coarse-fine-networks_amd/csrc/pwfuseds.hip b/coarse-fine-networks_amd/csrc/pwfuseds.hip
--- a/coarse-fine-networks_amd/csrc/pwfuseds.hip
+++ b/coarse-fine-networks_amd/csrc/pwfuseds.hip
@@ -37,12 +37,14 @@
     const float* acc; int acc_s, acc_Ho, acc_Wo, Hi, Wi, T;
     int N, M, K, Q, nstrips, stages;
     int dbg;
+    PwTail t;
 };
 
-template <int MTW, int NTW, int ACT>
+template <int MTW, int NTW, int ACT, bool TL = false>
 __global__ __launch_bounds__(512, 1) void pw_bwd_fused_split_kernel(const PfsArgs a) {
     extern __shared__ __attribute__((aligned(16))) float smem[];
     constexpr bool EPI = ACT >= 0;
+    static_assert(!(TL && EPI), "the tail epilogue replaces the act' epilogue");
     constexpr int ACTV = EPI ? ACT : CFN_ACT_NONE;
     constexpr int BM = 32 * MTW, BN = 32 * NTW;
     constexpr int NG = BM / 16, NX = BN / 16;
@@ -62,6 +64,7 @@
     float* sCx = smem + 2 * IMG + 3 * BM;
     float* sSt = sCx + 2 * BN;
     unsigned* sW = reinterpret_cast<unsigned*>(sSt + 8 * BN);
+    float* sSr = reinterpret_cast<float*>(sW + 3 * BN * (BMP / 2));
     for (int k = tid; k < BN; k += 512) {
         const bool ok = EPI && k < K;
         sCx[2 * k] = ok ? (float)a.pa[(long)n * K + k] : 1.0f;
@@ -223,6 +226,16 @@
         for (int t = 0; t < NT16; ++t)
 #pragma unroll
             for (int r = 0; r < 4; ++r) { sa[t][r] = 0.0f; sb[t][r] = 0.0f; }
+        float sr[TL ? NT16 : 1][4];
+#pragma unroll
+        for (int t = 0; t < (TL ? NT16 : 1); ++t)
+#pragma unroll
+            for (int r = 0; r < 4; ++r) sr[t][r] = 0.0f;
+        const unsigned kqb = (unsigned)((long)K * Q * 4), mcb = (unsigned)a.t.nch * 1024u;
+        __amdgpu_buffer_rsrc_t rt2 = cfn_rsrc(const_cast<float*>(TL && a.t.g2 ? a.t.g2 + (long)n * K * Q : a.gy), TL && a.t.g2 ? kqb : 0u);
+        __amdgpu_buffer_rsrc_t rty = cfn_rsrc(const_cast<float*>(TL ? a.t.y + (long)n * K * Q : a.gy), TL ? kqb : 0u);
+        __amdgpu_buffer_rsrc_t rtd = cfn_rsrc(const_cast<float*>(TL && a.t.yd ? a.t.yd + (long)n * K * Q : a.gy), TL && a.t.yd ? kqb : 0u);
+        __amdgpu_buffer_rsrc_t rtm = cfn_rsrc(const_cast<float*>(TL ? reinterpret_cast<const float*>(a.t.mask + (long)n * K * a.t.nch * 256) : a.gy), TL ? (unsigned)K * mcb : 0u);
         const int hw = a.Hi * a.Wi;
         const int acc_pitch4 = a.T * a.acc_Ho * a.acc_Wo * 4;
         __amdgpu_buffer_rsrc_t racc = cfn_rsrc(const_cast<float*>(a.acc ? a.acc + (long)n * K * (acc_pitch4 / 4) : a.gy), a.acc ? (unsigned)((long)K * acc_pitch4) : 0u);
@@ -257,6 +270,23 @@
 #undef PFS_DG
                     if (NT16 > 4 && (t & 1)) __builtin_amdgcn_sched_barrier(0);
                 }
+            }
+            float tg2[TL ? NT16 : 1][4], ty3[TL ? NT16 : 1][4], tyd[TL ? NT16 : 1][4];
+            unsigned tmw[TL ? NT16 : 1][4];
+            if (TL) {
+                const int qt = q0 + pbase + m16;
+                const int tvo = qt < Q ? (4 * kq * Q + pbase + m16) * 4 : OOB;
+                const int mo = qt < Q ? pw_tail_mask_off(qt) + 4 * kq * (int)mcb : OOB;
+#pragma unroll
+                for (int t = 0; t < NT16; ++t)
+#pragma unroll
+                    for (int r = 0; r < 4; ++r) {
+                        const int so = (q0 + (t * 16 + r) * Q) * 4;
+                        tg2[TL ? t : 0][r] = __builtin_bit_cast(float, __builtin_amdgcn_raw_buffer_load_b32(rt2, tvo, so, 0));
+                        ty3[TL ? t : 0][r] = __builtin_bit_cast(float, __builtin_amdgcn_raw_buffer_load_b32(rty, tvo, so, 0));
+                        tyd[TL ? t : 0][r] = __builtin_bit_cast(float, __builtin_amdgcn_raw_buffer_load_b32(rtd, tvo, so, 0));
+                        tmw[TL ? t : 0][r] = __builtin_amdgcn_raw_buffer_load_b32(rtm, mo, (t * 16 + r) * (int)mcb, 0);
+                    }
             }
             const int q = q0 + pbase + m16;
             const bool qv = q < Q;
@@ -303,34 +333,50 @@
                         sb[t][r] += dz;
                         v = dz * pa;
                     }
+                    if (TL) {
+                        const float gs = v + tg2[TL ? t : 0][r];
+                        const float g = ((tmw[TL ? t : 0][r] >> pw_tail_mask_bit(q)) & 1u) ? gs : 0.0f;
+                        sa[t][r] = fmaf(g, ty3[TL ? t : 0][r], sa[t][r]);
+                        sb[t][r] += g;
+                        sr[TL ? t : 0][r] = fmaf(g, tyd[TL ? t : 0][r], sr[TL ? t : 0][r]);
+                        v = g;
+                    }
                     __builtin_amdgcn_raw_buffer_store_b32(__builtin_bit_cast(unsigned, v), rd, gvo, (q0 + (t * 16 + r) * Q) * 4, 0);
                 }
                 if (NT16 > 4) __builtin_amdgcn_sched_barrier(0);
             }
             __syncthreads();
         }
-        if (EPI) {
+        if (EPI || TL) {
 #pragma unroll
             for (int t = 0; t < NT16; ++t)
 #pragma unroll
                 for (int r = 0; r < 4; ++r) {
-                    float u = sa[t][r], v = sb[t][r];
-#pragma unroll
-                    for (int o = 1; o < 16; o <<= 1) { u += __shfl_xor(u, o, 64); v += __shfl_xor(v, o, 64); }
+                    float u = sa[t][r], v = sb[t][r], z = sr[TL ? t : 0][r];
+#pragma unroll
+                    for (int o = 1; o < 16; o <<= 1) {
+                        u += __shfl_xor(u, o, 64); v += __shfl_xor(v, o, 64);
+                        if (TL) z += __shfl_xor(z, o, 64);
+                    }
                     if (m16 == 0) {
                         const int ci = t * 16 + 4 * kq + r;
                         sSt[((wave & 3) * BN + ci) * 2] = u;
                         sSt[((wave & 3) * BN + ci) * 2 + 1] = v;
+                        if (TL) sSr[(wave & 3) * BN + ci] = z;
                     }
                 }
         }
         __syncthreads();
         const int t2 = tid - 256;
-        if (EPI && t2 < K) {
+        if ((EPI || TL) && t2 < K) {
             const float u = (sSt[2 * t2] + sSt[(BN + t2) * 2]) + (sSt[(2 * BN + t2) * 2] + sSt[(3 * BN + t2) * 2]);
             const float v = (sSt[2 * t2 + 1] + sSt[(BN + t2) * 2 + 1]) + (sSt[(2 * BN + t2) * 2 + 1] + sSt[(3 * BN + t2) * 2 + 1]);
-            cfn_add64(&a.gA[(long)n * K + t2], (double)u);
-            cfn_add64(&a.gB[(long)n * K + t2], (double)v);
+            cfn_add64(&(TL ? a.t.gA : a.gA)[(long)n * K + t2], (double)u);
+            cfn_add64(&(TL ? a.t.gB : a.gB)[(long)n * K + t2], (double)v);
+            if (TL && a.t.gAr) {
+                const float z = (sSr[t2] + sSr[BN + t2]) + (sSr[2 * BN + t2] + sSr[3 * BN + t2]);
+                cfn_add64(&a.t.gAr[(long)n * K + t2], (double)z);
+            }
         }
         __syncthreads();
     }
@@ -346,9 +392,9 @@
 }
 
 template <int MTW, int NTW>
-static int pfs_launch(const PfsArgs& a, int act, bool epi, unsigned blocks, hipStream_t st) {
+static int pfs_launch(const PfsArgs& a, int act, bool epi, unsigned blocks, hipStream_t st, bool tl = false) {
     constexpr int BM = 32 * MTW, BN = 32 * NTW, BMP = BM + 8;
-    size_t lds = ((size_t)2 * (BM + BN) * PFS_PITCH + 3 * BM + 10 * BN) * sizeof(float) + (size_t)3 * BN * BMP * 2;
+    size_t lds = ((size_t)2 * (BM + BN) * PFS_PITCH + 3 * BM + 10 * BN) * sizeof(float) + (size_t)3 * BN * BMP * 2 + (tl ? (size_t)4 * BN * sizeof(float) : 0);
     const size_t lds_cw = (size_t)4 * (MTW * NTW / 2) * 32 * 33 * sizeof(float);
     if (lds_cw > lds) lds = lds_cw;
 #define CFN_PFS_GO(ACTV)                                                                                        \
@@ -357,7 +403,13 @@
         (void)hipFuncSetAttribute((const void*)k, hipFuncAttributeMaxDynamicSharedMemorySize, (int)lds);        \
         hipLaunchKernelGGL(k, dim3(blocks), dim3(512), lds, st, a);                                             \
     } while (0)
-    if (!epi) CFN_PFS_GO(-1);
+    if (tl) {
+        if constexpr (MTW == 4 && NTW == 1) {
+            auto k = pw_bwd_fused_split_kernel<MTW, NTW, -1, true>;
+            (void)hipFuncSetAttribute((const void*)k, hipFuncAttributeMaxDynamicSharedMemorySize, (int)lds);
+            hipLaunchKernelGGL(k, dim3(blocks), dim3(512), lds, st, a);
+        } else return -1;
+    } else if (!epi) CFN_PFS_GO(-1);
     else if (act == CFN_ACT_RELU) CFN_PFS_GO(CFN_ACT_RELU);
     else if (act == CFN_ACT_SWISH) CFN_PFS_GO(CFN_ACT_SWISH);
     else CFN_PFS_GO(CFN_ACT_NONE);
@@ -1012,7 +1064,7 @@
 
 int pwfs_try_launch(const float* gy, const float* y, const double* gsum, const double* gsumsq, const float* w, const float* x, const double* A,
                     const double* B, int act, float* gx, double* gA, double* gB, double* gw, int N, int Cin, int Cout, int T, int Hi, int Wi,
-                    const float* acc, int acc_stride, const double* gscale, hipStream_t st) {
+                    const float* acc, int acc_stride, const double* gscale, hipStream_t st, const PwTail* tail) {
     const char* env_on = getenv("CFN_PWF_SPLIT");
     const int on = env_on ? atoi(env_on) : 1;
     if (!on || pws_terms_now() != 6) return -1;
@@ -1021,6 +1073,7 @@
     const bool wide_k = Cin > 64 && Cin <= 128 && Cout > 32 && Cout <= 64;
     const bool l1_m = on >= 3 && Cout > 32 && Cout <= 64 && Cin >= 16 && Cin <= 32;
     const bool l1_k = on >= 3 && Cin > 32 && Cin <= 64 && Cout >= 16 && Cout <= 32;
+    if (tail && (A != nullptr || !thin_k)) return -1;
     static const int l3_on = getenv("CFN_PWF_L3") ? atoi(getenv("CFN_PWF_L3")) : 1;
     if (on >= 1 && l3_on && A == nullptr && Cout > 192 && Cout <= 224 && Cin > 32 && Cin <= 96) {
         const long Ql3 = (long)T * Hi * Wi;
@@ -1052,6 +1105,7 @@
     a.acc_Ho = (Hi - 1) / a.acc_s + 1; a.acc_Wo = (Wi - 1) / a.acc_s + 1;
     a.N = N; a.M = Cout; a.K = Cin; a.Q = (int)Ql;
     { const char* e = getenv("CFN_PWFS_DBG"); a.dbg = e ? atoi(e) : 0; }
+    if (tail) a.t = *tail;
     const long nst = cfn_cdiv(Ql, PFS_PT);
     static const int wgs = getenv("CFN_PWFS_WGS") ? atoi(getenv("CFN_PWFS_WGS")) : 512;
     long want = wgs / N;
@@ -1061,10 +1115,10 @@
     a.stages = (int)stages;
     a.nstrips = (int)cfn_cdiv(nst, stages);
     const unsigned blocks = (unsigned)((long)N * a.nstrips);
-    CfnProfScope prof(CFN_K_PWCONV_BWD, st, 4.0 * N * ((double)Cout * Ql * (a.y ? 2 : 1) + (double)Cin * Ql * 2));
+    CfnProfScope prof(CFN_K_PWCONV_BWD, st, 4.0 * N * ((double)Cout * Ql * (a.y ? 2 : 1) + (double)Cin * Ql * 2) + pw_tail_bytes(tail, N, Cin, Ql));
     const bool epi = A != nullptr;
-    if (wide_m) return pfs_launch<4, 2>(a, act, epi, blocks, st);
-    if (thin_k) return pfs_launch<4, 1>(a, act, epi, blocks, st);
+    if (wide_m) return pfs_launch<4, 2>(a, act, epi, blocks, st, tail != nullptr);
+    if (thin_k) return pfs_launch<4, 1>(a, act, epi, blocks, st, tail != nullptr);
     if (l1_m) return pfs_launch<2, 1>(a, act, epi, blocks, st);
     if (l1_k) return pfs_launch<1, 2>(a, act, epi, blocks, st);
     return pfs_launch<2, 4>(a, act, epi, blocks, st);
diff --git a/coarse-fine-networks_amd/x3d_fine.py b/coarse-fine-networks_amd/x3d_fine.py
--- a/coarse-fine-networks_amd/x3d_fine.py
+++ b/coarse-fine-networks_amd/x3d_fine.py
@@ -111,6 +111,12 @@
 
 def _count(y):
     return y.shape[2] * y.shape[3] * y.shape[4]
+
+
+def _with_fold(out, fold):
+    if fold is not None:
+        (out[0] if isinstance(out, tuple) else out)._cfn_fold = fold
+    return out
 
 
 class Bottleneck(nn.Module):
@@ -175,7 +181,9 @@
     def forward(self, x):
         if USE_TORCH_OPS:
             return self._forward_torch_ops(x)
-        x, x_res = x if isinstance(x, tuple) else (x, x)
+        pair = isinstance(x, tuple)
+        x, x_res = x if pair else (x, x)
+        fold_in = getattr(x, '_cfn_fold', None)
         xr, xa, xb, xact = _unpack(x)
         n = xr.shape[0]
         tr = self.training
@@ -183,7 +191,10 @@
 
         ts = self.t_stride
         tok = ops.ShortcutToken() if (isinstance(self.downsample, nn.Sequential) and self.stride > 1 and ts == 1) else None
-        y1, s1, q1 = ops.pwconv(xr, self.conv1.weight, xa, xb, xact, 1, stats=tr, token=tok, role='main')
+        park = fold_in if (pair and self.downsample is None) else None
+        if park is None and tok is None:
+            fold_in = None
+        y1, s1, q1 = ops.pwconv(xr, self.conv1.weight, xa, xb, xact, 1, stats=tr, token=tok, role='main', fold=fold_in)
         A1, B1 = self.bn1.fold(s1, q1, _count(y1), n)
         if ts == 1:
             y2, s2, q2 = ops.dwconv3d(y1, self.conv2.weight, A1, B1, ACT_RELU, self.stride, stats=tr or has_se)
@@ -194,6 +205,7 @@
         se = (self.fc1.weight, self.fc1.bias, self.fc2.weight, self.fc2.bias) if has_se else None
         A2, B2 = self.bn2.fold(s2, q2, _count(y2), n, se=se)
         link = ops.TailLink() if torch.is_grad_enabled() else None
+        fold = ops.FoldLink() if link is not None else None
         y3, s3, q3 = ops.pwconv(y2, self.conv3.weight, A2, B2, ACT_SWISH, 1, stats=tr, tail=link, tail_role='y')
         A3, B3 = self.bn3.fold(s3, q3, _count(y3), n)
 
@@ -204,13 +216,13 @@
                 res = xm.detach()[:, :, ::s_, ::s_, ::s_]
                 if planes_out > res.shape[1]:
                     res = torch.cat([res, res.new_zeros((res.shape[0], planes_out - res.shape[1]) + tuple(res.shape[2:]))], dim=1)
-                return ops.bn_add_relu(y3, A3, B3, res.contiguous(), split=self.split_out, link=link)
+                return _with_fold(ops.bn_add_relu(y3, A3, B3, res.contiguous(), split=self.split_out, link=link, fold=fold), fold)
             yd, sd, qd = ops.pwconv(_every(xr, ts), self.downsample[0].weight, xa, xb, xact, self.stride, stats=tr, token=tok, role='short',
                                     tail=link, tail_role='res')
             Ad, Bd = self.downsample[1].fold(sd, qd, _count(yd), n)
-            return ops.bn_add_relu(y3, A3, B3, yd, Ad, Bd, split=self.split_out, link=link)
+            return _with_fold(ops.bn_add_relu(y3, A3, B3, yd, Ad, Bd, split=self.split_out, link=link, fold=fold), fold)
         res = x_res.materialize() if isinstance(x_res, Deferred) else x_res
-        return ops.bn_add_relu(y3, A3, B3, res, split=self.split_out, link=link)
+        return _with_fold(ops.bn_add_relu(y3, A3, B3, res, split=self.split_out, link=link, fold=fold, park=park), fold)
 
 
 class ResNet(nn.Module):
@@ -329,6 +341,7 @@
         for i, layer in enumerate((self.layer1, self.layer2, self.layer3, self.layer4), start=1):
             x = layer(x)
             if self.global_tower:
+                x._cfn_fold = None
                 feat_g['layer%d' % i] = ops.pool_hw(x, 7, 7)
         if self.global_tower:
             n = x.shape[0]
diff --git a/include/cfn_hip.h b/include/cfn_hip.h
--- a/include/cfn_hip.h
+++ b/include/cfn_hip.h
@@ -56,6 +56,10 @@
                          const float* x, const double* A, const double* B, int act, float* gx, double* gA, double* gB,
                          double* gw, int N, int Cin, int Cout, int T, int Hi, int Wi, const float* acc, int acc_stride,
                          const double* gscale, void* stream);
+int cfn_pwconv_bwd_fused_tail(const float* gy, const float* y, const double* gsum, const double* gsumsq, const float* w,
+                              const float* x, float* g, double* gw, int N, int Cin, int Cout, int T, int Hi, int Wi,
+                              const float* acc, int acc_stride, const double* gscale, const float* g2, const float* ty,
+                              const float* yd, const int* mask, double* tA, double* tB, double* tAr, void* stream);
 
 int cfn_stem_conv_fwd(const float* x, const float* w, float* y, int N, int Cimg, int Cout, int T, int Hi, int Wi,
                       void* stream);
```

Result: no change. 104.4 clips/s (median of 6 runs) (+0.7%).
